# zjykzj/YOLOv4

Measured on AMD Instinct MI355X. Metric: images/sec fwd+bwd @608x608 bs=64 per GPU (YOLOv4 training step: forward + YOLOLoss + backward), higher is better.
Workload: dtype f32

## Files before the change

include/yolov4_amd.h:

```cpp
#ifndef YOLOV4_AMD_H
#define YOLOV4_AMD_H

#include <stddef.h>
#include <stdint.h>

#ifdef __cplusplus
extern "C" {
#endif

#define Y4_OK 0
#define Y4_ERR_SHAPE 1
#define Y4_ERR_NULL 2
#define Y4_ERR_LAUNCH 3
#define Y4_ERR_WORKSPACE 4
#define Y4_ERR_NODEVICE 5
#define Y4_ERR_FORMAT 6
#define Y4_ERR_UNSUPPORTED 7

#define Y4_ACT_LINEAR 0
#define Y4_ACT_LEAKY 1
#define Y4_ACT_MISH 2
#define Y4_ACT_RELU 3

const char* y4_strerror(int code);
int y4_version(void);
int y4_device_count(void);

int y4_set_conv_mode(int mode);
int y4_get_conv_mode(void);
int y4_set_planes_bf16(int on);
int y4_get_planes_bf16(void);
int y4_conv_planes_fit(int B, int H, int W, int Cin, int Cout, int k, int stride, int dgrad_planes);
size_t y4_conv2d_fwd_workspace(int Cin, int Cout, int k);
int y4_conv2d_fwd_f32(const float* x, int ldx, const float* w, float* y, int ldy,
                      int B, int H, int W, int Cin, int Cout, int k, int stride,
                      const float* scale, const float* shift, int act,
                      const float* residual, int ldr, const unsigned* x_amax ,
                      unsigned* y_amax ,
                      void* workspace, size_t workspace_bytes, void* stream);
size_t y4_conv2d_prepared_bytes(int Cout, int K);
int y4_conv2d_prepare_filter_f32(const float* w, int Cout, int K, void* prepared, size_t prepared_bytes, void* stream);
int y4_conv2d_fwd_prepared_f32(const float* x, int ldx, void* w_prepared, float* y, int ldy,
                               int B, int H, int W, int Cin, int Cout, int k, int stride,
                               const float* scale, const float* shift, int act,
                               const float* residual, int ldr, const unsigned* x_amax, unsigned* y_amax, void* stream);
int y4_amax_f32(const float* x, int ldx, long long M, int C, unsigned* amax_bits, void* stream);
int y4_amax_merge_u32(unsigned* dst, const unsigned* src, void* stream);

int y4_last_conv_kernel(char* buf, int cap);

size_t y4_conv2d_bnstats_workspace(int B, int H, int W, int Cin, int Cout, int k, int stride);
int y4_conv2d_fwd_bnstats_f32(const float* x, int ldx, const float* w, float* y, int ldy,
                              int B, int H, int W, int Cin, int Cout, int k, int stride,
                              float* partials, size_t partial_bytes, long long* nparts_host,
                              const unsigned* x_amax ,
                              void* workspace, size_t workspace_bytes ,
                              void* dgrad_filter ,
                              size_t dgrad_filter_bytes , void* stream);

int y4_planes_split_f32(const float* x, int ldx, long long M, int C, const unsigned* amax, void* planes, void* stream);
int y4_planes_split_into_f32(const float* x, int ldx, long long M, int C, const unsigned* amax, void* planes, int ld_planes, int c_valid,
                             void* stream);
int y4_conv2d_fwd_planes_f32(const void* x_planes, const float* w, float* y, int ldy,
                             int B, int H, int W, int Cin, int Cout, int k, int stride,
                             float* partials, size_t partial_bytes, long long* nparts_host, const unsigned* x_amax,
                             void* workspace, size_t workspace_bytes,
                             void* dgrad_filter ,
                             size_t dgrad_filter_bytes,
                             int y_bf16 ,
                             const float* bias ,
                             void* stream);

int y4_conv2d_dgrad_planes_f32(const void* dy_planes, const float* w , float* dx, int lddx,
                               int B, int H, int W, int Cin, int Cout, int k,
                               int stride ,
                               void* workspace, size_t workspace_bytes, const unsigned* dy_amax,
                               const float* residual, int ldr, void* stream);
size_t y4_conv2d_wgrad_planes_workspace(int B, int H, int W, int Cin, int Cout, int k, int stride);
int y4_conv2d_wgrad_planes_f32(const void* x_planes, const void* dy_planes, float* dw,
                               int B, int H, int W, int Cin, int Cout, int k, int stride,
                               void* workspace, size_t workspace_bytes, const unsigned* x_amax, const unsigned* dy_amax,
                               void* stream);

int y4_conv2d_generic_fwd_f32(const float* x, int ldx, const float* w, float* y, int ldy,
                              int B, int H, int W, int Cin, int Cout, int k, int stride,
                              const float* scale, const float* shift, int act, const float* residual, int ldr, void* stream);
int y4_conv2d_generic_dgrad_f32(const float* dy, int lddy, const float* w, float* dx, int lddx,
                                int B, int H, int W, int Cin, int Cout, int k, int stride,
                                const float* residual, int ldr, void* stream);
int y4_conv2d_generic_wgrad_f32(const float* x, int ldx, const float* dy, int lddy, float* dw,
                                int B, int H, int W, int Cin, int Cout, int k, int stride, void* stream);
int y4_conv2d_stem_dgrad_f32(const float* dy, int lddy, const float* w, float* dx, long long sxb, long long sxc, long long sxh,
                             long long sxw, int B, int H, int W, int Cout, void* stream);

int y4_conv2d_stem_fwd_f32(const float* x, long long sxb, long long sxc, long long sxh, long long sxw,
                           const float* w, float* y, int ldy, int B, int H, int W, int Cout,
                           const float* scale, const float* shift, int act,
                           float* bnstats_partials, void* stream);

size_t y4_conv2d_dgrad_workspace(int Cin, int Cout, int k);
int y4_conv2d_dgrad_f32(const float* dy, int lddy, const float* w , float* dx, int lddx,
                        int B, int H, int W, int Cin, int Cout, int k, int stride,
                        void* workspace, size_t workspace_bytes, const unsigned* dy_amax ,
                        const float* residual, int ldr, void* stream);

size_t y4_conv2d_wgrad_workspace(int B, int H, int W, int Cin, int Cout, int k, int stride);
int y4_conv2d_wgrad_f32(const float* x, int ldx, const float* dy, int lddy, float* dw,
                        int B, int H, int W, int Cin, int Cout, int k, int stride,
                        void* workspace, size_t workspace_bytes,
                        const unsigned* x_amax, const unsigned* dy_amax , void* stream);
size_t y4_conv2d_stem_wgrad_workspace(int B, int H, int W, int Cout);
int y4_conv2d_stem_wgrad_f32(const float* x, long long sxb, long long sxc, long long sxh, long long sxw,
                             const float* dy, int lddy, float* dw, int B, int H, int W, int Cout,
                             void* workspace, size_t workspace_bytes, void* stream);

int y4_stem_fused_ok(long long sxb, long long sxc, long long sxh, long long sxw, int B, int H, int W, int Cout);
size_t y4_stem_bn_act_fwd_workspace(int B, int H, int W, int Cout);
int y4_stem_bn_act_fwd_f32(const float* x, long long sxb, long long sxc, long long sxh, long long sxw, const float* w,
                           int B, int H, int W, int Cout, const float* gamma, const float* beta, int act,
                           float* mean, float* invstd, float* running_mean, float* running_var, long long* num_batches_tracked,
                           float momentum, float eps, float* z, int ldz, unsigned* out_amax,
                           void* workspace, size_t workspace_bytes, void* stream);
size_t y4_stem_bn_act_bwd_workspace(int B, int H, int W, int Cout);
int y4_stem_bn_act_bwd_f32(const float* x, long long sxb, long long sxc, long long sxh, long long sxw, const float* w,
                           const float* dz, int lddz, const float* mean, const float* invstd, const float* gamma,
                           const float* beta, int act, int B, int H, int W, int Cout,
                           float* dgamma, float* dbeta, float* dw, void* workspace, size_t workspace_bytes, void* stream);

size_t y4_bn_workspace(long long M, int C);
size_t y4_bn_finalize_workspace(int C);
int y4_bn_stats_f32(const float* y, int ldy, long long M, int C, float* mean, float* invstd,
                    float* running_mean, float* running_var, long long* num_batches_tracked,
                    float momentum, float eps, void* workspace, size_t workspace_bytes, void* stream);
int y4_bn_finalize_partials_f32(const float* partials, long long nparts, long long M, int C,
                                float* mean, float* invstd, float* running_mean, float* running_var,
                                long long* num_batches_tracked, float momentum, float eps,
                                void* workspace, size_t workspace_bytes, void* stream);
int y4_bn_planes_bound_f32(const float* gamma, const float* beta, int C, long long M, const unsigned* floor_word, unsigned* out,
                           void* stream);
int y4_bn_act_fwd_f32(const float* y, int ldy, const float* mean, const float* invstd,
                      const float* gamma, const float* beta, int act,
                      const float* residual, int ldr, float* z, int ldz,
                      long long M, int C, unsigned* out_amax, int z_planes, const unsigned* res_amax, float* planes_twin,
                      void* stream);
int y4_bn_act_bwd_f32(const float* dz, int lddz, const float* y, int ldy,
                      const float* mean, const float* invstd, const float* gamma, const float* beta,
                      int act, float* dy, int lddy, float* dgamma, float* dbeta,
                      long long M, int C, void* workspace, size_t workspace_bytes,
                      unsigned* out_amax ,
                      unsigned* f16_planes ,
                      float* planes_twin ,
                      int frozen_stats ,
                      void* stream);
size_t y4_bias_grad_workspace(long long M, int C);
int y4_bias_grad_f32(const float* dy, int lddy, long long M, int C, float* dbias,
                     void* workspace, size_t workspace_bytes, void* stream);
int y4_bn_fold_f32(const float* gamma, const float* beta, const float* running_mean,
                   const float* running_var, float eps, float* scale, float* shift, int C, void* stream);

int y4_copy_channels_f32(const float* src, int lds, float* dst, int ldd, long long M, int C, void* stream);
int y4_add_f32(const float* a, int lda, const float* b, int ldb, float* out, int ldo,
               long long M, int C, void* stream);
int y4_maxpool_s1_fwd_f32(const float* x, int ldx, float* y, int ldy, signed char* idx,
                          int B, int H, int W, int C, int ksize, void* stream);
int y4_maxpool_s1_bwd_f32(const float* dy, int lddy, const signed char* idx, float* dx, int lddx,
                          int accumulate, int B, int H, int W, int C, int ksize, void* stream);
int y4_upsample2x_fwd_f32(const float* x, int ldx, float* y, int ldy, int B, int H, int W, int C, void* stream);
int y4_upsample2x_bwd_f32(const float* dy, int lddy, float* dx, int lddx, int B, int H, int W, int C, void* stream);

int y4_yolo_decode_train_f32(const float* logits, int ldl, float* output, float* pred,
                             int B, int F, int A, int n_classes, const float* anchors_wh_host, void* stream);
int y4_yolo_decode_eval_f32(const float* logits, int ldl, float* out, long long n_total, long long box_off,
                            int B, int F, int A, int n_classes, const float* anchors_wh_host,
                            float stride, void* stream);
int y4_yolo_decode_bwd_f32(const float* logits, int ldl, const float* g_output, const float* g_pred,
                           float* g_logits, int B, int F, int A, int n_classes,
                           const float* anchors_wh_host, void* stream);

size_t y4_yolo_loss_workspace(int B, int F, int A, int K, int n_classes);
int y4_yolo_loss_fwd_f32(const float* output, const float* pred, const float* labels, int K,
                         int B, int F, int A, int n_classes, float stride, float ignore_thresh,
                         const float* all_anchors_host, int n_all_anchors, const int* anch_mask_host,
                         float* obj_mask, double* loss_parts,
                         void* workspace, size_t workspace_bytes, void* stream);
int y4_yolo_loss_bwd_f32(const float* output, int output_is_masked, const float* obj_mask,
                         const float* gscale, float* g_output,
                         int B, int F, int A, int K, int n_classes,
                         const void* workspace, size_t workspace_bytes, void* stream);
int y4_yolo_loss_mask_output_f32(float* output, const float* obj_mask, int B, int F, int A, int K,
                                 int n_classes, const void* workspace, size_t workspace_bytes, void* stream);
// ... 206 lines not shown
```

yolov4_amd/_lib.py:

```python
import ctypes
import os
from ctypes import c_char_p, c_double, c_float, c_int, c_longlong, c_size_t, c_void_p

_HERE = os.path.dirname(os.path.abspath(__file__))
LIB_PATH = os.environ.get('Y4_LIB_PATH') or os.path.join(_HERE, 'lib', 'libyolov4_amd.so')

ACT_IDS = {'linear': 0, 'leaky_relu': 1, 'mish': 2, 'relu': 3}


class Y4Error(RuntimeError):
    pass


P = c_void_p
I, L, F, Z = c_int, c_longlong, c_float, c_size_t

PROTOTYPES = {
    'y4_strerror': (c_char_p, [I]),
    'y4_version': (I, []),
    'y4_device_count': (I, []),
    'y4_set_conv_mode': (I, [I]),
    'y4_get_conv_mode': (I, []),
    'y4_set_planes_bf16': (I, [I]),
    'y4_get_planes_bf16': (I, []),
    'y4_conv_planes_fit': (I, [I, I, I, I, I, I, I, I]),
    'y4_conv2d_fwd_workspace': (Z, [I, I, I]),
    'y4_conv2d_fwd_f32': (I, [P, I, P, P, I, I, I, I, I, I, I, I, P, P, I, P, I, P, P, P, Z, P]),
    'y4_amax_f32': (I, [P, I, L, I, P, P]),
    'y4_conv2d_prepared_bytes': (Z, [I, I]),
    'y4_conv2d_prepare_filter_f32': (I, [P, I, I, P, Z, P]),
    'y4_conv2d_fwd_prepared_f32': (I, [P, I, P, P, I, I, I, I, I, I, I, I, P, P, I, P, I, P, P, P]),
    'y4_amax_merge_u32': (I, [P, P, P]),
    'y4_last_conv_kernel': (I, [ctypes.c_char_p, I]),
    'y4_conv2d_bnstats_workspace': (Z, [I, I, I, I, I, I, I]),
    'y4_conv2d_fwd_bnstats_f32': (I, [P, I, P, P, I, I, I, I, I, I, I, I, P, Z, P, P, P, Z, P, Z, P]),
    'y4_planes_split_f32': (I, [P, I, L, I, P, P, P]),
    'y4_planes_split_into_f32': (I, [P, I, L, I, P, P, I, I, P]),
    'y4_conv2d_fwd_planes_f32': (I, [P, P, P, I, I, I, I, I, I, I, I, P, Z, P, P, P, Z, P, Z, I, P, P]),
    'y4_conv2d_dgrad_planes_f32': (I, [P, P, P, I, I, I, I, I, I, I, I, P, Z, P, P, I, P]),
    'y4_conv2d_wgrad_planes_workspace': (Z, [I, I, I, I, I, I, I]),
    'y4_conv2d_wgrad_planes_f32': (I, [P, P, P, I, I, I, I, I, I, I, P, Z, P, P, P]),
    'y4_conv2d_generic_fwd_f32': (I, [P, I, P, P, I, I, I, I, I, I, I, I, P, P, I, P, I, P]),
    'y4_conv2d_generic_dgrad_f32': (I, [P, I, P, P, I, I, I, I, I, I, I, I, P, I, P]),
    'y4_conv2d_generic_wgrad_f32': (I, [P, I, P, I, P, I, I, I, I, I, I, I, P]),
    'y4_conv2d_stem_dgrad_f32': (I, [P, I, P, P, L, L, L, L, I, I, I, I, P]),
    'y4_conv2d_stem_fwd_f32': (I, [P, L, L, L, L, P, P, I, I, I, I, I, P, P, I, P, P]),
    'y4_conv2d_dgrad_workspace': (Z, [I, I, I]),
    'y4_conv2d_dgrad_f32': (I, [P, I, P, P, I, I, I, I, I, I, I, I, P, Z, P, P, I, P]),
    'y4_conv2d_wgrad_workspace': (Z, [I, I, I, I, I, I, I]),
    'y4_conv2d_wgrad_f32': (I, [P, I, P, I, P, I, I, I, I, I, I, I, P, Z, P, P, P]),
    'y4_conv2d_stem_wgrad_workspace': (Z, [I, I, I, I]),
    'y4_conv2d_stem_wgrad_f32': (I, [P, L, L, L, L, P, I, P, I, I, I, I, P, Z, P]),
    'y4_stem_fused_ok': (I, [L, L, L, L, I, I, I, I]),
    'y4_stem_bn_act_fwd_workspace': (Z, [I, I, I, I]),
    'y4_stem_bn_act_fwd_f32': (I, [P, L, L, L, L, P, I, I, I, I, P, P, I, P, P, P, P, P, F, F, P, I, P, P, Z, P]),
    'y4_stem_bn_act_bwd_workspace': (Z, [I, I, I, I]),
    'y4_stem_bn_act_bwd_f32': (I, [P, L, L, L, L, P, P, I, P, P, P, P, I, I, I, I, I, P, P, P, P, Z, P]),
    'y4_bn_workspace': (Z, [L, I]),
    'y4_bn_finalize_workspace': (Z, [I]),
    'y4_bn_finalize_partials_f32': (I, [P, L, L, I, P, P, P, P, P, F, F, P, Z, P]),
    'y4_bn_stats_f32': (I, [P, I, L, I, P, P, P, P, P, F, F, P, Z, P]),
    'y4_bn_act_fwd_f32': (I, [P, I, P, P, P, P, I, P, I, P, I, L, I, P, I, P, P, P]),
    'y4_bn_planes_bound_f32': (I, [P, P, I, L, P, P, P]),
    'y4_bn_act_bwd_f32': (I, [P, I, P, I, P, P, P, P, I, P, I, P, P, L, I, P, Z, P, P, P, I, P]),
    'y4_bias_grad_workspace': (Z, [L, I]),
    'y4_bias_grad_f32': (I, [P, I, L, I, P, P, Z, P]),
    'y4_bn_fold_f32': (I, [P, P, P, P, F, P, P, I, P]),
    'y4_copy_channels_f32': (I, [P, I, P, I, L, I, P]),
    'y4_add_f32': (I, [P, I, P, I, P, I, L, I, P]),
    'y4_maxpool_s1_fwd_f32': (I, [P, I, P, I, P, I, I, I, I, I, P]),
    'y4_maxpool_s1_bwd_f32': (I, [P, I, P, P, I, I, I, I, I, I, I, P]),
    'y4_upsample2x_fwd_f32': (I, [P, I, P, I, I, I, I, I, P]),
    'y4_upsample2x_bwd_f32': (I, [P, I, P, I, I, I, I, I, P]),
    'y4_yolo_decode_train_f32': (I, [P, I, P, P, I, I, I, I, P, P]),
    'y4_yolo_decode_eval_f32': (I, [P, I, P, L, L, I, I, I, I, P, F, P]),
    'y4_yolo_decode_bwd_f32': (I, [P, I, P, P, P, I, I, I, I, P, P]),
    'y4_yolo_loss_workspace': (Z, [I, I, I, I, I]),
    'y4_yolo_loss_fwd_f32': (I, [P, P, P, I, I, I, I, I, F, F, P, I, P, P, P, P, Z, P]),
    'y4_yolo_loss_bwd_f32': (I, [P, I, P, P, P, I, I, I, I, I, P, Z, P]),
    'y4_yolo_loss_mask_output_f32': (I, [P, P, I, I, I, I, I, P, Z, P]),
    'y4_yolo_loss_dense_targets_f32': (I, [P, P, P, I, I, I, I, I, P, Z, P]),
    'y4_yolo_box_loss_fwd_f32': (I, [P, I, F, I, I, I, I, I, P, P, Z, P]),
    'y4_yolo_box_loss_bwd_f32': (I, [P, I, F, P, P, I, I, I, I, I, P, Z, P]),
    'y4_post_count_f32': (I, [P, I, L, I, F, I, P, P]),
    'y4_post_scan_i32': (I, [P, I, L, P, P, P]),
    'y4_post_compact_f32': (I, [P, P, P, I, I, P, P, P, P]),
    'y4_post_nms_workspace': (Z, [L, I]),
    'y4_post_nms_f32': (I, [P, I, L, I, F, F, P, L, P, P, P, Z, P]),
    'y4_post_count_ex_f32': (I, [P, I, L, I, F, I, I, P, P]),
    'y4_post_nms_ex_workspace': (Z, [L, I, P]),
    'y4_post_nms_ex_f32': (I, [P, I, L, I, F, F, P, P, L, P, P, P, Z, P]),
    'y4_post_topk_workspace': (Z, [L, I]),
    'y4_post_topk_compact_f32': (I, [P, P, P, I, I, I, L, P, P, P, P, Z, P]),
    'y4_nms_workspace': (Z, [L]),
    'y4_nms_f32': (I, [P, P, L, F, I, P, P, P, Z, P]),
    'y4_bboxes_iou_f32': (I, [P, L, P, L, I, P, P]),
    'y4_act_fwd_f32': (I, [P, P, L, I, P]),
    'y4_act_bwd_f32': (I, [P, P, P, L, I, P]),
    'y4_upsample_nearest_fwd_f32': (I, [P, I, P, I, I, I, I, I, I, I, I, P]),
    'y4_upsample_nearest_bwd_f32': (I, [P, I, P, I, I, I, I, I, I, I, I, P]),
    'y4_adam_step_f32': (I, [P, P, P, P, L, F, F, F, F, F, I, F, P]),
    'y4_adam_hyper_f32': (I, [F, F, F, F, I, P]),
    'y4_adam_multi_step_f32': (I, [P, I, P, I, F, F, F, F, P]),
    'y4_sgd_multi_step_f32': (I, [P, I, P, I, F, P]),
    'y4_grad_sumsq_multi_f32': (I, [P, I, F, P, P]),
    'y4_grad_guard_f32': (I, [P, I, c_double, P, P]),
    'y4_adam_multi_step_guarded_f32': (I, [P, I, P, I, F, F, F, F, P, P]),
    'y4_sgd_multi_step_guarded_f32': (I, [P, I, P, I, F, P, P]),
    'y4_ema_multi_f32': (I, [P, I, F, P, P]),
    'y4_preprocess_u8_f32': (I, [P, I, I, L, I, P, L, L, L, I, P]),
    'y4_augment_means_u8': (I, [P, P, I, P, P]),
    'y4_augment_mosaic_u8_f32': (I, [P, P, I, P, P, I, P, P, L, L, L, L, I, P]),
    'y4_avgpool_global_fwd_f32': (I, [P, I, P, I, I, I, I, P]),
    'y4_avgpool_global_bwd_f32': (I, [P, I, P, I, I, I, I, P]),
    'y4_linear_fwd_f32': (I, [P, I, P, P, P, I, I, I, I, P]),
    'y4_linear_bwd_f32': (I, [P, I, P, P, I, P, I, P, P, I, I, I, P]),
    'y4_ce_smooth_fwd_f32': (I, [P, I, P, I, I, c_double, P, P, P]),
    'y4_ce_smooth_bwd_f32': (I, [P, I, P, P, P, P, I, I, I, c_double, P]),
    'y4_topk_correct_f32': (I, [P, I, P, I, I, P, I, P, P, P]),
    'y4_coco_workspace': (Z, [I, I]),
    'y4_coco_match_f64': (I, [P, P, P, I, P, P, P, P, P, I, I, P, P, P, P, P, Z, P]),
    'y4_coco_accumulate_f64': (I, [P, P, P, I, P, P, P, I, P, P, P, P, P]),
    'y4_jpeg_parse_host': (I, [P, Z, P]),
    'y4_jpeg_entropy_host': (I, [P, Z, P, P, L, P]),
    'y4_jpeg_workspace': (Z, [P, I]),
    'y4_jpeg_decode_u8': (I, [P, P, I, P, Z, P]),
    'y4_jpeg_encode_setup': (I, [I, I, I, I, I, I, P, P]),
    'y4_jpeg_encode_u8': (I, [P, P, I, P]),
    'y4_jpeg_encode_bound': (Z, [P]),
    'y4_jpeg_encode_host': (I, [P, P, P, P, Z, P]),
    'y4_draw_boxes_u8': (I, [P, P, I, P]),
}

ERR_FORMAT, ERR_UNSUPPORTED = 6, 7


NMS_METRICS = {'iou': 0, 'diou': 1}
NMS_SOFT = {None: 0, 'linear': 1, 'gaussian': 2}


class NmsOpts(ctypes.Structure):
    _fields_ = [('metric', c_int), ('soft', c_int), ('sigma', c_float), ('agnostic', c_int), ('max_det', c_int),
                ('reserved', c_int * 3)]


class AugSrc(ctypes.Structure):
    _fields_ = [('src', c_void_p), ('h', c_int), ('w', c_int), ('pitch', c_longlong), ('swap_rb', c_int),
                ('crop_left', c_int), ('crop_top', c_int), ('crop_w', c_int), ('crop_h', c_int), ('flip', c_int),
                ('color', c_int), ('dhue', c_float), ('dsat', c_float), ('dexp', c_float), ('win_x', c_int),
                ('win_y', c_int)]


class AugSample(ctypes.Structure):
    _fields_ = [('cut_x', c_int), ('cut_y', c_int), ('n_src', c_int), ('first', c_int)]


class JpegInfo(ctypes.Structure):
    _fields_ = [('width', c_int), ('height', c_int), ('ncomp', c_int), ('hs', c_int * 3), ('vs', c_int * 3),
                ('mcus_x', c_int), ('mcus_y', c_int), ('blocks_w', c_int * 3), ('blocks_h', c_int * 3),
                ('restart_interval', c_int), ('orientation', c_int), ('reserved', c_int), ('coef_count', c_longlong)]


class JpegJob(ctypes.Structure):
    _fields_ = [('coef', c_void_p), ('out', c_void_p), ('out_pitch', c_longlong), ('ws_offset', c_longlong),
                ('info', JpegInfo), ('apply_orientation', c_int), ('swap_rb', c_int), ('qt', (ctypes.c_uint16 * 64) * 3)]


class JpegEncJob(ctypes.Structure):
    _fields_ = [('pixels', c_void_p), ('coef', c_void_p), ('pitch', c_longlong), ('info', JpegInfo), ('swap_rb', c_int),
                ('reserved', c_int * 3), ('qt', (ctypes.c_uint16 * 64) * 3)]


class DrawBox(ctypes.Structure):
    _fields_ = [('x1', c_int), ('y1', c_int), ('x2', c_int), ('y2', c_int), ('half', c_int), ('px1', c_int), ('py1', c_int),
                ('px2', c_int), ('py2', c_int), ('tx', c_int), ('ty', c_int), ('scale', c_int), ('text_off', c_int),
                ('text_len', c_int), ('color', ctypes.c_uint8 * 4), ('reserved', c_int)]


class DrawJob(ctypes.Structure):
    _fields_ = [('image', c_void_p), ('pitch', c_longlong), ('width', c_int), ('height', c_int), ('boxes', c_void_p),
                ('boxes_host', c_void_p), ('text', c_void_p), ('glyphs', c_void_p), ('n_boxes', c_int), ('text_bytes', c_int),
                ('n_glyphs', c_int), ('reserved', c_int)]


_lib = None


def lib():
    global _lib
    if _lib is None:
        if not os.path.isfile(LIB_PATH):
            raise Y4Error(f'{LIB_PATH} is missing: build it with `make -C yolov4_amd/csrc` '
                          '(hipcc --offload-arch=gfx950); there is no fallback path')
        handle = ctypes.CDLL(LIB_PATH)
        for name, (res, args) in PROTOTYPES.items():
            fn = getattr(handle, name)
            fn.restype = res
            fn.argtypes = args
# ... 20 lines not shown
```

yolov4_amd/csrc/conv_f16x2.hip:

```cpp
#include <stdlib.h>
#include "common.h"
#include <cstdlib>
#include "conv_geom.h"

namespace {

using y4::ConvGeom;
using y4::WgradGeom;

typedef _Float16 f16x8 __attribute__((ext_vector_type(8)));
typedef _Float16 f16x2v __attribute__((ext_vector_type(2)));
typedef unsigned int u32x2 __attribute__((ext_vector_type(2)));

__device__ __host__ __forceinline__ unsigned f16x2_scale_exp(unsigned amax_bits) {
    const unsigned e = (amax_bits >> 23) & 0xffu;
    if (e == 0u || e == 255u) return 127u;
    int se = 268 - (int)e;
    if (se < 2) se = 2;
    if (se > 252) se = 252;
    return (unsigned)se;
}
__device__ __forceinline__ float f16x2_scale(const unsigned* amax) {
    return __uint_as_float(f16x2_scale_exp(amax ? *amax : 0u) << 23);
}
// ... 1292 lines not shown
        const f32x4 v = *reinterpret_cast<const f32x4*>(x + row * ld + c);
#pragma unroll
        for (int e = 0; e < 4; ++e) {
            const unsigned b = __float_as_uint(v[e]) & 0x7fffffffu;
            if (c + e < C && b < 0x7f800000u && b > m) m = b;
        }
    }
    amax_block_commit(m, out);
}
__global__ __launch_bounds__(256) void amax_strided_kernel(const float* __restrict__ x, long long ld, long long M, int C,
                                                           unsigned* __restrict__ out) {
    unsigned m = 0u;
    const long long total = M * C;
    for (long long i = blockIdx.x * (long long)blockDim.x + threadIdx.x; i < total; i += (long long)gridDim.x * blockDim.x) {
        const long long row = i / C;
        const unsigned b = __float_as_uint(x[row * ld + (i - row * C)]) & 0x7fffffffu;
        if (b < 0x7f800000u && b > m) m = b;
    }
    amax_block_commit(m, out);
}
__global__ void amax_merge_kernel(unsigned* __restrict__ dst, const unsigned* __restrict__ src) {
    if (threadIdx.x == 0 && blockIdx.x == 0) { const unsigned v = *src; if (v) atomicMax(dst, v); }
}

constexpr int AMAX_PART_MAX = 1024;
__global__ __launch_bounds__(256) void amax_partials_kernel(const float* __restrict__ x, long long n, unsigned* __restrict__ part) {
    __shared__ unsigned wmax[4];
    unsigned m = 0u;
    const long long n4 = n >> 2;
    for (long long i = blockIdx.x * (long long)blockDim.x + threadIdx.x; i < n4; i += (long long)gridDim.x * blockDim.x) {
        const f32x4 v = *reinterpret_cast<const f32x4*>(x + 4 * i);
#pragma unroll
        for (int e = 0; e < 4; ++e) {
            const unsigned b = __float_as_uint(v[e]) & 0x7fffffffu;
            if (b < 0x7f800000u && b > m) m = b;
        }
    }
    if (blockIdx.x == 0 && threadIdx.x < (int)(n & 3)) {
        const unsigned b = __float_as_uint(x[(n4 << 2) + threadIdx.x]) & 0x7fffffffu;
        if (b < 0x7f800000u && b > m) m = b;
    }
#pragma unroll
    for (int off = 32; off > 0; off >>= 1) {
        const unsigned o = (unsigned)__shfl_xor((int)m, off, 64);
        m = o > m ? o : m;
    }
    if ((threadIdx.x & 63) == 0) wmax[threadIdx.x >> 6] = m;
    __syncthreads();
    if (threadIdx.x == 0) {
        const unsigned a = wmax[0] > wmax[1] ? wmax[0] : wmax[1], b = wmax[2] > wmax[3] ? wmax[2] : wmax[3];
        part[blockIdx.x] = a > b ? a : b;
    }
}
__device__ __forceinline__ unsigned amax_fold_partials(const unsigned* __restrict__ part, int nparts, unsigned* __restrict__ out) {
    __shared__ unsigned wmax[4];
    unsigned m = 0u;
    for (int i = threadIdx.x; i < nparts; i += 256) { const unsigned v = part[i]; m = v > m ? v : m; }
#pragma unroll
    for (int off = 32; off > 0; off >>= 1) {
        const unsigned o = (unsigned)__shfl_xor((int)m, off, 64);
        m = o > m ? o : m;
    }
    if ((threadIdx.x & 63) == 0) wmax[threadIdx.x >> 6] = m;
    __syncthreads();
    const unsigned a = wmax[0] > wmax[1] ? wmax[0] : wmax[1], b = wmax[2] > wmax[3] ? wmax[2] : wmax[3];
    const unsigned v = a > b ? a : b;
    if (blockIdx.x == 0 && threadIdx.x == 0) *out = v;
    return v;
}
__global__ __launch_bounds__(256) void f16x2_split_filter_folded_kernel(const float* __restrict__ w, unsigned short* __restrict__ planes,
                                                                        long long n, const unsigned* __restrict__ part, int nparts,
                                                                        unsigned* __restrict__ amax_out) {
    const unsigned amax = amax_fold_partials(part, nparts, amax_out);
    const float s = __uint_as_float(f16x2_scale_exp(amax) << 23);
    for (long long i = blockIdx.x * (long long)blockDim.x + threadIdx.x; i < n; i += (long long)gridDim.x * blockDim.x) {
        unsigned short hi, lo;
        split2(w[i], s, hi, lo);
        const long long o = (i >> 5) * 64 + (i & 31);
        planes[o] = hi;
        planes[o + 32] = lo;
    }
}
__global__ __launch_bounds__(256) void f16x2_split_filter_dual_kernel(const float* __restrict__ w, unsigned short* __restrict__ planes,
                                                                      unsigned short* __restrict__ planes_t, int Cout, int Cin, int kk,
                                                                      int Cout_pad, const unsigned* __restrict__ part, int nparts,
                                                                      unsigned* __restrict__ amax_out, unsigned* __restrict__ amax_out_t,
                                                                      int mirror) {
    const unsigned amax = amax_fold_partials(part, nparts, amax_out);
    if (blockIdx.x == 0 && threadIdx.x == 0) *amax_out_t = amax;
    const float s = __uint_as_float(f16x2_scale_exp(amax) << 23);
    const long long n = (long long)Cout * kk * Cin;
    for (long long i = blockIdx.x * (long long)blockDim.x + threadIdx.x; i < n; i += (long long)gridDim.x * blockDim.x) {
        unsigned short hi, lo;
        split2(w[i], s, hi, lo);
        const long long o = (i >> 5) * 64 + (i & 31);
        planes[o] = hi;
        planes[o + 32] = lo;
    }
    const long long total = (long long)Cin * kk * Cout_pad;
    for (long long i = blockIdx.x * (long long)blockDim.x + threadIdx.x; i < total; i += (long long)gridDim.x * blockDim.x) {
        const int nn = (int)(i % Cout_pad);
        const long long t = i / Cout_pad;
        const int tp = (int)(t % kk);
        const int tap = mirror ? kk - 1 - tp : tp;
        const int c = (int)(t / kk);
        const float v = nn < Cout ? w[((long long)nn * kk + tap) * Cin + c] : 0.0f;
        unsigned short hi, lo;
        split2(v, s, hi, lo);
        const long long o = (i >> 5) * 64 + (i & 31);
        planes_t[o] = hi;
        planes_t[o + 32] = lo;
    }
}
__global__ __launch_bounds__(256) void f16x2_transpose_split_filter_folded_kernel(const float* __restrict__ w,
                                                                                  unsigned short* __restrict__ planes, int Cout, int Cin,
                                                                                  int kk, int Cout_pad, const unsigned* __restrict__ part,
                                                                                  int nparts, unsigned* __restrict__ amax_out, int mirror) {
    const unsigned amax = amax_fold_partials(part, nparts, amax_out);
    const float s = __uint_as_float(f16x2_scale_exp(amax) << 23);
    const long long total = (long long)Cin * kk * Cout_pad;
    for (long long i = blockIdx.x * (long long)blockDim.x + threadIdx.x; i < total;
         i += (long long)gridDim.x * blockDim.x) {
        const int n = (int)(i % Cout_pad);
        const long long t = i / Cout_pad;
        const int tp = (int)(t % kk);
        const int tap = mirror ? kk - 1 - tp : tp;
        const int c = (int)(t / kk);
        const float v = n < Cout ? w[((long long)n * kk + tap) * Cin + c] : 0.0f;
        unsigned short hi, lo;
        split2(v, s, hi, lo);
        const long long o = (i >> 5) * 64 + (i & 31);
        planes[o] = hi;
        planes[o + 32] = lo;
    }
}

constexpr int FP_PARTS = 256;
__global__ __launch_bounds__(256) void f16x2_refresh_filter_kernel(const float* __restrict__ w, unsigned short* __restrict__ planes,
                                                                   long long n, unsigned* part_max, unsigned long long* part_sum,
                                                                   unsigned* hdr) {
    __shared__ unsigned wmax[4];
    __shared__ unsigned long long wsum[4];
    __shared__ int is_last;
    unsigned m = 0u;
    unsigned long long cs = 0ull;
    auto take = [&](const float x, const unsigned long long i) {
        const unsigned bits = __float_as_uint(x);
        cs += (unsigned long long)bits * (2ull * i + 1ull) + 0x9e3779b97f4a7c15ull;
        const unsigned b = bits & 0x7fffffffu;
        if (b < 0x7f800000u && b > m) m = b;
    };
    {
        const long long n4 = n >> 2, stride = (long long)gridDim.x * blockDim.x;
        long long i = blockIdx.x * (long long)blockDim.x + threadIdx.x;
        for (; i + 3 * stride < n4; i += 4 * stride) {
            f32x4 v[4];
#pragma unroll
            for (int u = 0; u < 4; ++u) v[u] = *reinterpret_cast<const f32x4*>(w + 4 * (i + u * stride));
#pragma unroll
            for (int u = 0; u < 4; ++u)
#pragma unroll
                for (int e = 0; e < 4; ++e) take(v[u][e], (unsigned long long)(4 * (i + u * stride) + e));
        }
        for (; i < n4; i += stride) {
            const f32x4 v = *reinterpret_cast<const f32x4*>(w + 4 * i);
#pragma unroll
            for (int e = 0; e < 4; ++e) take(v[e], (unsigned long long)(4 * i + e));
        }
        if (blockIdx.x == 0 && threadIdx.x < (int)(n & 3)) take(w[(n4 << 2) + threadIdx.x], (unsigned long long)((n4 << 2) + threadIdx.x));
    }
#pragma unroll
    for (int off = 32; off > 0; off >>= 1) {
        const unsigned o = (unsigned)__shfl_xor((int)m, off, 64);
        m = o > m ? o : m;
        cs += __shfl_xor(cs, off, 64);
    }
    if ((threadIdx.x & 63) == 0) { wmax[threadIdx.x >> 6] = m; wsum[threadIdx.x >> 6] = cs; }
    __syncthreads();
    if (threadIdx.x == 0) {
        const unsigned a = wmax[0] > wmax[1] ? wmax[0] : wmax[1], b = wmax[2] > wmax[3] ? wmax[2] : wmax[3];
        __hip_atomic_store(part_max + blockIdx.x, a > b ? a : b, __ATOMIC_RELAXED, __HIP_MEMORY_SCOPE_AGENT);
        __hip_atomic_store(part_sum + blockIdx.x, wsum[0] + wsum[1] + wsum[2] + wsum[3], __ATOMIC_RELAXED, __HIP_MEMORY_SCOPE_AGENT);
        asm volatile("s_waitcnt vmcnt(0)" ::: "memory");
        const unsigned t = __hip_atomic_fetch_add(hdr + 5, 1u, __ATOMIC_RELAXED, __HIP_MEMORY_SCOPE_AGENT);
        is_last = t == gridDim.x - 1;
    }
    __syncthreads();
    if (!is_last) return;
    m = 0u; cs = 0ull;
// ... 107 lines not shown
    const size_t smem = 2ull * 2 * (TN_ + TJ_) * ROWB;
    auto kern = conv_wgrad_f16x2<TN_, TJ_, MS>;
    static Y4DynLds lds_attr;
    if (!lds_attr.ensure(reinterpret_cast<const void*>(kern), smem)) return Y4_ERR_LAUNCH;
    y4::note_kernel("conv_wgrad_f16x2<%d, %d, %d>", TN_, TJ_, MS);
    hipLaunchKernelGGL(kern, dim3(g.ntn * g.ntj * g.splits), dim3(256), smem, st, g);
    Y4_CHECK_LAUNCH();
    return Y4_OK;
}

int f16x2_shape() {
    static int s = -1;
    if (s < 0) {
        const char* e = getenv("Y4_F16X2_SHAPE");
        s = e ? atoi(e) : g_f16x2_shape;
        if (s != 16 && s != 32) s = g_f16x2_shape;
    }
    return s;
}

}

namespace y4 {

int f16x2_gather(const ConvGeom& g, bool transposed, hipStream_t st, int* nparts) {
    if (!transposed && !g.scale && !g.shift && !g.dst_amax && g.act == Y4_ACT_LINEAR && g.pad == 1 &&
        tile_conv_ok(g.Cs, g.Cs_valid, g.N, g.k, g.stride, g.Hs, g.Ws))
        return f16x2_tile(g, st, nparts);
    if (stream1x1_f16x2_ok(g)) return dispatch_stream1x1_f16x2(g, st, nparts);
    if (halo_ok(g)) {
        if (f16x2_shape() == 16) return transposed ? launch_halo_f16x2<true, 16>(g, st, nparts) : launch_halo_f16x2<false, 16>(g, st, nparts);
        return transposed ? launch_halo_f16x2<true, 32>(g, st, nparts) : launch_halo_f16x2<false, 32>(g, st, nparts);
    }
    if (f16x2_shape() == 16)
        return transposed ? dispatch_gather_f16x2<true, 16>(g, st, nparts) : dispatch_gather_f16x2<false, 16>(g, st, nparts);
    return transposed ? dispatch_gather_f16x2<true, 32>(g, st, nparts) : dispatch_gather_f16x2<false, 32>(g, st, nparts);
}

int f16x2_wgrad(const WgradGeom& g, hipStream_t st) {
    if (f16x2_shape() == 16) {
        if (g.tn == 128 && g.tj == 128) return launch_wgrad_f16x2<128, 128, 16>(g, st);
        if (g.tn == 128) return launch_wgrad_f16x2<128, 64, 16>(g, st);
        if (g.tj == 128) return launch_wgrad_f16x2<64, 128, 16>(g, st);
        return launch_wgrad_f16x2<64, 64, 16>(g, st);
    }
    if (g.tn == 128 && g.tj == 128) return launch_wgrad_f16x2<128, 128, 32>(g, st);
    if (g.tn == 128) return launch_wgrad_f16x2<128, 64, 32>(g, st);
    if (g.tj == 128) return launch_wgrad_f16x2<64, 128, 32>(g, st);
    return launch_wgrad_f16x2<64, 64, 32>(g, st);
}

static int filter_amax_partials(const float* w, long long n, unsigned* part, hipStream_t st) {
    if (reinterpret_cast<uintptr_t>(w) & 15) return -1;
    long long blocks = (n / 4 + 1023) / 1024;
    if (blocks < 1) blocks = 1;
    if (blocks > AMAX_PART_MAX) blocks = AMAX_PART_MAX;
    hipLaunchKernelGGL(amax_partials_kernel, dim3((unsigned)blocks), dim3(256), 0, st, w, n, part);
    return (int)blocks;
}

int f16x2_refresh_prepared(const float* w, void* prepared, int Cout, int K, hipStream_t st) {
    const long long n = (long long)Cout * K;
    unsigned* hdr = static_cast<unsigned*>(prepared);
    unsigned* part_max = hdr + 16;
    unsigned long long* part_sum = reinterpret_cast<unsigned long long*>(hdr + 16 + FP_PARTS);
    unsigned short* planes = reinterpret_cast<unsigned short*>(static_cast<char*>(prepared) + 64 + 4096);
    long long blocks = (n + 4095) / 4096;
    if (blocks < 1) blocks = 1;
    if (blocks > FP_PARTS) blocks = FP_PARTS;
    hipLaunchKernelGGL(f16x2_refresh_filter_kernel, dim3((unsigned)blocks), dim3(256), 0, st, w, planes, n, part_max, part_sum, hdr);
    Y4_CHECK_LAUNCH();
    return Y4_OK;
}

int f16x2_filter_planes(const float* w, unsigned short* planes, int Cout, int K, unsigned* amax_out, unsigned* part, hipStream_t st) {
    const long long n = (long long)Cout * K;
    const int np = filter_amax_partials(w, n, part, st);
    if (np < 0) return Y4_ERR_SHAPE;
    Y4_CHECK_LAUNCH();
    const int blocks = (int)((n + 255) / 256 > 4096 ? 4096 : (n + 255) / 256);
    hipLaunchKernelGGL(f16x2_split_filter_folded_kernel, dim3(blocks), dim3(256), 0, st, w, planes, n, part, np, amax_out);
    Y4_CHECK_LAUNCH();
    return Y4_OK;
}

int f16x2_filter_planes_dual(const float* w, unsigned short* planes, unsigned* amax_out, unsigned* part, unsigned short* planes_t,
                             unsigned* amax_out_t, int Cout, int Cin, int kk, int Cout_pad, bool mirror, hipStream_t st) {
    const long long n = (long long)Cout * kk * Cin;
    const int np = filter_amax_partials(w, n, part, st);
    if (np < 0) return Y4_ERR_SHAPE;
    Y4_CHECK_LAUNCH();
    const long long total = (long long)Cin * kk * Cout_pad;
    const long long most = n > total ? n : total;
    const int blocks = (int)((most + 255) / 256 > 4096 ? 4096 : (most + 255) / 256);
    hipLaunchKernelGGL(f16x2_split_filter_dual_kernel, dim3(blocks), dim3(256), 0, st, w, planes, planes_t, Cout, Cin, kk, Cout_pad,
                       part, np, amax_out, amax_out_t, mirror ? 1 : 0);
    Y4_CHECK_LAUNCH();
    return Y4_OK;
}

int f16x2_filter_planes_transposed(const float* w, unsigned short* planes, int Cout, int Cin, int kk, int Cout_pad,
                                   unsigned* amax_out, unsigned* part, hipStream_t st, bool mirror) {
    const int np = filter_amax_partials(w, (long long)Cout * kk * Cin, part, st);
    if (np < 0) return Y4_ERR_SHAPE;
    Y4_CHECK_LAUNCH();
    const long long total = (long long)Cin * kk * Cout_pad;
    const int blocks = (int)((total + 255) / 256 > 4096 ? 4096 : (total + 255) / 256);
    hipLaunchKernelGGL(f16x2_transpose_split_filter_folded_kernel, dim3(blocks), dim3(256), 0, st, w, planes, Cout, Cin, kk,
                       Cout_pad, part, np, amax_out, mirror ? 1 : 0);
    Y4_CHECK_LAUNCH();
    return Y4_OK;
// ... 26 lines not shown
```

yolov4_amd/csrc/conv_geom.h:

```cpp
#pragma once
#include "common.h"

namespace y4 {

struct ConvGeom {
    const float* src; const float* wt; float* dst;
    const float* scale; const float* shift; const float* res;
    float* stats;
    long long lds_, ldd, ldr;
    int B, Hs, Ws, Cs;
    int Cs_valid;
    int Hd, Wd, N;
    int k, stride, pad;
    int M;
    int K;
    int act;
    int mtiles, ntiles;
    int cls_tile0[5];
    int cls_h[2], cls_w[2];
    int cls_slot0[5];
    unsigned long long src_total_bytes;
    unsigned wt_bytes;
    const unsigned short* wt_planes;
    const unsigned* src_amax; const unsigned* wt_amax;
    unsigned* dst_amax;
};

struct WgradGeom {
    const float* x; const float* dy; float* out;
    long long ldx, lddy;
    int B, H, W, Cin, Ho, Wo, Cout;
    int k, stride, pad;
    int M;
    int J;
    int ntn, ntj, splits, chunks_per_split;
    int tn, tj;
    const unsigned* x_amax; const unsigned* dy_amax;
    unsigned long long x_total_bytes, dy_total_bytes;
};

int f16x2_gather(const ConvGeom& g, bool transposed, hipStream_t st, int* nparts);
int f16x2_wgrad(const WgradGeom& g, hipStream_t st);
int f16x2_refresh_prepared(const float* w, void* prepared, int Cout, int K, hipStream_t st);
int f16x2_filter_planes(const float* w, unsigned short* planes, int Cout, int K, unsigned* amax_out, unsigned* part, hipStream_t st);
int f16x2_filter_planes_dual(const float* w, unsigned short* planes, unsigned* amax_out, unsigned* part, unsigned short* planes_t,
                             unsigned* amax_out_t, int Cout, int Cin, int kk, int Cout_pad, bool mirror, hipStream_t st);
int f16x2_filter_planes_transposed(const float* w, unsigned short* planes, int Cout, int Cin, int kk, int Cout_pad,
                                   unsigned* amax_out, unsigned* part, hipStream_t st, bool mirror = false);
int slab_reduce(const float* slabs, float* dw, long long n, int splits, hipStream_t st);
int amax_launch(const float* x, long long ld, long long M, int C, unsigned* amax_bits, hipStream_t st,
                bool prezeroed = false);
int amax_merge(unsigned* dst, const unsigned* src, hipStream_t st);


bool tile_conv_ok(int Cs, int Cs_valid, int N, int k, int stride, int H, int W);
int f16x2_tile(const ConvGeom& g, hipStream_t st, int* nparts);
bool tile_dgrad_s2_ok(int Cs, int Cs_valid, int N, int k, int stride, int Hs, int Ws);
int f16x2_tile_dgrad_s2(const ConvGeom& g, hipStream_t st);

bool tile_wgrad_ok(int Cin, int Cout, int k, int stride, int H, int W, long long ldx, long long lddy);
int tile_wgrad_slabs(int Cin, int Cout);
int f16x2_wgrad_tile(const WgradGeom& g, hipStream_t st);

bool planes_conv_ok(int Cin, int Cout, int k, int stride);
int planes_conv(const void* src, const unsigned* src_amax, const void* wt_planes, const unsigned* wt_amax, float* dst, long long ldd,
                const float* res, long long ldr, float* stats, int* nparts, int B, int Hs, int Ws, int Cs, int N, int k, int stride,
                hipStream_t st, bool bf = false, bool dst_bf16 = false);
int planes_dgrad_s2(const void* dy, const unsigned* dy_amax, const void* wt_planes, const unsigned* wt_amax, float* dx, long long lddx,
                    int B, int H, int W, int Cin, int Cout, hipStream_t st, bool bf = false);
int planes_split(const float* x, long long ld, long long M, int C, const unsigned* amax, void* planes, hipStream_t st, bool bf = false,
                 long long pitch_ch = 0, int c_valid = 0);
void planes_wgrad_plan(int B, int H, int W, int Cin, int Cout, int k, int* ntn, int* ntj, int* splits, int* sps, int tn = 128, bool bf = false);
int planes_wgrad_tn(int Cout, bool bf);
int planes_wgrad(const void* x, const unsigned* x_amax, const void* dy, const unsigned* dy_amax, float* dw, void* workspace,
                 size_t workspace_bytes, int B, int H, int W, int Cin, int Cout, int k, hipStream_t st, bool bf = false,
                 int stride = 1);

void note_kernel(const char* fmt, ...);
}
```

yolov4_amd/csrc/conv_igemm.hip:

```cpp
#include <stdlib.h>
#include "common.h"
#include <cstdarg>
#include <cstdio>
#include "conv_geom.h"

namespace {

constexpr int BK = 32;


using y4::ConvGeom;
using y4::WgradGeom;

template <int BM, int BN, int WM, int WN, bool TRANSPOSED, int BKT = 32>
__global__ __launch_bounds__(256, (BKT == 16 ? 3 : 2)) void conv_gather_mfma_f32(const ConvGeom g) {
    constexpr int LPR = BKT / 4;
    constexpr int RPP = 256 / LPR;
    constexpr int PA = BM / RPP, PB = BN / RPP;
    constexpr int LDS_PITCH = BKT + 4;
    constexpr int BK = BKT;
    constexpr int WTM = BM / WM, WTN = BN / WN;
    constexpr int TM = WTM / 32, TN = WTN / 32;
    static_assert(WM * WN == 4, "4 waves");
    extern __shared__ __attribute__((aligned(16))) float smem[];
// ... 1551 lines not shown

constexpr int STEM_WAVES = 4096;

}

namespace y4 {
int stem_wgrad_fold(const float* slabs, int nslabs, double* part, float* dw, int Cout, hipStream_t st) {
    hipLaunchKernelGGL(stem_wgrad_reduce1_kernel, dim3(64), dim3(256), 0, st, slabs, part, nslabs);
    Y4_CHECK_LAUNCH();
    hipLaunchKernelGGL(stem_wgrad_reduce2_kernel, dim3(1), dim3(256), 0, st, part, dw, 64, Cout);
    Y4_CHECK_LAUNCH();
    return Y4_OK;
}
int slab_reduce(const float* slabs, float* dw, long long n, int splits, hipStream_t st) {
    if ((n & 3) == 0 && !(reinterpret_cast<uintptr_t>(dw) & 15) && !(reinterpret_cast<uintptr_t>(slabs) & 15)) {
        const long long nvec = n / 4;
        if (nvec >= 64 * 1024)
            hipLaunchKernelGGL(slab_reduce_vec_kernel<64>, dim3((unsigned)((nvec + 63) / 64)), dim3(256), 0, st,
                               reinterpret_cast<const f32x4*>(slabs), reinterpret_cast<f32x4*>(dw), nvec, splits);
        else
            hipLaunchKernelGGL(slab_reduce_vec_kernel<16>, dim3((unsigned)((nvec + 15) / 16)), dim3(256), 0, st,
                               reinterpret_cast<const f32x4*>(slabs), reinterpret_cast<f32x4*>(dw), nvec, splits);
    } else {
        const int blocks = (int)((n + 255) / 256 > 2048 ? 2048 : (n + 255) / 256);
        hipLaunchKernelGGL(slab_reduce_kernel, dim3(blocks), dim3(256), 0, st, slabs, dw, n, splits);
    }
    Y4_CHECK_LAUNCH();
    return Y4_OK;
}
}

extern "C" {

int y4_set_conv_mode(int mode) {
    if (mode < 0 || mode > 3) return Y4_ERR_SHAPE;
    g_conv_mode = mode;
    return Y4_OK;
}
int y4_get_conv_mode(void) { return g_conv_mode; }

constexpr size_t FWD_WS_HDR = 64 + 4096;

size_t y4_conv2d_fwd_workspace(int Cin, int Cout, int k) {
    if (Cin <= 0 || Cout <= 0 || k <= 0) return 0;
    return FWD_WS_HDR + (size_t)Cout * k * k * Cin * 6;
}

static int conv_fwd_impl(const float* x, int ldx, const float* w, float* y, int ldy,
                         int B, int H, int W, int Cin, int Cout, int k, int stride,
                         const float* scale, const float* shift, int act,
                         const float* residual, int ldr, float* stats, int* nparts, const unsigned* x_amax,
                         unsigned* y_amax, void* workspace, size_t workspace_bytes, void* stream,
                         void* w_prepared = nullptr, void* dgrad_filter = nullptr, size_t dgrad_filter_bytes = 0) {
    if (!x || (!w && !w_prepared) || !y) return Y4_ERR_NULL;
    if (B <= 0 || H <= 0 || W <= 0 || Cout <= 0 || (k != 1 && k != 3) || (stride != 1 && stride != 2))
        return Y4_ERR_SHAPE;
    if (Cin <= 0 || Cin % BK != 0 || ldx < Cin || ldy < Cout || (ldx & 3) || (residual && ldr < Cout))
        return Y4_ERR_SHAPE;
    if ((reinterpret_cast<uintptr_t>(x) & 15) || (reinterpret_cast<uintptr_t>(w) & 15)) return Y4_ERR_SHAPE;
    const int pad = (k - 1) / 2;
    ConvGeom g{};
    g.src = x; g.wt = w; g.dst = y; g.scale = scale; g.shift = shift; g.res = residual; g.stats = stats;
    g.lds_ = ldx; g.ldd = ldy; g.ldr = ldr;
    g.B = B; g.Hs = H; g.Ws = W; g.Cs = Cin; g.Cs_valid = Cin;
    g.Hd = (H + 2 * pad - k) / stride + 1;
    g.Wd = (W + 2 * pad - k) / stride + 1;
    g.N = Cout; g.k = k; g.stride = stride; g.pad = pad;
    const long long M = (long long)B * g.Hd * g.Wd;
    if (M >= (1ll << 31)) return Y4_ERR_SHAPE;
    g.M = (int)M; g.K = k * k * Cin; g.act = act;
    if (w_prepared) {
        if (g_conv_mode != 3) return Y4_ERR_SHAPE;
        if (reinterpret_cast<uintptr_t>(w_prepared) & 15) return Y4_ERR_SHAPE;
        unsigned* hdr = static_cast<unsigned*>(w_prepared);
        g.wt_planes = reinterpret_cast<unsigned short*>(static_cast<char*>(w_prepared) + 64 + 4096);
        if (!x_amax) {
            const int rc = y4::amax_launch(x, ldx, (long long)B * H * W, Cin, hdr + 1, y4_stream(stream));
            if (rc != Y4_OK) return rc;
            x_amax = hdr + 1;
        }
        g.src_amax = x_amax; g.wt_amax = hdr; g.dst_amax = y_amax;
        return y4::f16x2_gather(g, false, y4_stream(stream), nparts);
    }
    if (g_conv_mode != 0) {
        const long long nw = (long long)Cout * g.K;
        if (!workspace) return Y4_ERR_NULL;
        if (workspace_bytes < y4_conv2d_fwd_workspace(Cin, Cout, k)) return Y4_ERR_WORKSPACE;
        if (reinterpret_cast<uintptr_t>(workspace) & 15) return Y4_ERR_SHAPE;
        unsigned* hdr = static_cast<unsigned*>(workspace);
        unsigned short* planes = reinterpret_cast<unsigned short*>(static_cast<char*>(workspace) + FWD_WS_HDR);
        g.wt_planes = planes;
        if (g_conv_mode == 3) {
            int rc;
            if (dgrad_filter) {
                if (dgrad_filter_bytes < y4_conv2d_dgrad_workspace(Cin, Cout, k)) return Y4_ERR_WORKSPACE;
                if (reinterpret_cast<uintptr_t>(dgrad_filter) & 15) return Y4_ERR_SHAPE;
                const int cp = (Cout + 31) / 32 * 32;
                unsigned* hdr_t = reinterpret_cast<unsigned*>(static_cast<char*>(dgrad_filter) + (size_t)Cin * k * k * cp * 6);
                rc = y4::f16x2_filter_planes_dual(w, planes, hdr, hdr + 16, static_cast<unsigned short*>(dgrad_filter), hdr_t, Cout, Cin,
                                                  k * k, cp, y4::tile_conv_ok(cp, Cout, Cin, k, stride, H, W), y4_stream(stream));
            } else {
                rc = y4::f16x2_filter_planes(w, planes, Cout, g.K, hdr, hdr + 16, y4_stream(stream));
            }
            if (rc != Y4_OK) return rc;
            if (!x_amax) {
                rc = y4::amax_launch(x, ldx, (long long)B * H * W, Cin, hdr + 1, y4_stream(stream));
                if (rc != Y4_OK) return rc;
                x_amax = hdr + 1;
            }
            g.src_amax = x_amax; g.wt_amax = hdr; g.dst_amax = y_amax;
            return y4::f16x2_gather(g, false, y4_stream(stream), nparts);
        }
        const int blocks = (int)((nw + 255) / 256 > 4096 ? 4096 : (nw + 255) / 256);
        hipLaunchKernelGGL(split_filter_kernel, dim3(blocks), dim3(256), 0, y4_stream(stream), w, planes, nw,
                           g_conv_mode == 2 ? 1 : 3);
        Y4_CHECK_LAUNCH();
    }
    return dispatch_gather<false>(g, y4_stream(stream), nparts);
}

int y4_conv2d_fwd_f32(const float* x, int ldx, const float* w, float* y, int ldy,
                      int B, int H, int W, int Cin, int Cout, int k, int stride,
                      const float* scale, const float* shift, int act,
                      const float* residual, int ldr, const unsigned* x_amax, unsigned* y_amax,
                      void* workspace, size_t workspace_bytes, void* stream) {
    return conv_fwd_impl(x, ldx, w, y, ldy, B, H, W, Cin, Cout, k, stride, scale, shift, act, residual, ldr, nullptr,
                         nullptr, x_amax, y_amax, workspace, workspace_bytes, stream);
}

int y4_amax_f32(const float* x, int ldx, long long M, int C, unsigned* amax_bits, void* stream) {
    if (!x || !amax_bits) return Y4_ERR_NULL;
    if (M < 0 || C <= 0 || ldx < C) return Y4_ERR_SHAPE;
    return y4::amax_launch(x, ldx, M, C, amax_bits, y4_stream(stream));
}

int y4_amax_merge_u32(unsigned* dst, const unsigned* src, void* stream) {
    if (!dst || !src) return Y4_ERR_NULL;
    return y4::amax_merge(dst, src, y4_stream(stream));
}

size_t y4_conv2d_bnstats_workspace(int B, int H, int W, int Cin, int Cout, int k, int stride) {
    if (B <= 0 || H <= 0 || W <= 0 || Cout <= 0 || (k != 1 && k != 3) || (stride != 1 && stride != 2)) return 0;
    const int pad = (k - 1) / 2;
    const long long M = (long long)B * ((H + 2 * pad - k) / stride + 1) * ((W + 2 * pad - k) / stride + 1);
    long long rows = Cin == 3 ? (M + 255) / 256 : (M + 63) / 64;
    const long long per_img = (long long)B * ((M / B + 127) / 128);
    if (per_img > rows) rows = per_img;
    return (size_t)rows * 2 * Cout * sizeof(float);
}

int y4_conv2d_fwd_bnstats_f32(const float* x, int ldx, const float* w, float* y, int ldy,
                              int B, int H, int W, int Cin, int Cout, int k, int stride,
                              float* partials, size_t partial_bytes, long long* nparts_host, const unsigned* x_amax,
                              void* workspace, size_t workspace_bytes, void* dgrad_filter, size_t dgrad_filter_bytes,
                              void* stream) {
// ... 48 lines not shown
    ConvGeom g{};
    if (residual && ldr < Cin) return Y4_ERR_SHAPE;
    g.src = dy; g.wt = wt; g.dst = dx; g.scale = nullptr; g.shift = nullptr; g.res = residual;
    g.wt_planes = static_cast<const unsigned short*>(workspace);
    g.lds_ = lddy; g.ldd = lddx; g.ldr = ldr;
    g.B = B;
    g.Hs = (H + 2 * pad - k) / stride + 1;
    g.Ws = (W + 2 * pad - k) / stride + 1;
    g.Cs = Cout_pad; g.Cs_valid = Cout;
    g.Hd = H; g.Wd = W; g.N = Cin; g.k = k; g.stride = stride; g.pad = pad;
    const long long M = (long long)B * H * W;
    if (M >= (1ll << 31)) return Y4_ERR_SHAPE;
    g.M = (int)M; g.K = k * k * Cout_pad; g.act = Y4_ACT_LINEAR;
    if (g_conv_mode == 3) {
        if (!dy_amax) {
            const int rc = y4::amax_launch(dy, lddy, (long long)B * g.Hs * g.Ws, Cout, hdr + 1, st);
            if (rc != Y4_OK) return rc;
            dy_amax = hdr + 1;
        }
        g.src_amax = dy_amax; g.wt_amax = wamax;
        if (y4::tile_conv_ok(Cout_pad, Cout, Cin, k, stride, H, W)) return y4::f16x2_tile(g, st, nullptr);
        if (y4::tile_dgrad_s2_ok(Cout_pad, Cout, Cin, k, stride, g.Hs, g.Ws)) return y4::f16x2_tile_dgrad_s2(g, st);
        return y4::f16x2_gather(g, true, st, nullptr);
    }
    return dispatch_gather<true>(g, st);
}

int y4_conv2d_dgrad_f32(const float* dy, int lddy, const float* w, float* dx, int lddx,
                        int B, int H, int W, int Cin, int Cout, int k, int stride,
                        void* workspace, size_t workspace_bytes, const unsigned* dy_amax,
                        const float* residual, int ldr, void* stream) {
    return conv_dgrad_impl(dy, lddy, w, dx, lddx, B, H, W, Cin, Cout, k, stride, workspace, workspace_bytes, dy_amax,
                           residual, ldr, stream);
}

int y4_last_conv_kernel(char* buf, int cap) {
    if (!buf || cap <= 0) return Y4_ERR_NULL;
    snprintf(buf, (size_t)cap, "%s", g_last_kernel);
    g_last_kernel[0] = 0;
    return Y4_OK;
}

size_t y4_conv2d_prepared_bytes(int Cout, int K) {
    if (Cout <= 0 || K <= 0) return 0;
    return 64 + 4096 + (size_t)Cout * (size_t)K * 4;
}

int y4_conv2d_prepare_filter_f32(const float* w, int Cout, int K, void* prepared, size_t prepared_bytes, void* stream) {
    if (!w || !prepared) return Y4_ERR_NULL;
    if (Cout <= 0 || K <= 0 || (K & 31)) return Y4_ERR_SHAPE;
    if (prepared_bytes < y4_conv2d_prepared_bytes(Cout, K)) return Y4_ERR_WORKSPACE;
    if ((reinterpret_cast<uintptr_t>(prepared) & 15) || (reinterpret_cast<uintptr_t>(w) & 15)) return Y4_ERR_SHAPE;
    return y4::f16x2_refresh_prepared(w, prepared, Cout, K, y4_stream(stream));
}

int y4_conv2d_fwd_prepared_f32(const float* x, int ldx, void* w_prepared, float* y, int ldy,
                               int B, int H, int W, int Cin, int Cout, int k, int stride,
                               const float* scale, const float* shift, int act,
                               const float* residual, int ldr, const unsigned* x_amax, unsigned* y_amax, void* stream) {
    if (!w_prepared) return Y4_ERR_NULL;
    return conv_fwd_impl(x, ldx, nullptr, y, ldy, B, H, W, Cin, Cout, k, stride, scale, shift, act, residual, ldr, nullptr,
                         nullptr, x_amax, y_amax, nullptr, 0, stream, w_prepared);
}

size_t y4_conv2d_wgrad_workspace(int B, int H, int W, int Cin, int Cout, int k, int stride) {
    WgradGeom g{};
    wgrad_plan(B, H, W, Cin, Cout, k, stride, g);
    int splits = g.splits;
    if (y4::tile_wgrad_ok(Cin, Cout, k, stride, H, W, 0, 0) && y4::tile_wgrad_slabs(Cin, Cout) > splits) splits = y4::tile_wgrad_slabs(Cin, Cout);
    return (splits > 1 ? (size_t)splits * Cout * g.J * sizeof(float) : 0) + 64;
}

int y4_conv2d_wgrad_f32(const float* x, int ldx, const float* dy, int lddy, float* dw,
                        int B, int H, int W, int Cin, int Cout, int k, int stride,
                        void* workspace, size_t workspace_bytes, const unsigned* x_amax, const unsigned* dy_amax,
                        void* stream) {
    if (!x || !dy || !dw) return Y4_ERR_NULL;
    if (B <= 0 || H <= 0 || W <= 0 || Cout <= 0 || (k != 1 && k != 3) || (stride != 1 && stride != 2))
        return Y4_ERR_SHAPE;
    if (Cin <= 0 || (Cin & 3) || ldx < Cin || (ldx & 3) || (lddy & 3) || lddy < ((Cout + 3) & ~3)) return Y4_ERR_SHAPE;
    if ((reinterpret_cast<uintptr_t>(x) & 15) || (reinterpret_cast<uintptr_t>(dy) & 15)) return Y4_ERR_SHAPE;
    WgradGeom g{};
    wgrad_plan(B, H, W, Cin, Cout, k, stride, g);
    if ((long long)B * g.Ho * g.Wo >= (1ll << 31)) return Y4_ERR_SHAPE;
    g.x = x; g.dy = dy; g.ldx = ldx; g.lddy = lddy;
    {
        g.x_total_bytes = (unsigned long long)B * H * W * (unsigned long long)ldx * 4ull;
        g.dy_total_bytes = (unsigned long long)B * g.Ho * g.Wo * (unsigned long long)lddy * 4ull;
        const unsigned long long range_px = (unsigned long long)g.chunks_per_split * 32ull + 2ull * g.Ho * g.Wo;
        const unsigned long long per_px = 4ull * (unsigned long long)(lddy > ldx * stride * stride ? lddy : ldx * stride * stride);
        if (range_px * per_px >= 0xfffffff0ull) return Y4_ERR_SHAPE;
    }
    hipStream_t st = y4_stream(stream);
    const bool tile = g_conv_mode == 3 && y4::tile_wgrad_ok(Cin, Cout, k, stride, H, W, ldx, lddy);
    if (tile) g.splits = y4::tile_wgrad_slabs(Cin, Cout);
    const size_t slab_bytes = g.splits > 1 ? (size_t)g.splits * Cout * g.J * sizeof(float) : 0;
    if (g.splits > 1) {
        if (!workspace) return Y4_ERR_NULL;
        if (workspace_bytes < slab_bytes) return Y4_ERR_WORKSPACE;
        g.out = static_cast<float*>(workspace);
    } else {
        g.out = dw;
    }
    int rc;
    if (g_conv_mode == 3) {
        if (!x_amax || !dy_amax) {
// ... 100 lines not shown
```

yolov4_amd/csrc/conv_planes.hip:

```cpp
#include <stdlib.h>
#include <type_traits>
#include "common.h"
#include "conv_geom.h"

namespace {

typedef _Float16 f16x8 __attribute__((ext_vector_type(8)));
typedef float f32x4v __attribute__((ext_vector_type(4)));

__device__ __host__ __forceinline__ unsigned pl_scale_exp(unsigned amax_bits) {
    const unsigned e = (amax_bits >> 23) & 0xffu;
    if (e == 0u || e == 255u) return 127u;
    int se = 268 - (int)e;
    if (se < 2) se = 2;
    if (se > 252) se = 252;
    return (unsigned)se;
}
__device__ __forceinline__ float pl_scale(const unsigned* amax) { return __uint_as_float(pl_scale_exp(amax ? *amax : 0u) << 23); }
__device__ __forceinline__ float pl_unscale(const unsigned* amax) { return __uint_as_float((254u - pl_scale_exp(amax ? *amax : 0u)) << 23); }

struct PlaneConvGeom {
    const unsigned char* src;
    const unsigned char* wt;
    float* dst; long long ldd;
// ... 1128 lines not shown
    const long long total = M * (C / 4);
    const int blocks = (int)((total + 255) / 256 > 4096 ? 4096 : (total + 255) / 256);
    if (bf) {
        hipLaunchKernelGGL(planes_split_bf16_kernel, dim3(blocks > 0 ? blocks : 1), dim3(256), 0, st, x, ld, M, C,
                           static_cast<unsigned char*>(planes), pitch, c_valid > 0 ? c_valid : C);
        Y4_CHECK_LAUNCH();
        return Y4_OK;
    }
    hipLaunchKernelGGL(planes_split_kernel, dim3(blocks > 0 ? blocks : 1), dim3(256), 0, st, x, ld, M, C, amax,
                       static_cast<unsigned char*>(planes), pitch, c_valid > 0 ? c_valid : C);
    Y4_CHECK_LAUNCH();
    return Y4_OK;
}

}

static int g_planes_bf16 = 0;
static inline bool pl_mode_ok() { const int m = y4_get_conv_mode(); return m == 3 || m == 2; }
static inline bool pl_bf() { const int m = y4_get_conv_mode(); return m == 2 || (m == 3 && g_planes_bf16); }

extern "C" {

int y4_set_planes_bf16(int on) { g_planes_bf16 = on ? 1 : 0; return Y4_OK; }
int y4_conv_planes_fit(int B, int H, int W, int Cin, int Cout, int k, int stride, int dgrad_planes) {
    if (!pl_mode_ok()) return 0;
    const bool bf = pl_bf();
    if (bf && ((Cin & 63) || (Cout & 63))) return 0;
    return y4::planes_fit(B, H, W, Cin, Cout, k, stride, bf, dgrad_planes != 0) ? 1 : 0;
}
int y4_get_planes_bf16(void) { return g_planes_bf16; }

int y4_planes_split_f32(const float* x, int ldx, long long M, int C, const unsigned* amax, void* planes, void* stream) {
    if (!x || !planes || (!amax && !pl_bf())) return Y4_ERR_NULL;
    if (M <= 0 || C <= 0 || (C & 31) || ldx < C || (ldx & 3)) return Y4_ERR_SHAPE;
    if (pl_bf() && (C & 63)) return Y4_ERR_SHAPE;
    if ((reinterpret_cast<uintptr_t>(x) & 15) || (reinterpret_cast<uintptr_t>(planes) & 15)) return Y4_ERR_SHAPE;
    return y4::planes_split(x, ldx, M, C, amax, planes, y4_stream(stream), pl_bf());
}

int y4_planes_split_into_f32(const float* x, int ldx, long long M, int C, const unsigned* amax, void* planes, int ld_planes, int c_valid,
                             void* stream) {
    if (!x || !planes || (!amax && !pl_bf())) return Y4_ERR_NULL;
    if (M <= 0 || C <= 0 || (C & 31) || ldx < C || (ldx & 3) || ld_planes < C || (ld_planes & 31) || c_valid < 0 || c_valid > C) return Y4_ERR_SHAPE;
    if (pl_bf() && (C & 63)) return Y4_ERR_SHAPE;
    if ((reinterpret_cast<uintptr_t>(x) & 15) || (reinterpret_cast<uintptr_t>(planes) & 127)) return Y4_ERR_SHAPE;
    return y4::planes_split(x, ldx, M, C, amax, planes, y4_stream(stream), pl_bf(), ld_planes, c_valid);
}

int y4_conv2d_fwd_planes_f32(const void* x_planes, const float* w, float* y, int ldy,
                             int B, int H, int W, int Cin, int Cout, int k, int stride,
                             float* partials, size_t partial_bytes, long long* nparts_host, const unsigned* x_amax,
                             void* workspace, size_t workspace_bytes, void* dgrad_filter, size_t dgrad_filter_bytes,
                             int y_bf16, const float* bias, void* stream) {
    if (!x_planes || !w || !y || !workspace) return Y4_ERR_NULL;
    if (bias && (y_bf16 || partials || (reinterpret_cast<uintptr_t>(bias) & 3))) return Y4_ERR_SHAPE;
    if (!pl_mode_ok()) return Y4_ERR_SHAPE;
    const bool bf = pl_bf();
    if (!bf && !x_amax) return Y4_ERR_NULL;
    if (B <= 0 || H <= 0 || W <= 0 || !y4::planes_conv_ok(Cin, Cout, k, stride) || ldy < Cout || (ldy & 3)) return Y4_ERR_SHAPE;
    if (bf && (Cin & 63)) return Y4_ERR_SHAPE;
    if (workspace_bytes < y4_conv2d_fwd_workspace(Cin, Cout, k)) return Y4_ERR_WORKSPACE;
    if ((reinterpret_cast<uintptr_t>(x_planes) & 15) || (reinterpret_cast<uintptr_t>(w) & 15) ||
        (reinterpret_cast<uintptr_t>(workspace) & 15) || (reinterpret_cast<uintptr_t>(y) & 15)) return Y4_ERR_SHAPE;
    const int pad = (k - 1) / 2;
    const long long M = (long long)B * ((H + 2 * pad - k) / stride + 1) * ((W + 2 * pad - k) / stride + 1);
    if (partials && partial_bytes < (size_t)((M + 127) / 128) * 2 * Cout * sizeof(float)) return Y4_ERR_WORKSPACE;
    hipStream_t st = y4_stream(stream);
    unsigned* hdr = static_cast<unsigned*>(workspace);
    unsigned short* planes = reinterpret_cast<unsigned short*>(static_cast<char*>(workspace) + 64 + 4096);
    int rc;
    if (dgrad_filter) {
        if ((Cout & 31) || (bf && (Cout & 63))) return Y4_ERR_SHAPE;
        if (dgrad_filter_bytes < y4_conv2d_dgrad_workspace(Cin, Cout, k)) return Y4_ERR_WORKSPACE;
        if (reinterpret_cast<uintptr_t>(dgrad_filter) & 15) return Y4_ERR_SHAPE;
        unsigned* hdr_t = reinterpret_cast<unsigned*>(static_cast<char*>(dgrad_filter) + (size_t)Cin * k * k * Cout * 6);
        if (bf) rc = bf16_filter(w, planes, static_cast<unsigned short*>(dgrad_filter), Cout, Cin, k * k, stride == 1, st);
        else rc = y4::f16x2_filter_planes_dual(w, planes, hdr, hdr + 16, static_cast<unsigned short*>(dgrad_filter), hdr_t, Cout, Cin, k * k,
                                               Cout, stride == 1, st);
    } else {
        if (bf) rc = bf16_filter(w, planes, nullptr, Cout, Cin, k * k, false, st);
        else rc = y4::f16x2_filter_planes(w, planes, Cout, k * k * Cin, hdr, hdr + 16, st);
    }
    if (rc != Y4_OK) return rc;
    int np = 0;
    rc = y4::planes_conv(x_planes, x_amax, planes, hdr, y, ldy, bias, 0, partials, &np, B, H, W, Cin, Cout, k, stride, st, bf, y_bf16 != 0);
    if (nparts_host) *nparts_host = np;
    return rc;
}


int y4_conv2d_dgrad_planes_f32(const void* dy_planes, const float* w, float* dx, int lddx,
                               int B, int H, int W, int Cin, int Cout, int k, int stride,
                               void* workspace, size_t workspace_bytes, const unsigned* dy_amax,
                               const float* residual, int ldr, void* stream) {
    if (!dy_planes || !dx || !workspace) return Y4_ERR_NULL;
    if (!pl_mode_ok()) return Y4_ERR_SHAPE;
    const bool bf = pl_bf();
    if (!bf && !dy_amax) return Y4_ERR_NULL;
    if (stride == 2) {
        if ((bf && (Cout & 63)) || k != 3 || residual || B <= 0 || H <= 0 || W <= 0 || (H & 1) || (W & 1) || !y4::planes_conv_ok(Cout, Cin, k, 1) ||
            lddx < Cin || (lddx & 3)) return Y4_ERR_SHAPE;
        if (workspace_bytes < y4_conv2d_dgrad_workspace(Cin, Cout, k)) return Y4_ERR_WORKSPACE;
        if ((reinterpret_cast<uintptr_t>(dy_planes) & 15) || (reinterpret_cast<uintptr_t>(w) & 15) ||
            (reinterpret_cast<uintptr_t>(workspace) & 15) || (reinterpret_cast<uintptr_t>(dx) & 15)) return Y4_ERR_SHAPE;
        hipStream_t st2 = y4_stream(stream);
        unsigned* hdr2 = reinterpret_cast<unsigned*>(static_cast<char*>(workspace) + (size_t)Cin * 9 * Cout * 6);
        if (w) {
            const int rc = bf ? bf16_filter(w, nullptr, static_cast<unsigned short*>(workspace), Cout, Cin, 9, false, st2)
                              : y4::f16x2_filter_planes_transposed(w, static_cast<unsigned short*>(workspace), Cout, Cin, 9, Cout, hdr2, hdr2 + 16, st2, false);
            if (rc != Y4_OK) return rc;
        }
        return y4::planes_dgrad_s2(dy_planes, dy_amax, workspace, hdr2, dx, lddx, B, H, W, Cin, Cout, st2, bf);
    }
    if (stride != 1) return Y4_ERR_SHAPE;
    if (B <= 0 || H <= 0 || W <= 0 || !y4::planes_conv_ok(Cout, Cin, k, 1) || lddx < Cin || (lddx & 3)) return Y4_ERR_SHAPE;
    if (bf && (Cout & 63)) return Y4_ERR_SHAPE;
    if (residual && (ldr < Cin || (ldr & 3) || (reinterpret_cast<uintptr_t>(residual) & 15))) return Y4_ERR_SHAPE;
    if (workspace_bytes < y4_conv2d_dgrad_workspace(Cin, Cout, k)) return Y4_ERR_WORKSPACE;
    if ((reinterpret_cast<uintptr_t>(dy_planes) & 15) || (reinterpret_cast<uintptr_t>(w) & 15) ||
        (reinterpret_cast<uintptr_t>(workspace) & 15) || (reinterpret_cast<uintptr_t>(dx) & 15)) return Y4_ERR_SHAPE;
    hipStream_t st = y4_stream(stream);
    const long long total = (long long)Cin * k * k * Cout;
    unsigned* hdr = reinterpret_cast<unsigned*>(static_cast<char*>(workspace) + (size_t)total * 6);
    if (w) {
        const int rc = bf ? bf16_filter(w, nullptr, static_cast<unsigned short*>(workspace), Cout, Cin, k * k, true, st)
                          : y4::f16x2_filter_planes_transposed(w, static_cast<unsigned short*>(workspace), Cout, Cin, k * k, Cout, hdr, hdr + 16, st, true);
        if (rc != Y4_OK) return rc;
    }
    return y4::planes_conv(dy_planes, dy_amax, workspace, hdr, dx, lddx, residual, ldr, nullptr, nullptr, B, H, W, Cout, Cin, k, 1, st, bf);
}

size_t y4_conv2d_wgrad_planes_workspace(int B, int H, int W, int Cin, int Cout, int k, int stride) {
    if (B <= 0 || H <= 0 || W <= 0 || Cin <= 0 || Cout <= 0 || k <= 0 || (stride != 1 && stride != 2)) return 0;
// ... 28 lines not shown
```

yolov4_amd/csrc/pointwise.hip:

```cpp
#include "common.h"

namespace {

constexpr int PW_THREADS = 256;
constexpr int PW_UNROLL = 4;
#define Y4_ACT_SWITCH(ACTV, CALL)                                              \
    switch (ACTV) {                                                            \
        case Y4_ACT_MISH: { constexpr int A_ = Y4_ACT_MISH; CALL; } break;     \
        case Y4_ACT_LEAKY: { constexpr int A_ = Y4_ACT_LEAKY; CALL; } break;   \
        case Y4_ACT_RELU: { constexpr int A_ = Y4_ACT_RELU; CALL; } break;     \
        default: { constexpr int A_ = Y4_ACT_LINEAR; CALL; } break;            \
    }

struct RowMap {
    int tpr;
    int rpb;
};
static inline RowMap row_map(int C) {
    RowMap r;
    int c4 = C / 4;
    r.tpr = c4 < PW_THREADS ? c4 : PW_THREADS;
    int p = 1;
    while (p * 2 <= r.tpr) p *= 2;
    r.tpr = p;
// ... 73 lines not shown
    for (int c0 = 0; c0 < C2; c0 += cw) {
        const int c = c0 + col;
        double s[8] = {0, 0, 0, 0, 0, 0, 0, 0};
        if (c < C2) {
            long long p = p0 + rg;
            for (; p + 7ll * rg_n < p1; p += 8ll * rg_n) {
                float v[8];
#pragma unroll
                for (int u = 0; u < 8; ++u) v[u] = part[(p + (long long)u * rg_n) * C2 + c];
#pragma unroll
                for (int u = 0; u < 8; ++u) s[u] += (double)v[u];
            }
            for (; p < p1; p += rg_n) s[0] += (double)part[p * C2 + c];
        }
        red[threadIdx.x] = ((s[0] + s[1]) + (s[2] + s[3])) + ((s[4] + s[5]) + (s[6] + s[7]));
        __syncthreads();
        if (rg == 0 && c < C2) {
            double t = red[col];
            for (int g = 1; g < rg_n; ++g) t += red[g * cw + col];
            bacc[(long long)blockIdx.x * C2 + c] = t;
        }
        __syncthreads();
    }
}

__device__ __forceinline__ void fold_rows32(const double* __restrict__ bacc, int nb, int C, int c0, double (&red)[2][8][32],
                                            double& s, double& ss) {
    const int cl = threadIdx.x & 31, g = threadIdx.x >> 5;
    const int c = c0 + cl;
    double a = 0, b2 = 0;
    if (c < C) {
        int r = g;
        for (; r + 56 < nb; r += 64) {
            double va[8], vb[8];
#pragma unroll
            for (int u = 0; u < 8; ++u) {
                va[u] = bacc[(long long)(r + 8 * u) * 2 * C + c];
                vb[u] = bacc[(long long)(r + 8 * u) * 2 * C + C + c];
            }
#pragma unroll
            for (int u = 0; u < 8; ++u) { a += va[u]; b2 += vb[u]; }
        }
        for (; r < nb; r += 8) { a += bacc[(long long)r * 2 * C + c]; b2 += bacc[(long long)r * 2 * C + C + c]; }
    }
    red[0][g][cl] = a; red[1][g][cl] = b2;
    __syncthreads();
    s = 0; ss = 0;
    if (g == 0) {
#pragma unroll
        for (int k = 0; k < 8; ++k) { s += red[0][k][cl]; ss += red[1][k][cl]; }
    }
}

__global__ __launch_bounds__(256) void bn_finalize_kernel(const double* __restrict__ bacc, int nb, long long M, int C, float eps,
                                                          float momentum, float* __restrict__ mean, float* __restrict__ invstd,
                                                          float* __restrict__ rmean, float* __restrict__ rvar, long long* nbt) {
    __shared__ double red[2][8][32];
    double s, ss;
    fold_rows32(bacc, nb, C, blockIdx.x * 32, red, s, ss);
    if (blockIdx.x == 0 && threadIdx.x == 0 && nbt) *nbt += 1;
    const int c = blockIdx.x * 32 + (threadIdx.x & 31);
    if ((threadIdx.x >> 5) != 0 || c >= C) return;
    const double mu = s / (double)M;
    double var = ss / (double)M - mu * mu;
    if (var < 0) var = 0;
    mean[c] = (float)mu;
    invstd[c] = (float)(1.0 / sqrt(var + (double)eps));
    if (rmean) rmean[c] = (1.0f - momentum) * rmean[c] + momentum * (float)mu;
    if (rvar) {
        const double unb = M > 1 ? var * (double)M / (double)(M - 1) : var;
        rvar[c] = (1.0f - momentum) * rvar[c] + momentum * (float)unb;
    }
}


__global__ __launch_bounds__(256) void bn_planes_bound_kernel(const float* __restrict__ gamma, const float* __restrict__ beta, int C,
                                                              float sqrt_m1, const unsigned* __restrict__ res_amax,
                                                              unsigned* __restrict__ out, const unsigned* __restrict__ floor_word = nullptr) {
    __shared__ float red[256];
    float m = 0.f;
    for (int c = threadIdx.x; c < C; c += 256) m = fmaxf(m, fabsf(gamma[c]) * sqrt_m1 + fabsf(beta[c]));
    red[threadIdx.x] = m;
    __syncthreads();
    for (int s = 128; s > 0; s >>= 1) {
        if (threadIdx.x < s) red[threadIdx.x] = fmaxf(red[threadIdx.x], red[threadIdx.x + s]);
        __syncthreads();
    }
    if (threadIdx.x == 0) {
        float b = red[0] * 1.0001f;
        if (res_amax) b += __uint_as_float(*res_amax) * 1.0001f;
        unsigned w = __float_as_uint(b);
        if (floor_word && *floor_word > w) w = *floor_word;
        *out = w;
    }
}


__device__ __forceinline__ unsigned st_off(unsigned voff, unsigned soff) { return voff + soff; }
constexpr int POL_NT = 2;
typedef unsigned u2v __attribute__((ext_vector_type(2)));
__device__ __forceinline__ unsigned pair_swap(unsigned v) {
    return (unsigned)__builtin_amdgcn_update_dpp(0, (int)v, 0xB1, 0xf, 0xf, true);
}
__device__ __forceinline__ unsigned planes_col_off(int c0, bool paired) {
    const unsigned tile = (unsigned)(c0 >> 5) * 128u;
    return paired ? tile + ((c0 & 4) ? 64u : 0u) + (unsigned)((c0 & 24) >> 3) * 16u : tile + (unsigned)(c0 & 31) * 2u;
}
__device__ __forceinline__ void store_planes4(__amdgpu_buffer_rsrc_t rs, unsigned voff, unsigned soff, int c0, const f32x4 o, float ps,
                                              bool paired) {
    typedef _Float16 h2 __attribute__((ext_vector_type(2)));
    h2 h01, h23, l01, l23;
    const float t0 = o[0] * ps, t1 = o[1] * ps, t2 = o[2] * ps, t3 = o[3] * ps;
    h01[0] = (_Float16)t0; h01[1] = (_Float16)t1; h23[0] = (_Float16)t2; h23[1] = (_Float16)t3;
    l01[0] = (_Float16)((t0 - (float)h01[0]) * 2048.f); l01[1] = (_Float16)((t1 - (float)h01[1]) * 2048.f);
    l23[0] = (_Float16)((t2 - (float)h23[0]) * 2048.f); l23[1] = (_Float16)((t3 - (float)h23[1]) * 2048.f);
    const unsigned hv0 = __builtin_bit_cast(unsigned, h01), hv1 = __builtin_bit_cast(unsigned, h23);
    const unsigned lv0 = __builtin_bit_cast(unsigned, l01), lv1 = __builtin_bit_cast(unsigned, l23);
    if (paired) {
        const bool odd = (c0 & 4) != 0;
        const unsigned r0 = pair_swap(odd ? hv0 : lv0), r1 = pair_swap(odd ? hv1 : lv1);
        u32x4 v;
        if (odd) { v[0] = r0; v[1] = r1; v[2] = lv0; v[3] = lv1; }
        else { v[0] = hv0; v[1] = hv1; v[2] = r0; v[3] = r1; }
        __builtin_amdgcn_raw_buffer_store_b128(v, rs, (int)st_off(voff, soff), 0, 0);
    } else {
        u2v hv, lv;
        hv[0] = hv0; hv[1] = hv1; lv[0] = lv0; lv[1] = lv1;
        __builtin_amdgcn_raw_buffer_store_b64(hv, rs, (int)st_off(voff, soff), 0, 0);
        __builtin_amdgcn_raw_buffer_store_b64(lv, rs, (int)(st_off(voff, soff) + 64u), 0, 0);
    }
}

__device__ __forceinline__ void store_bf16x4(__amdgpu_buffer_rsrc_t rs, unsigned voff, unsigned soff, const f32x4 o) {
    u2v v;
    v[0] = (unsigned)__builtin_bit_cast(unsigned short, (__bf16)o[0]) | ((unsigned)__builtin_bit_cast(unsigned short, (__bf16)o[1]) << 16);
    v[1] = (unsigned)__builtin_bit_cast(unsigned short, (__bf16)o[2]) | ((unsigned)__builtin_bit_cast(unsigned short, (__bf16)o[3]) << 16);
    __builtin_amdgcn_raw_buffer_store_b64(v, rs, (int)st_off(voff, soff), 0, 0);
}

template <bool YBF> struct YRaw { u32x4 r; };
template <> struct YRaw<true> { u2v r; };
template <bool YBF, int POL>
__device__ __forceinline__ void y_load(YRaw<YBF>& d, __amdgpu_buffer_rsrc_t rs, unsigned voff, unsigned soff) {
    if constexpr (YBF) d.r = __builtin_amdgcn_raw_buffer_load_b64(rs, (int)voff, (int)soff, POL);
    else d.r = __builtin_amdgcn_raw_buffer_load_b128(rs, (int)voff, (int)soff, POL);
}
template <bool YBF> __device__ __forceinline__ f32x4 y_get(const YRaw<YBF>& d) {
// ... 584 lines not shown
}
static int fold_partials(const float* part, long long nparts, int C, double* bacc, int* nb, hipStream_t st) {
    long long want = (nparts + 15) / 16;
    int blocks = (int)(want < FOLD_BLOCKS ? want : FOLD_BLOCKS);
    if (blocks < 1) blocks = 1;
    const long long per = (nparts + blocks - 1) / blocks;
    blocks = (int)((nparts + per - 1) / per);
    if (blocks < 1) blocks = 1;
    *nb = blocks;
    int cw = 32;
    while (cw < 2 * C && cw < PW_THREADS) cw *= 2;
    hipLaunchKernelGGL(fold_partials_kernel, dim3(blocks), dim3(PW_THREADS), 0, st, part, nparts, 2 * C, cw, bacc);
    Y4_CHECK_LAUNCH();
    return Y4_OK;
}

int y4_bn_stats_f32(const float* y, int ldy, long long M, int C, float* mean, float* invstd,
                    float* running_mean, float* running_var, long long* num_batches_tracked,
                    float momentum, float eps, void* workspace, size_t workspace_bytes, void* stream) {
    if (!y || !mean || !invstd || !workspace) return Y4_ERR_NULL;
    if (!vec_ok(y, ldy, C) || M <= 0) return Y4_ERR_SHAPE;
    if (workspace_bytes < y4_bn_workspace(M, C)) return Y4_ERR_WORKSPACE;
    hipStream_t st = y4_stream(stream);
    double* acc = static_cast<double*>(workspace);
    double* bacc = acc + 2 * C;
    float* part = reinterpret_cast<float*>(acc + (size_t)(1 + FOLD_BLOCKS) * 2 * C);
    const RowMap rm = row_map(C);
    const int nrows = stat_rows(M, rm.rpb);
    const long long blocks = bn_blocks(M, C);
    hipLaunchKernelGGL(bn_stats_kernel, dim3((unsigned)blocks), dim3(PW_THREADS), 0, st, y, (long long)ldy, M, C,
                       rm.tpr, rm.rpb, nrows, part);
    Y4_CHECK_LAUNCH();
    int nb = 0;
    { const int rc = fold_partials(part, blocks, C, bacc, &nb, st); if (rc != Y4_OK) return rc; }
    hipLaunchKernelGGL(bn_finalize_kernel, dim3((C + 31) / 32), dim3(256), 0, st, bacc, nb, M, C, eps, momentum, mean,
                       invstd, running_mean, running_var, num_batches_tracked);
    Y4_CHECK_LAUNCH();
    return Y4_OK;
}

int y4_bn_finalize_partials_f32(const float* partials, long long nparts, long long M, int C,
                                float* mean, float* invstd, float* running_mean, float* running_var,
                                long long* num_batches_tracked, float momentum, float eps,
                                void* workspace, size_t workspace_bytes, void* stream) {
    if (!partials || !mean || !invstd || !workspace) return Y4_ERR_NULL;
    if (nparts <= 0 || M <= 0 || C <= 0) return Y4_ERR_SHAPE;
    if (workspace_bytes < y4_bn_finalize_workspace(C)) return Y4_ERR_WORKSPACE;
    hipStream_t st = y4_stream(stream);
    double* bacc = static_cast<double*>(workspace) + 2 * C;
    int nb = 0;
    { const int rc = fold_partials(partials, nparts, C, bacc, &nb, st); if (rc != Y4_OK) return rc; }
    hipLaunchKernelGGL(bn_finalize_kernel, dim3((C + 31) / 32), dim3(256), 0, st, bacc, nb, M, C, eps, momentum, mean,
                       invstd, running_mean, running_var, num_batches_tracked);
    Y4_CHECK_LAUNCH();
    return Y4_OK;
}

int y4_bn_planes_bound_f32(const float* gamma, const float* beta, int C, long long M, const unsigned* floor_word, unsigned* out,
                           void* stream) {
    if (!gamma || !beta || !out) return Y4_ERR_NULL;
    if (C <= 0 || M <= 0) return Y4_ERR_SHAPE;
    hipLaunchKernelGGL(bn_planes_bound_kernel, dim3(1), dim3(256), 0, y4_stream(stream), gamma, beta, C,
                       sqrtf((float)(M > 1 ? M - 1 : 1)), nullptr, out, floor_word);
    Y4_CHECK_LAUNCH();
    return Y4_OK;
}

int y4_bn_act_fwd_f32(const float* y, int ldy, const float* mean, const float* invstd,
                      const float* gamma, const float* beta, int act,
                      const float* residual, int ldr, float* z, int ldz,
                      long long M, int C, unsigned* out_amax, int z_planes, const unsigned* res_amax, float* planes_twin,
                      void* stream) {
    if (!y || !mean || !invstd || !gamma || !beta) return Y4_ERR_NULL;
    const int ybf = (z_planes >> 4) & 1;
    z_planes &= 15;
    if (!z && (!out_amax || z_planes)) return Y4_ERR_NULL;
    if (z_planes < 0 || z_planes > 3) return Y4_ERR_SHAPE;
    if (planes_twin && (!z_planes || (reinterpret_cast<uintptr_t>(planes_twin) & 15))) return Y4_ERR_SHAPE;
    if (z_planes && ((!out_amax && z_planes != 3) || (C & 31))) return Y4_ERR_SHAPE;
    if (z_planes && !planes_twin && ldz != C && (ldz < C || (ldz & 31) || (reinterpret_cast<uintptr_t>(z) & 127))) return Y4_ERR_SHAPE;
    if (z_planes == 2 && residual && !res_amax) return Y4_ERR_NULL;
    if (!vec_ok(y, ldy, C) || (z && !vec_ok(z, ldz, C)) || (residual && !vec_ok(residual, ldr, C)) || M <= 0)
        return Y4_ERR_SHAPE;
    if (z_planes == 2) {
        hipLaunchKernelGGL(bn_planes_bound_kernel, dim3(1), dim3(256), 0, y4_stream(stream), gamma, beta, C,
                           sqrtf((float)(M > 1 ? M - 1 : 1)), residual ? res_amax : nullptr, out_amax);
        Y4_CHECK_LAUNCH();
    }
    const RowMap rm = row_map(C);
    long long blocks = (M + rm.rpb * PW_UNROLL - 1) / (rm.rpb * PW_UNROLL);
    if (blocks > 256 * 16) blocks = 256 * 16;
    const bool nt = bn_loads_nt(M, C);
#define Y4_BN_FWD(RES_, YBF_)                                                                                                    \
    if (nt) Y4_BN_FWD_(RES_, YBF_, true); else Y4_BN_FWD_(RES_, YBF_, false)
#define Y4_BN_FWD_(RES_, YBF_, NT_)                                                                                              \
    hipLaunchKernelGGL((bn_act_fwd_kernel<A_, RES_, YBF_, NT_>), dim3((unsigned)blocks), dim3(PW_THREADS), 0, y4_stream(stream), y, \
                       (long long)ldy, mean, invstd, gamma, beta, residual, (long long)ldr, z, (long long)ldz, M, C, rm.tpr,      \
                       rm.rpb, z_planes == 3 ? nullptr : out_amax, z_planes == 3 ? 2 : (z_planes ? 1 : 0), planes_twin)
    if (residual) {
        if (ybf) { Y4_ACT_SWITCH(act, Y4_BN_FWD(true, true)); }
        else { Y4_ACT_SWITCH(act, Y4_BN_FWD(true, false)); }
    } else {
        if (ybf) { Y4_ACT_SWITCH(act, Y4_BN_FWD(false, true)); }
        else { Y4_ACT_SWITCH(act, Y4_BN_FWD(false, false)); }
    }
#undef Y4_BN_FWD
// ... 227 lines not shown
```

yolov4_amd/darknet/darknet.py:

```python
import os

import torch
from torch import nn

from .. import ops


class Mish(nn.Module):

    def forward(self, x):
        return ops.ActFn.apply(x, 'mish')


_ACT_MODULES = {
    'relu': lambda: nn.ReLU(inplace=True),
    'leaky_relu': lambda: nn.LeakyReLU(negative_slope=0.1, inplace=True),
    'mish': Mish,
    'linear': nn.Identity,
}


class ConvBNAct(nn.Module):

    def __init__(self, in_ch: int, out_ch: int, kernel_size: int, stride: int, bias=False, bn=True, act='leaky_relu'):
        super().__init__()
        if act not in _ACT_MODULES:
            raise ValueError(f"{act} does not support.")
        pad = (kernel_size - 1) // 2
        self.conv = nn.Conv2d(in_ch, out_ch, (kernel_size, kernel_size), (stride, stride), padding=pad, bias=bias)
        self.conv.weight.data = self.conv.weight.data.contiguous(memory_format=torch.channels_last)
        self.norm = nn.BatchNorm2d(out_ch) if bn else nn.Identity()
        self.act = _ACT_MODULES[act]()
        self.act_name = act
        self.kernel_size = kernel_size
        self.stride = stride
        self.has_bn = bool(bn)

    def forward(self, x, residual=None, out=None, dres_put=None, dres_take=None, out_planes=False, dx_put=None, scale_from=None):
        n = self.norm
        io = {}
        out_planes = soft(out_planes, self)
        cfg = {'out': out, 'k': self.kernel_size, 's': self.stride, 'act': self.act_name, 'bn': self.has_bn,
               'training': self.training, 'io': io, 'x_amax': ops.amax_of(x), 'out_amax': ops.amax_of(out),
               'dres_put': dres_put, 'dres_take': dres_take, 'out_planes': out_planes, 'dx_put': dx_put,
               'out_cat': getattr(out, 'y4_cat', None), 'scale_from': scale_from,
               'x_twin': getattr(x, 'y4_twin', None) if takes_planes(self, x.shape[2:], geo_of(x)) else None,
               'grad': torch.is_grad_enabled()}
        if self.has_bn:
            use_batch_stats = self.training or n.running_mean is None
            cfg['training'] = use_batch_stats
            cfg['eps'] = n.eps
            cfg['momentum'] = n.momentum if n.momentum is not None else 1.0 / float(int(n.num_batches_tracked) + 1)
            track = self.training and n.track_running_stats
            cfg['running_mean'] = n.running_mean if (track or not use_batch_stats) else None
            cfg['running_var'] = n.running_var if (track or not use_batch_stats) else None
            cfg['nbt'] = n.num_batches_tracked if track else None
            gamma, beta = n.weight, n.bias
            cfg['gamma_param'], cfg['beta_param'] = n.weight, n.bias
        else:
            gamma = beta = None
        w = self.conv.weight
        if w.dim() == 4 and not w.is_contiguous(memory_format=torch.channels_last):
            self.conv.weight.data = w.data.contiguous(memory_format=torch.channels_last)
            w = self.conv.weight
        cfg['weight_param'] = self.conv.weight
        z = ops.ConvBNActFn.apply(x, w, self.conv.bias, gamma, beta, residual, cfg)
        if io.get('z_planes'):
            z = ops.as_planes(z)
        if io.get('z_twin') is not None:
            z.y4_twin = io['z_twin']
        return ops.tag_amax(z, io.get('z_amax'))


def observed(*mods):
    g = torch.nn.modules.module
    if (g._global_forward_hooks or g._global_forward_pre_hooks or g._global_backward_hooks or g._global_backward_pre_hooks
            or getattr(g, '_global_forward_hooks_always_called', None)):
        return True
    for m in mods:
        if m is not None and (m._forward_hooks or m._forward_pre_hooks or m._backward_hooks or m._backward_pre_hooks):
            return True
    return False


def soft(want, *mods):
    return 'both' if (want is True and observed(*mods)) else want


def takes_planes(m, hw=None, geo=None):
    if isinstance(m, ConvBNAct) and not m.has_bn:
        return _nobn_takes_planes(m, geo)
    if not isinstance(m, ConvBNAct) or not m.has_bn or not m.training:
        return False
    if geo is not None and hw is None and m.stride == 1:
        hw = geo[1:]
    if m.stride != 1 and not (hw is not None and ops.planes_stride2_ok(m.kernel_size, m.stride, int(hw[0]), int(hw[1]))):
        return False
    ci, co = m.conv.in_channels, m.conv.out_channels
    pm = ops.planes_mode()
    co_min = 64 if (pm == 'bf16' and _BF16_N64 and m.kernel_size == 1 and m.stride == 1) else 128
    if ci % 32 or co % 32 or co < co_min or ci < 64 or m.kernel_size not in (1, 3):
        return False
    if not (ops.PLANES['on'] and m.conv.weight.is_cuda):
        return False
    if not (pm == 'f16x2' or (pm == 'bf16' and ci % 64 == 0 and co % 64 == 0)):
        return False
    return geo is None or ops.planes_fit(geo[0], geo[1], geo[2], ci, co, m.kernel_size, m.stride, dgrad=m.stride == 1)


_HEAD_PLANES = os.environ.get('Y4_HEAD_PLANES', '1') != '0'
_BF16_N64 = os.environ.get('Y4_BF16_N64', '1') != '0'


def _nobn_takes_planes(m, geo):
    if not (_HEAD_PLANES and m.training and torch.is_grad_enabled() and m.act_name == 'linear' and m.stride == 1
            and m.kernel_size in (1, 3) and ops.PLANES['on'] and m.conv.weight.is_cuda):
        return False
    pm = ops.planes_mode()
    if pm is None:
# ... 152 lines not shown
```

yolov4_amd/ops.py:

```python
import ctypes
import functools
import os

import torch

from ._lib import ACT_IDS, Y4Error, check, float_array, int_array, lib

CL = torch.channels_last


def _stream():
    return ctypes.c_void_p(torch.cuda.current_stream().cuda_stream)


def _ptr(t):
    return ctypes.c_void_p(t.data_ptr()) if t is not None else None


def _require_gpu(t, what):
    if not t.is_cuda:
        raise Y4Error(f'{what}: tensor is on {t.device}; the yolov4_amd hot path runs on an MI355X only '
                      '(no CPU fallback)')
    if t.dtype != torch.float32:
        raise Y4Error(f'{what}: expected float32, got {t.dtype}')


def nhwc_pitch(t):
    if t.dim() != 4:
        return None
    B, C, H, W = t.shape
    sb, sc, sh, sw = t.stride()
    if C > 1 and sc != 1:
        return None
    ld = sw if W > 1 else (sh if H > 1 else (sb if B > 1 else C))
    if ld < C:
        return None
    if W > 1 and sw != ld:
        return None
    if H > 1 and sh != W * ld:
        return None
    if B > 1 and sb != H * W * ld:
        return None
    return ld


def empty_nhwc(B, C, H, W, device, pad_to=1):
    Cp = (C + pad_to - 1) // pad_to * pad_to
    buf = torch.empty((B, Cp, H, W), device=device, dtype=torch.float32, memory_format=CL)
    return buf if Cp == C else buf[:, :C]


def as_nhwc(t, need_vec4=True, min_pitch=0):
    ld = nhwc_pitch(t)
    ok = ld is not None and (not need_vec4 or (ld % 4 == 0 and t.data_ptr() % 16 == 0)) and ld >= min_pitch
    if ok:
        return t, ld
    B, C, H, W = t.shape
    pad = 1
    if need_vec4:
# ... 149 lines not shown
_S2_PLANES = os.environ.get('Y4_PLANES_S2', '1') != '0'
_S2_DGRAD_PLANES = os.environ.get('Y4_PLANES_S2_DGRAD', '1') != '0'
_BF16_Y = os.environ.get('Y4_BF16_Y', '1') != '0'


def conv_fwd_raw(x, w, k, s, scale=None, shift=None, act='linear', residual=None, out=None, out_pad=1, x_amax=None,
                 out_amax=None, w_prepared=None):
    L = lib()
    B, Cin, H, W = x.shape
    Cout = w.shape[0]
    Ho, Wo = conv_out_hw(H, W, k, s)
    if out is None:
        out = empty_nhwc(B, Cout, Ho, Wo, x.device, pad_to=out_pad)
    ldy = nhwc_pitch(out)
    w = krsc(w)
    if not fast_conv_shape(Cin, k, s) or (Cin == 3 and (Cout > 32 or residual is not None)):
        if k % 2 == 0:
            raise Y4Error('even kernel sizes are not supported (pad = (k - 1) // 2 would not keep the map size)')
        x, ldx = as_nhwc(x, need_vec4=False)
        ldr = 0
        if residual is not None:
            residual, ldr = as_nhwc(residual, need_vec4=False)
        check(L.y4_conv2d_generic_fwd_f32(_ptr(x), ldx, _ptr(w), _ptr(out), ldy, B, H, W, Cin, Cout, k, s, _ptr(scale), _ptr(shift),
                                          ACT_IDS[act], _ptr(residual), ldr, _stream()), 'conv2d_generic_fwd')
        return out
    if Cin == 3:
        if k != 3 or s != 1 or residual is not None:
            raise Y4Error('Cin=3 is supported for the 3x3/s1 stem only')
        sb, sc, sh, sw = x.stride()
        check(L.y4_conv2d_stem_fwd_f32(_ptr(x), sb, sc, sh, sw, _ptr(w), _ptr(out), ldy, B, H, W, Cout,
                                       _ptr(scale), _ptr(shift), ACT_IDS[act], None, _stream()), 'conv2d_stem_fwd')
        return out
    x, ldx = as_nhwc(x)
    ldr = 0
    if residual is not None:
        residual, ldr = as_nhwc(residual, need_vec4=False)
    if w_prepared is not None:
        check(L.y4_conv2d_fwd_prepared_f32(_ptr(x), ldx, _ptr(w_prepared), _ptr(out), ldy, B, H, W, Cin, Cout, k, s,
                                           _ptr(scale), _ptr(shift), ACT_IDS[act], _ptr(residual), ldr, _ptr(x_amax),
                                           _ptr(out_amax), _stream()), 'conv2d_fwd_prepared')
        return out
    nbytes = L.y4_conv2d_fwd_workspace(Cin, Cout, k)
    ws = _ws(nbytes, x.device)
    check(L.y4_conv2d_fwd_f32(_ptr(x), ldx, _ptr(w), _ptr(out), ldy, B, H, W, Cin, Cout, k, s,
                              _ptr(scale), _ptr(shift), ACT_IDS[act], _ptr(residual), ldr, _ptr(x_amax), _ptr(out_amax),
                              _ptr(ws), nbytes, _stream()), 'conv2d_fwd')
    return out


def dgrad_filter_buffer(Cin, Cout, k, device):
    return _ws(lib().y4_conv2d_dgrad_workspace(Cin, Cout, k), device)


def conv_fwd_bnstats_raw(x, w, k, s, running_mean, running_var, nbt, momentum, eps, x_amax=None, dgrad_filter=None):
    L = lib()
    B, Cin, H, W = x.shape
    Cout = w.shape[0]
    Ho, Wo = conv_out_hw(H, W, k, s)
    if not fast_conv_shape(Cin, k, s) or (Cin == 3 and Cout > 32) or Cout % 4:
        if Cout % 4:
            raise Y4Error('BatchNorm over a channel count that is not a multiple of 4 is not supported')
        y = conv_fwd_raw(x, w, k, s, out=empty_nhwc(B, Cout, Ho, Wo, x.device, pad_to=4), x_amax=x_amax)
        mean, invstd = bn_stats_raw(y, running_mean, running_var, nbt, momentum, eps)
        return y, mean, invstd
    y = empty_nhwc(B, Cout, Ho, Wo, x.device)
    ldy = nhwc_pitch(y)
    w = krsc(w)
    pbytes = L.y4_conv2d_bnstats_workspace(B, H, W, Cin, Cout, k, s)
    part = _ws(pbytes, x.device)
    if Cin == 3:
        if k != 3 or s != 1:
            raise Y4Error('Cin=3 is supported for the 3x3/s1 stem only')
        sb, sc, sh, sw = x.stride()
        check(L.y4_conv2d_stem_fwd_f32(_ptr(x), sb, sc, sh, sw, _ptr(w), _ptr(y), ldy, B, H, W, Cout,
                                       None, None, ACT_IDS['linear'], _ptr(part), _stream()), 'conv2d_stem_fwd')
        nparts = (B * H * W + 255) // 256
    else:
        x, ldx = as_nhwc(x)
        n = ctypes.c_longlong(0)
        nbytes = L.y4_conv2d_fwd_workspace(Cin, Cout, k)
        cws = _ws(nbytes, x.device)
        check(L.y4_conv2d_fwd_bnstats_f32(_ptr(x), ldx, _ptr(w), _ptr(y), ldy, B, H, W, Cin, Cout, k, s,
                                          _ptr(part), pbytes, ctypes.byref(n), _ptr(x_amax), _ptr(cws), nbytes,
                                          _ptr(dgrad_filter), dgrad_filter.numel() if dgrad_filter is not None else 0, _stream()),
              'conv2d_fwd_bnstats')
        nparts = n.value
    mean = torch.empty(Cout, device=x.device, dtype=torch.float32)
    invstd = torch.empty(Cout, device=x.device, dtype=torch.float32)
    wsb = L.y4_bn_finalize_workspace(Cout)
    ws = _ws(wsb, x.device)
    check(L.y4_bn_finalize_partials_f32(_ptr(part), nparts, B * Ho * Wo, Cout, _ptr(mean), _ptr(invstd),
                                        _ptr(running_mean), _ptr(running_var), _ptr(nbt), float(momentum), float(eps),
                                        _ptr(ws), wsb, _stream()), 'bn_finalize_partials')
    return y, mean, invstd


def stem_fused_ok(x, Cout, k, s):
    if x.dim() != 4 or x.shape[1] != 3 or k != 3 or s != 1 or x.dtype != torch.float32:
        return False
    B, _, H, W = x.shape
    return bool(lib().y4_stem_fused_ok(*x.stride(), B, H, W, Cout))


def stem_bn_act_fwd_raw(x, w, gamma, beta, act, running_mean, running_var, nbt, momentum, eps, out=None, out_amax=None):
    L = lib()
    B, _, H, W = x.shape
    Cout = w.shape[0]
    z = out if _slot_ok(out, (B, Cout, H, W)) else empty_nhwc(B, Cout, H, W, x.device)
    mean = torch.empty(Cout, device=x.device, dtype=torch.float32)
    invstd = torch.empty(Cout, device=x.device, dtype=torch.float32)
    nbytes = L.y4_stem_bn_act_fwd_workspace(B, H, W, Cout)
    ws = _ws(nbytes, x.device)
    check(L.y4_stem_bn_act_fwd_f32(_ptr(x), *x.stride(), _ptr(krsc(w)), B, H, W, Cout, _ptr(gamma), _ptr(beta), ACT_IDS[act],
                                   _ptr(mean), _ptr(invstd), _ptr(running_mean), _ptr(running_var), _ptr(nbt), float(momentum),
                                   float(eps), _ptr(z), nhwc_pitch(z), _ptr(out_amax), _ptr(ws), nbytes, _stream()),
          'stem_bn_act_fwd')
    return z, mean, invstd


def stem_bn_act_bwd_raw(x, w, dz, mean, invstd, gamma, beta, act, dgamma_out=None, dbeta_out=None, dw_out=None):
    L = lib()
    B, _, H, W = x.shape
    Cout = w.shape[0]
    dz, lddz = as_nhwc(dz, need_vec4=False)

    def slot(t):
        ok = t is not None and t.dtype == torch.float32 and tuple(t.shape) == (Cout,) and t.is_contiguous() and t.is_cuda
        return t if ok else torch.empty(Cout, device=x.device, dtype=torch.float32)
    dgamma, dbeta = slot(dgamma_out), slot(dbeta_out)
    if dw_out is not None and tuple(dw_out.shape) == tuple(w.shape) and _is_krsc_dense(dw_out):
        dw = dw_out
        WGRAD_STATS['in_place'] += 1
    else:
        WGRAD_STATS['temporary'] += 1
        dw = krsc(torch.empty(tuple(w.shape), device=x.device, dtype=torch.float32).contiguous(memory_format=CL))
    nbytes = L.y4_stem_bn_act_bwd_workspace(B, H, W, Cout)
    ws = _ws(nbytes, x.device)
    check(L.y4_stem_bn_act_bwd_f32(_ptr(x), *x.stride(), _ptr(krsc(w)), _ptr(dz), lddz, _ptr(mean), _ptr(invstd), _ptr(gamma),
                                   _ptr(beta), ACT_IDS[act], B, H, W, Cout, _ptr(dgamma), _ptr(dbeta), _ptr(dw),
                                   _ptr(ws), nbytes, _stream()), 'stem_bn_act_bwd')
    return dw, dgamma, dbeta


class Planes:
    __slots__ = ('buf', 'shape', 'amax')

# ... 4 lines not shown
class PlanesTensor(torch.Tensor):
    __torch_function__ = torch._C._disabled_torch_function_impl

    def _refuse(self, *a, **kw):
        raise Y4Error('this tensor holds a PRE-SPLIT activation (two fp16 pieces per element, csrc/conv_planes.hip), not '
                      'float32 values: only ConvBNAct can consume it.  Register the forward hook before the forward pass '
                      '(hooked modules return fp32), or run with Y4_PLANES=0 to keep every intermediate tensor fp32.')

    cpu = to = numpy = tolist = item = float = double = half = bfloat16 = int = long = clone = _refuse
    sum = mean = abs = max = min = amax = amin = norm = std = var = exp = log = sigmoid = tanh = relu = _refuse
    __add__ = __radd__ = __sub__ = __rsub__ = __mul__ = __rmul__ = __truediv__ = __rtruediv__ = __neg__ = __pow__ = _refuse
    __iadd__ = __isub__ = __imul__ = __itruediv__ = __matmul__ = __getitem__ = __setitem__ = _refuse
    __lt__ = __le__ = __gt__ = __ge__ = __float__ = __int__ = __bool__ = __array__ = __dlpack__ = _refuse
    __reduce_ex__ = __reduce__ = __deepcopy__ = _refuse

    def __repr__(self, *a, **kw):
        return (f'PlanesTensor(shape={tuple(self.shape)}, device={self.device}: pre-split fp16 pairs, NOT float32 values; '
                'see yolov4_amd.ops.PlanesTensor)')

    __str__ = __repr__

    def __format__(self, spec):
        return self.__repr__()

    def detach(self):
        return as_planes(torch.Tensor.detach(self), getattr(self, 'y4_amax', None))


def as_planes(t, cell=None):
    if type(t) is not PlanesTensor:
        t = t.as_subclass(PlanesTensor)
    t.y4_planes = True
    if cell is not None:
        t.y4_amax = cell
    return t


def planes_split_raw(x, amax=None):
    L = lib()
    B, C, H, W = x.shape
    x, ldx = as_nhwc(x)
    if planes_mode() == 'bf16':
        amax = None
    else:
        if amax is None:
            amax = amax_of(x)
        if amax is None:
            amax = amax_raw(x)
    buf = torch.empty((B, H, W, C * 4), dtype=torch.uint8, device=x.device)
    check(L.y4_planes_split_f32(_ptr(x), ldx, B * H * W, C, _ptr(amax), _ptr(buf), _stream()), 'planes_split')
    return Planes(buf, (B, C, H, W), amax)


def conv_fwd_planes_raw(xp, w, k, s, stats=True, dgrad_filter=None, y_bf16=False, bias=None, out=None):
    L = lib()
    B, Cin, H, W = xp.shape
    Cout = w.shape[0]
    Ho, Wo = conv_out_hw(H, W, k, s)
    y = out if _slot_ok(out, (B, Cout, Ho, Wo)) else empty_nhwc(B, Cout, Ho, Wo, xp.buf.device)
    w = krsc(w)
    nbytes = L.y4_conv2d_fwd_workspace(Cin, Cout, k)
    ws = _ws(nbytes, xp.buf.device)
    pbytes = ((B * Ho * Wo + 127) // 128) * 2 * Cout * 4 if stats else 0
    part = _ws(pbytes, xp.buf.device) if stats else None
    n = ctypes.c_longlong(0)
    check(L.y4_conv2d_fwd_planes_f32(_ptr(xp.buf), _ptr(w), _ptr(y), nhwc_pitch(y), B, H, W, Cin, Cout, k, s,
                                     _ptr(part), pbytes, ctypes.byref(n), _ptr(xp.amax), _ptr(ws), nbytes,
                                     _ptr(dgrad_filter), dgrad_filter.numel() if dgrad_filter is not None else 0,
                                     1 if y_bf16 else 0, _ptr(bias), _stream()),
          'conv2d_fwd_planes')
    return (y, part, n.value) if stats else y


def conv_fwd_planes_bnstats_raw(xp, w, k, s, running_mean, running_var, nbt, momentum, eps, dgrad_filter=None, y_bf16=False):
    L = lib()
    y, part, nparts = conv_fwd_planes_raw(xp, w, k, s, dgrad_filter=dgrad_filter, y_bf16=y_bf16)
    Cout = w.shape[0]
    M = y.shape[0] * y.shape[2] * y.shape[3]
    mean = torch.empty(Cout, device=y.device, dtype=torch.float32)
    invstd = torch.empty(Cout, device=y.device, dtype=torch.float32)
    wsb = L.y4_bn_finalize_workspace(Cout)
    ws = _ws(wsb, y.device)
    check(L.y4_bn_finalize_partials_f32(_ptr(part), nparts, M, Cout, _ptr(mean), _ptr(invstd),
                                        _ptr(running_mean), _ptr(running_var), _ptr(nbt), float(momentum), float(eps),
                                        _ptr(ws), wsb, _stream()), 'bn_finalize_partials')
    return y, mean, invstd


def planes_of(t):
    if t is None or not getattr(t, 'y4_planes', False):
        return None
    return Planes(t, t.shape, getattr(t, 'y4_amax', None))


def conv_dgrad_planes_raw(dyp, w, x_shape, k, residual=None, prepared=None, s=1):
    L = lib()
    B, Cin, H, W = x_shape
    Cout = w.shape[0]
    dx = empty_nhwc(B, Cin, H, W, dyp.buf.device)
    nbytes = L.y4_conv2d_dgrad_workspace(Cin, Cout, k)
    ws = prepared if prepared is not None else _ws(nbytes, dyp.buf.device)
    ldr = 0
    if residual is not None:
        residual, ldr = as_nhwc(residual)
    check(L.y4_conv2d_dgrad_planes_f32(_ptr(dyp.buf), None if prepared is not None else _ptr(krsc(w)), _ptr(dx), nhwc_pitch(dx), B, H, W, Cin, Cout, k,
                                       s, _ptr(ws), nbytes, _ptr(dyp.amax), _ptr(residual), ldr, _stream()), 'conv2d_dgrad_planes')
    return dx


def conv_wgrad_planes_raw(xp, dyp, w_shape, k, out=None, s=1):
    L = lib()
    B, Cin, H, W = xp.shape
    Cout = w_shape[0]
    if out is not None and tuple(out.shape) == tuple(w_shape) and _is_krsc_dense(out) and out.data_ptr() % 16 == 0:
        dw = out
        WGRAD_STATS['in_place'] += 1
    else:
        WGRAD_STATS['temporary'] += 1
        dw = krsc(torch.empty(w_shape, device=xp.buf.device, dtype=torch.float32).contiguous(memory_format=CL))
    nbytes = L.y4_conv2d_wgrad_planes_workspace(B, H, W, Cin, Cout, k, s)
    ws = _ws(nbytes, xp.buf.device)
    check(L.y4_conv2d_wgrad_planes_f32(_ptr(xp.buf), _ptr(dyp.buf), _ptr(dw), B, H, W, Cin, Cout, k, s, _ptr(ws), nbytes,
                                       _ptr(xp.amax), _ptr(dyp.amax), _stream()), 'conv2d_wgrad_planes')
    return dw


def conv_stem_dgrad_raw(dy, w, x):
    L = lib()
    B, _, H, W = x.shape
    dy, lddy = as_nhwc(dy, need_vec4=False)
    dx = torch.empty_like(x, memory_format=torch.preserve_format)
    sb, sc, sh, sw = dx.stride()
    check(L.y4_conv2d_stem_dgrad_f32(_ptr(dy), lddy, _ptr(krsc(w)), _ptr(dx), sb, sc, sh, sw, B, H, W, w.shape[0], _stream()),
          'conv2d_stem_dgrad')
    return dx


def last_conv_kernel():
# ... 47 lines not shown
    Cout = w_shape[0]
    if out is not None and tuple(out.shape) == tuple(w_shape) and _is_krsc_dense(out) and out.data_ptr() % 16 == 0:
        dw = out
        WGRAD_STATS['in_place'] += 1
    else:
        WGRAD_STATS['temporary'] += 1
        dw = torch.empty(w_shape, device=dy.device, dtype=torch.float32).contiguous(memory_format=CL)
        dw = krsc(dw)
    if k not in (1, 3) or s not in (1, 2) or (Cin % 4 and Cin != 3) or (Cin == 3 and (k != 3 or s != 1 or Cout > 32)):
        xs, ldx = as_nhwc(x, need_vec4=False)
        dys, lddy = as_nhwc(dy, need_vec4=False)
        check(L.y4_conv2d_generic_wgrad_f32(_ptr(xs), ldx, _ptr(dys), lddy, _ptr(dw), B, H, W, Cin, Cout, k, s, _stream()),
              'conv2d_generic_wgrad')
        return dw
    if Cin == 3:
        dy, lddy = as_nhwc(dy, need_vec4=False)
        nbytes = L.y4_conv2d_stem_wgrad_workspace(B, H, W, Cout)
        ws = _ws(nbytes, dy.device)
        sb, sc, sh, sw = x.stride()
        check(L.y4_conv2d_stem_wgrad_f32(_ptr(x), sb, sc, sh, sw, _ptr(dy), lddy, _ptr(dw), B, H, W, Cout,
                                         _ptr(ws), nbytes, _stream()), 'conv2d_stem_wgrad')
        return dw
    x, ldx = as_nhwc(x)
    dy, lddy = as_nhwc(dy, min_pitch=(Cout + 3) // 4 * 4)
    nbytes = L.y4_conv2d_wgrad_workspace(B, H, W, Cin, Cout, k, s)
    ws = _ws(nbytes, dy.device)
    check(L.y4_conv2d_wgrad_f32(_ptr(x), ldx, _ptr(dy), lddy, _ptr(dw), B, H, W, Cin, Cout, k, s,
                                _ptr(ws), nbytes, _ptr(x_amax), _ptr(dy_amax), _stream()), 'conv2d_wgrad')
    return dw


def bn_stats_raw(y, running_mean, running_var, nbt, momentum, eps):
    L = lib()
    B, C, H, W = y.shape
    y, ld = as_nhwc(y)
    mean = torch.empty(C, device=y.device, dtype=torch.float32)
    invstd = torch.empty(C, device=y.device, dtype=torch.float32)
    nbytes = L.y4_bn_workspace(B * H * W, C)
    ws = _ws(nbytes, y.device)
    check(L.y4_bn_stats_f32(_ptr(y), ld, B * H * W, C, _ptr(mean), _ptr(invstd), _ptr(running_mean),
                            _ptr(running_var), _ptr(nbt), float(momentum), float(eps), _ptr(ws), nbytes, _stream()),
          'bn_stats')
    return mean, invstd


def _slot_ok(out, shape):
    if out is None:
        return False
    ld = nhwc_pitch(out)
    return (tuple(out.shape) == tuple(shape) and out.dtype == torch.float32 and ld is not None and ld % 4 == 0
            and out.data_ptr() % 16 == 0)


def bn_act_fwd_raw(y, mean, invstd, gamma, beta, act, residual=None, out=None, out_amax=None, planes=False, y_bf16=False, cell=None):
    L = lib()
    B, C, H, W = y.shape
    y, ldy = as_nhwc(y)
    ldr = 0
    if residual is not None:
        residual, ldr = as_nhwc(residual)
    yb = 16 if y_bf16 else 0
    if planes == 'slot':
        cb = out.y4_cat
        if residual is not None or not _slot_ok(out, (B, C, H, W)):
            raise Y4Error('a pre-split concat slot takes a BatchNorm result of its own shape, without a skip operand')
        bf = planes_mode() == 'bf16'
        zp = out.data_ptr()
        if bf:
            zp = cb.buf.data_ptr() + (zp - cb.buf.data_ptr()) // 2
        check(L.y4_bn_act_fwd_f32(_ptr(y), ldy, _ptr(mean), _ptr(invstd), _ptr(gamma), _ptr(beta), ACT_IDS[act], None, 0,
                                  ctypes.c_void_p(zp), nhwc_pitch(out), B * H * W, C, None if bf else _ptr(cb.cell[0:1]),
                                  (3 if bf else 1) + yb, None, None, _stream()), 'bn_act_fwd(planes slot)')
        return out
    if planes:
        both = planes == 'both'
        zp = empty_nhwc(B, C, H, W, y.device)
        z = (out if _slot_ok(out, (B, C, H, W)) else empty_nhwc(B, C, H, W, y.device)) if both else zp
        args = (_ptr(y), ldy, _ptr(mean), _ptr(invstd), _ptr(gamma), _ptr(beta), ACT_IDS[act], _ptr(residual), ldr)
        if planes_mode() == 'bf16':
            check(L.y4_bn_act_fwd_f32(*args, _ptr(z), nhwc_pitch(z), B * H * W, C, None, 3 + yb, None,
                                      _ptr(zp) if both else None, _stream()), 'bn_act_fwd(bf16)')
            zp = as_planes(zp)
            if both:
                z.y4_twin = zp
                return z
            return zp
        given = cell is not None
        if given and (residual is not None or both):
            raise Y4Error('a given plane scale goes with a plain planes-only result')
        cell = cell if given else planes_cell(y.device)
        res_cell = amax_of(residual) if residual is not None else None
        if given:
            mode = 1
        elif residual is not None and res_cell is None:
            check(L.y4_bn_act_fwd_f32(*args, None, C, B * H * W, C, _ptr(cell), yb, None, None, _stream()), 'bn_act_fwd(measure)')
            mode = 1
        else:
            mode = 2
        check(L.y4_bn_act_fwd_f32(*args, _ptr(z), nhwc_pitch(z), B * H * W, C, _ptr(cell), mode + yb, _ptr(res_cell),
                                  _ptr(zp) if both else None, _stream()), 'bn_act_fwd(planes)')
        zp = as_planes(zp, cell)
        if both:
            z.y4_twin = zp
            return tag_amax(z, cell[0:1])
        return as_planes(zp, cell[0:1])
    z = out if _slot_ok(out, (B, C, H, W)) else empty_nhwc(B, C, H, W, y.device)
    check(L.y4_bn_act_fwd_f32(_ptr(y), ldy, _ptr(mean), _ptr(invstd), _ptr(gamma), _ptr(beta), ACT_IDS[act],
                              _ptr(residual), ldr, _ptr(z), nhwc_pitch(z), B * H * W, C, _ptr(out_amax), yb, None, None, _stream()),
          'bn_act_fwd')
    return z


def bn_act_bwd_raw(dz, y, mean, invstd, gamma, beta, act, dgamma_out=None, dbeta_out=None, out_amax=None, planes=None,
                   frozen=False, bf16=False, twin=False, y_bf16=False):
    L = lib()
    B, C, H, W = y.shape
    dz, lddz = as_nhwc(dz)
    y, ldy = as_nhwc(y)
    dy = empty_nhwc(B, C, H, W, y.device)

    def slot(t):
        ok = t is not None and t.dtype == torch.float32 and tuple(t.shape) == (C,) and t.is_contiguous() and t.is_cuda
        return t if ok else torch.empty(C, device=y.device, dtype=torch.float32)
    dgamma, dbeta = slot(dgamma_out), slot(dbeta_out)
    dyp = empty_nhwc(B, C, H, W, y.device) if twin else None
    nbytes = L.y4_bn_workspace(B * H * W, C)
    ws = _ws(nbytes, y.device)
    check(L.y4_bn_act_bwd_f32(_ptr(dz), lddz, _ptr(y), ldy, _ptr(mean), _ptr(invstd), _ptr(gamma), _ptr(beta),
                              ACT_IDS[act], _ptr(dy), nhwc_pitch(dy), _ptr(dgamma), _ptr(dbeta), B * H * W, C,
                              _ptr(ws), nbytes, _ptr(out_amax), _ptr(planes), _ptr(dyp) if twin else None,
                              (1 if frozen else 0) | (2 if bf16 else 0) | (4 if y_bf16 else 0), _stream()),
          'bn_act_bwd')
    if twin:
        return dy, dgamma, dbeta, dyp
    return dy, dgamma, dbeta


def bias_grad_raw(dy):
    L = lib()
    B, C, H, W = dy.shape
    dy, ld = as_nhwc(dy, need_vec4=False)
    db = torch.empty(C, device=dy.device, dtype=torch.float32)
    nbytes = L.y4_bias_grad_workspace(B * H * W, C)
    ws = _ws(nbytes, dy.device)
    check(L.y4_bias_grad_f32(_ptr(dy), ld, B * H * W, C, _ptr(db), _ptr(ws), nbytes, _stream()), 'bias_grad')
# ... 28 lines not shown
    if ldd is None:
        raise Y4Error('copy_into: destination is not NHWC')
    check(L.y4_copy_channels_f32(_ptr(src), lds, _ptr(dst), ldd, B * H * W, C, _stream()), 'copy_channels')


_ASYNC = {'on': os.environ.get('Y4_ASYNC_WGRAD', '0') == '1', 'streams': {}, 'join_queued': False}


def set_async_wgrad(on):
    _ASYNC['on'] = bool(on)


def side_stream(device):
    key = device.index if device.index is not None else torch.cuda.current_device()
    st = _ASYNC['streams'].get(key)
    if st is None:
        st = torch.cuda.Stream(device=device)
        _ASYNC['streams'][key] = st
    return st


def join_side_stream(device=None):
    for st in _ASYNC['streams'].values():
        torch.cuda.current_stream(st.device).wait_stream(st)
    _ASYNC['join_queued'] = False


def _wgrad_to_param(x, dy, param, k, s, x_amax=None, dy_amax=None, fn=None):
    main = torch.cuda.current_stream(x.device)
    side = side_stream(x.device)
    ev = main.record_event()
    with torch.cuda.stream(side):
        side.wait_event(ev)
        dw = fn() if fn is not None else conv_wgrad_raw(x, dy, tuple(param.shape), k, s, x_amax=x_amax, dy_amax=dy_amax)
        if param.grad is None:
            dw.record_stream(main)
            param.grad = dw
        else:
            param.grad.record_stream(side)
            param.grad.add_(dw)
        ready = getattr(param, '_y4_grad_ready', None)
        if ready is not None:
            ready()
    x.record_stream(side)
    dy.record_stream(side)
    for cell in (x_amax, dy_amax):
        if cell is not None:
            cell.record_stream(side)
    if not _ASYNC['join_queued']:
        _ASYNC['join_queued'] = True
        torch.autograd.Variable._execution_engine.queue_callback(join_side_stream)


def _pad_out_channels(weight, bias, cop):
    co = weight.shape[0]
    if cop == co:
        return weight, bias
    wp = torch.zeros((cop,) + tuple(weight.shape[1:]), dtype=weight.dtype, device=weight.device).contiguous(memory_format=torch.channels_last)
    wp[:co].copy_(weight)
    bp = None
    if bias is not None:
        bp = torch.zeros(cop, dtype=bias.dtype, device=bias.device)
        bp[:co].copy_(bias)
    return wp, bp


def _split_padded(t, cop, amax=None):
    B, C, H, W = t.shape
    t, ld = as_nhwc(t)
    if ld < cop:
        v = empty_nhwc(B, cop, H, W, t.device)
        v[:, :C].copy_(t)
        t, ld = v, nhwc_pitch(v)
    buf = torch.empty((B, H, W, cop * 4), dtype=torch.uint8, device=t.device)
    check(lib().y4_planes_split_into_f32(_ptr(t), ld, B * H * W, cop, _ptr(amax), _ptr(buf), cop, C, _stream()), 'planes_split(padded)')
    return Planes(buf, (B, cop, H, W), amax)


class ConvBNActFn(torch.autograd.Function):

    @staticmethod
    def forward(ctx, x, weight, bias, gamma, beta, residual, cfg):
        k, s, act, training, bn = cfg['k'], cfg['s'], cfg['act'], cfg['training'], cfg['bn']
        _require_gpu(x, 'ConvBNAct input')
        _require_gpu(weight, 'ConvBNAct weight')
        dest = cfg.pop('out', None)
        ctx.cfg = {key: cfg.get(key) for key in ('k', 's', 'act', 'gamma_param', 'beta_param', 'weight_param',
                                                 'dres_put', 'dres_take', 'dx_put')}
        ctx.x_shape = tuple(x.shape)
        ctx.has_res = residual is not None
        f16 = f16x2_mode() and x.shape[1] != 3
        bfm = planes_mode() == 'bf16'
        xp = planes_of(x)
        if xp is None and cfg.get('x_twin') is not None:
            xp = planes_of(cfg['x_twin'])
        ctx.x_planes = xp is not None
        nobn_planes = xp is not None and not bn and act == 'linear' and residual is None and s == 1 and cfg.get('grad', True)
        if xp is not None and not ((f16 or bfm) and x.shape[1] % 32 == 0 and (nobn_planes or (
                bn and training and weight.shape[0] % 32 == 0 and (s == 1 or planes_stride2_ok(k, s, x.shape[2], x.shape[3]))))):
            raise Y4Error('a pre-split (planes) tensor reached a conv that cannot consume it')
        x_amax = live(cfg.get('x_amax')) if f16 else None
        z_amax = None
        io = cfg.get('io')
        if xp is not None:
            x_amax = xp.amax
        elif f16 and x_amax is None and (ctx.needs_input_grad[0] or ctx.needs_input_grad[1]):
            x_amax = amax_raw(x)
        ctx.x_amax = x_amax
        if bn and training:
            if x.shape[0] * conv_out_hw(x.shape[2], x.shape[3], k, s)[0] * conv_out_hw(x.shape[2], x.shape[3], k, s)[1] <= 1:
                raise ValueError('Expected more than 1 value per channel when training')
            ctx.dgrad_filter = None
            if ((f16 or (bfm and xp is not None)) and ctx.needs_input_grad[0] and x.shape[1] % 32 == 0 and fast_conv_shape(x.shape[1], k, s)
                    and weight.shape[0] % 4 == 0 and (xp is None or weight.shape[0] % 32 == 0)
                    and not (bfm and xp is not None and s == 2
                             and not s2_plane_dgrad(x.shape[0], x.shape[2], x.shape[3], x.shape[1], weight.shape[0]))):
                ctx.dgrad_filter = dgrad_filter_buffer(x.shape[1], weight.shape[0], k, x.device)
            ybf = ctx.y_bf16 = bool(bfm and xp is not None and weight.shape[0] % 32 == 0 and _BF16_Y)
            cb = cfg.get('out_cat')
            if (xp is None and residual is None and not cfg.get('out_planes') and not (cb is not None and cb.planes)
                    and not ctx.needs_input_grad[0] and stem_fused_ok(x, weight.shape[0], k, s)):
                if f16x2_mode():
                    z_amax = live(cfg.get('out_amax')) if (dest is not None and _slot_ok(dest, (x.shape[0], weight.shape[0]) + tuple(x.shape[2:]))) else None
                    if z_amax is None:
                        z_amax = new_amax(x.device)
                z, mean, invstd = stem_bn_act_fwd_raw(x, weight, gamma, beta, act, cfg['running_mean'], cfg['running_var'],
                                                      cfg['nbt'], cfg['momentum'], cfg['eps'], out=dest, out_amax=z_amax)
                ctx.save_for_backward(x, weight, mean, invstd, gamma, beta)
                ctx.mode = 'stem_fused'
                if io is not None:
                    io['z_amax'] = z_amax
                return z
            if xp is not None:
                y, mean, invstd = conv_fwd_planes_bnstats_raw(xp, weight, k, s, cfg['running_mean'], cfg['running_var'],
                                                              cfg['nbt'], cfg['momentum'], cfg['eps'], dgrad_filter=ctx.dgrad_filter,
                                                              y_bf16=ybf)
            else:
                y, mean, invstd = conv_fwd_bnstats_raw(x, weight, k, s, cfg['running_mean'], cfg['running_var'],
                                                       cfg['nbt'], cfg['momentum'], cfg['eps'], x_amax=x_amax,
                                                       dgrad_filter=ctx.dgrad_filter)
            want = cfg.get('out_planes')
            cb = cfg.get('out_cat')
            if cb is not None and cb.planes:
                z = bn_act_fwd_raw(y, mean, invstd, gamma, beta, act, residual, out=dest, planes='slot', y_bf16=ybf)
                if io is not None:
                    io['z_planes'] = True
                z_amax = cb.cell[0:1] if cb.cell is not None else None
            elif want and (f16 or bfm) and y.shape[1] % 32 == 0 and (want == 'both' or dest is None):
                sf = cfg.get('scale_from')
                z = bn_act_fwd_raw(y, mean, invstd, gamma, beta, act, residual, out=dest if want == 'both' else None,
                                   planes='both' if want == 'both' else True, y_bf16=ybf,
                                   cell=sf.cell if (sf is not None and sf.planes and sf.cell is not None and want is True) else None)
                z_amax = getattr(z, 'y4_amax', None)
                if io is not None:
                    io['z_planes'] = want != 'both'
                    io['z_twin'] = getattr(z, 'y4_twin', None)
            else:
                if f16x2_mode():
                    z_amax = live(cfg.get('out_amax')) if (dest is not None and _slot_ok(dest, tuple(y.shape))) else None
                    if z_amax is None:
                        z_amax = new_amax(x.device)
                z = bn_act_fwd_raw(y, mean, invstd, gamma, beta, act, residual, out=dest, out_amax=z_amax, y_bf16=ybf)
            ctx.save_for_backward(xp.buf if xp is not None else x, weight, y, mean, invstd, gamma, beta)
            ctx.mode = 'bn_train'
        elif bn and cfg.get('grad', True) and any(ctx.needs_input_grad[i] for i in (0, 1, 3, 4)):
            y = conv_fwd_raw(x, weight, k, s, x_amax=x_amax, out=empty_nhwc(x.shape[0], weight.shape[0],
                                                                              *conv_out_hw(x.shape[2], x.shape[3], k, s), x.device, pad_to=4))
            invstd, _ = bn_fold_raw(torch.ones_like(gamma), beta, cfg['running_mean'], cfg['running_var'], cfg['eps'])
            mean = cfg['running_mean']
            if f16x2_mode():
                z_amax = live(cfg.get('out_amax')) if (dest is not None and _slot_ok(dest, tuple(y.shape))) else None
                if z_amax is None:
                    z_amax = new_amax(x.device)
            z = bn_act_fwd_raw(y, mean, invstd, gamma, beta, act, residual, out=dest, out_amax=z_amax)
            ctx.save_for_backward(x, weight, y, mean.detach().clone(), invstd, gamma, beta)
            ctx.mode = 'bn_eval_grad'
        elif bn:
            frozen = not cfg.get('grad', True) and os.environ.get('Y4_NO_INFER_CACHE') != '1'
            fast = f16 and fast_conv_shape(x.shape[1], k, s)
            wprep = prepared_filter(cfg['weight_param']) if (frozen and fast and cfg.get('weight_param') is not None) else None
            scale, shift = bn_fold_raw(gamma, beta, cfg['running_mean'], cfg['running_var'], cfg['eps'])
            o = dest
            Ho, Wo = conv_out_hw(x.shape[2], x.shape[3], k, s)
            o = o if _slot_ok(o, (x.shape[0], weight.shape[0], Ho, Wo)) else None
            if fast:
                z_amax = live(cfg.get('out_amax')) if o is not None else None
                if z_amax is None:
                    z_amax = new_amax(x.device)
            z = conv_fwd_raw(x, weight, k, s, scale, shift, act, residual, out=o, x_amax=x_amax, out_amax=z_amax,
                             w_prepared=wprep)
            ctx.mode = 'bn_eval'
        elif nobn_planes:
            co = weight.shape[0]
            q = 64 if bfm else 32
            cop = (co + q - 1) // q * q
            wpad, bpad = _pad_out_channels(weight, bias, cop)
            Ho, Wo = conv_out_hw(x.shape[2], x.shape[3], k, s)
            zf = empty_nhwc(x.shape[0], cop, Ho, Wo, x.device)
            ctx.dgrad_filter = dgrad_filter_buffer(x.shape[1], cop, k, x.device) if ctx.needs_input_grad[0] else None
            conv_fwd_planes_raw(xp, wpad, k, s, stats=False, dgrad_filter=ctx.dgrad_filter, bias=bpad, out=zf)
            z = zf[:, :co]
            ctx.save_for_backward(xp.buf, weight)
            ctx.mode = 'nobn_linear'
        else:
            wprep = prepared_filter(cfg['weight_param']) if (not cfg.get('grad', True) and f16 and fast_conv_shape(x.shape[1], k, s)
                                                              and os.environ.get('Y4_NO_INFER_CACHE') != '1'
                                                              and cfg.get('weight_param') is not None) else None
            z = conv_fwd_raw(x, weight, k, s, None, bias, act, residual, out_pad=32, x_amax=x_amax, w_prepared=wprep)
            if act != 'linear':
                ctx.mode = 'nobn_act'
            else:
                ctx.save_for_backward(x, weight)
                ctx.mode = 'nobn_linear'
        if io is not None:
            io['z_amax'] = z_amax
        return z

    @staticmethod
    def backward(ctx, dz):
        cfg = ctx.cfg
        k, s, act = cfg['k'], cfg['s'], cfg['act']
        f16 = f16x2_mode() and ctx.x_shape[1] != 3
        dy_amax = dy_pl = dyP = wq = None
        x_amax = live(ctx.x_amax)
        x_planes = getattr(ctx, 'x_planes', False)
        if ctx.mode == 'stem_fused':
            x, weight, mean, invstd, gamma, beta = ctx.saved_tensors
            gp, bp, wp = cfg.get('gamma_param'), cfg.get('beta_param'), cfg.get('weight_param')

            def fresh(p):
                return p is not None and getattr(p, '_y4_grad_fresh', False) and p.grad is not None
            sink = fresh(gp) and fresh(bp) and ctx.needs_input_grad[3] and ctx.needs_input_grad[4]
            wsink = fresh(wp) and ctx.needs_input_grad[1]
            dw, dgamma, dbeta = stem_bn_act_bwd_raw(x, weight, dz, mean, invstd, gamma, beta, act,
                                                    gp.grad if sink else None, bp.grad if sink else None,
                                                    wp.grad if wsink else None)
            if sink and dgamma is gp.grad and dbeta is bp.grad:
                gp._y4_grad_fresh = bp._y4_grad_fresh = False
                gp._y4_grad_ready()
                bp._y4_grad_ready()
                dgamma = dbeta = None
            if wsink:
                wp._y4_grad_fresh = False
                if dw is not wp.grad:
                    wp.grad.add_(dw)
                wp._y4_grad_ready()
                dw = None
            return None, dw if ctx.needs_input_grad[1] else None, None, dgamma, dbeta, None, None
        if ctx.mode in ('bn_train', 'bn_eval_grad'):
            x, weight, y, mean, invstd, gamma, beta = ctx.saved_tensors
            gp, bp = cfg.get('gamma_param'), cfg.get('beta_param')
            sink = (gp is not None and bp is not None and getattr(gp, '_y4_grad_fresh', False)
                    and getattr(bp, '_y4_grad_fresh', False) and gp.grad is not None and bp.grad is not None
# ... 741 lines not shown
```

yolov4_amd/yolo/model/yolov4.py:

```python
import os
from collections import OrderedDict
from typing import Dict

import torch
from torch import nn

from ... import ops
from ...darknet.darknet import ConvBNAct, CSPDownSample0, CSPDownSample, chain, geo_of, observed, plan_for, soft, takes_planes
from .yololayer import YOLOLayer

L = 'leaky_relu'


def _five(big, small):
    return nn.Sequential(ConvBNAct(big, small, 1, 1, act=L), ConvBNAct(small, big, 3, 1, act=L),
                         ConvBNAct(big, small, 1, 1, act=L), ConvBNAct(small, big, 3, 1, act=L),
                         ConvBNAct(big, small, 1, 1, act=L))


class Backbone(nn.Module):

    def __init__(self):
        super().__init__()
        self.stem = ConvBNAct(3, 32, 3, 1, act='mish')
# ... 159 lines not shown
        self.yolo2 = nn.Sequential(ConvBNAct(256, 512, 3, 1, act=L),
                                   ConvBNAct(512, oc, 1, 1, bias=True, bn=False, act='linear'),
                                   YOLOLayer(cfg, layer_no=1, device=device))
        self.yolo3 = nn.Sequential(ConvBNAct(512, 1024, 3, 1, act=L),
                                   ConvBNAct(1024, oc, 1, 1, bias=True, bn=False, act='linear'),
                                   YOLOLayer(cfg, layer_no=2, device=device))

    def logits(self, p1, p2, p3):
        assert p1.shape[1] == 128 and p2.shape[1] == 256 and p3.shape[1] == 512
        out = []
        for h, p in ((self.yolo1, p1), (self.yolo2, p2), (self.yolo3, p3)):
            want = takes_planes(h[1], geo=geo_of(p)) and not observed(self, h, h[0], h[1])
            out.append(h[1](h[0](p, out_planes=bool(want))))
        return out

    def forward(self, p1, p2, p3):
        if observed(self.yolo1, self.yolo2, self.yolo3):
            return tuple(h(p) for h, p in ((self.yolo1, p1), (self.yolo2, p2), (self.yolo3, p3)))
        return tuple(h[2](lg) for h, lg in zip((self.yolo1, self.yolo2, self.yolo3), self.logits(p1, p2, p3)))


class YOLOv4(nn.Module):

    def __init__(self, cfg: Dict, device=None):
        super().__init__()
        assert cfg['TYPE'] == 'YOLOv4'
        self.backbone = Backbone()
        self.neck = Neck()
        self.head = Head(cfg, device=device)
        self._init(ckpt_path=cfg['BACKBONE_PRETRAINED'])

    def _init(self, ckpt_path=None):
        for m in self.modules():
            if isinstance(m, nn.Conv2d):
                nn.init.kaiming_normal_(m.weight, mode="fan_out", nonlinearity="relu")
                if m.bias is not None:
                    nn.init.constant_(m.bias, 0)
            elif isinstance(m, nn.BatchNorm2d):
                nn.init.normal_(m.weight, 0, 0.01)
                nn.init.constant_(m.bias, 0)
        if ckpt_path is not None and os.path.isfile(ckpt_path):
            ckpt = torch.load(ckpt_path, map_location='cpu', weights_only=True)['state_dict']
            ckpt = OrderedDict((k.replace("module.backbone.", ""), v) for k, v in ckpt.items() if 'backbone' in k)
            self.backbone.load_state_dict(ckpt, strict=True)

    def forward(self, x):
        if x.dtype != torch.float32:
            x = x.float()
        B, H, W = geo_of(x)
        hp = tuple(soft(takes_planes(h[0], geo=(B, -(-H // st), -(-W // st))), self.neck, self.neck.pan, self.head, h, h[0])
                   for h, st in ((self.head.yolo1, 8), (self.head.yolo2, 16), (self.head.yolo3, 32)))
        seen = observed(self.backbone, self.neck, self.neck.spp, self.neck.spp.conv1, self.neck.fpn)
        readers = ((self.neck.fpn.conv11,), (self.neck.fpn.conv4,), () if seen else (self.neck.spp.conv1[0],))
        p1, p2, p3 = self.neck(*self.backbone(x, readers=readers), head_planes=hp)
        if self.training:
            return list(self.head(p1, p2, p3))
        if observed(self.head, self.head.yolo1, self.head.yolo2, self.head.yolo3):
            return torch.cat(list(self.head(p1, p2, p3)), dim=1)
        logits = self.head.logits(p1, p2, p3)
        layers = (self.head.yolo1[2], self.head.yolo2[2], self.head.yolo3[2])
        counts = [ly.n_anchors * lg.shape[2] * lg.shape[3] for ly, lg in zip(layers, logits)]
        n_total = sum(counts)
        out = torch.empty((x.shape[0], n_total, 5 + layers[0].n_classes), device=x.device, dtype=torch.float32)
        off = 0
        for ly, lg, n in zip(layers, logits, counts):
            ly.decode_into(lg, out, n_total, off)
            off += n
        return out
```

Before: 452.2.

## Batch all conv filter plane preparation into two grouped kernel launches per step

After: 454.3 (median of 6 runs). Within noise of the previous version (+0.5%).

```diff
diff --git a/include/yolov4_amd.h b/include/yolov4_amd.h
--- a/include/yolov4_amd.h
+++ b/include/yolov4_amd.h
@@ -32,7 +32,7 @@
 int y4_get_planes_bf16(void);
 int y4_conv_planes_fit(int B, int H, int W, int Cin, int Cout, int k, int stride, int dgrad_planes);
 size_t y4_conv2d_fwd_workspace(int Cin, int Cout, int k);
-int y4_conv2d_fwd_f32(const float* x, int ldx, const float* w, float* y, int ldy,
+int y4_conv2d_fwd_f32(const float* x, int ldx, const float* w , float* y, int ldy,
                       int B, int H, int W, int Cin, int Cout, int k, int stride,
                       const float* scale, const float* shift, int act,
                       const float* residual, int ldr, const unsigned* x_amax ,
@@ -50,7 +50,7 @@
 int y4_last_conv_kernel(char* buf, int cap);
 
 size_t y4_conv2d_bnstats_workspace(int B, int H, int W, int Cin, int Cout, int k, int stride);
-int y4_conv2d_fwd_bnstats_f32(const float* x, int ldx, const float* w, float* y, int ldy,
+int y4_conv2d_fwd_bnstats_f32(const float* x, int ldx, const float* w , float* y, int ldy,
                               int B, int H, int W, int Cin, int Cout, int k, int stride,
                               float* partials, size_t partial_bytes, long long* nparts_host,
                               const unsigned* x_amax ,
@@ -58,10 +58,31 @@
                               void* dgrad_filter ,
                               size_t dgrad_filter_bytes , void* stream);
 
+#define Y4_FILTER_F16X2 0
+#define Y4_FILTER_BF16  1
+typedef struct y4_filter_desc {
+    const float* w;
+    long long fwd_off;
+    long long tr_off;
+    int Cout, Cin, kk;
+    int Cout_fwd;
+    int Cout_pad;
+    int mirror;
+    int format;
+    int blocks_max, first_max;
+    int blocks_split, first_split;
+    int reserved;
+} y4_filter_desc;
+int y4_conv2d_filter_table_layout(y4_filter_desc* table_host, int n_filters, size_t* arena_bytes, int* total_blocks_max,
+                                  int* total_blocks_split);
+int y4_conv2d_prepare_filters_f32(const y4_filter_desc* table_dev, const y4_filter_desc* table_host, int n_filters,
+                                  int total_blocks_max, int total_blocks_split, void* arena, size_t arena_bytes, void* stream);
+int y4_conv2d_dgrad_filter_mirror(int x_planes, int H, int W, int Cin, int Cout, int k, int stride);
+
 int y4_planes_split_f32(const float* x, int ldx, long long M, int C, const unsigned* amax, void* planes, void* stream);
 int y4_planes_split_into_f32(const float* x, int ldx, long long M, int C, const unsigned* amax, void* planes, int ld_planes, int c_valid,
                              void* stream);
-int y4_conv2d_fwd_planes_f32(const void* x_planes, const float* w, float* y, int ldy,
+int y4_conv2d_fwd_planes_f32(const void* x_planes, const float* w , float* y, int ldy,
                              int B, int H, int W, int Cin, int Cout, int k, int stride,
                              float* partials, size_t partial_bytes, long long* nparts_host, const unsigned* x_amax,
                              void* workspace, size_t workspace_bytes,
@@ -136,6 +157,11 @@
                                 float* mean, float* invstd, float* running_mean, float* running_var,
                                 long long* num_batches_tracked, float momentum, float eps,
                                 void* workspace, size_t workspace_bytes, void* stream);
+int y4_bn_finalize_partials_bound_f32(const float* partials, long long nparts, long long M, int C,
+                                      float* mean, float* invstd, float* running_mean, float* running_var,
+                                      long long* num_batches_tracked, float momentum, float eps,
+                                      const float* gamma, const float* beta, const unsigned* res_amax, const unsigned* floor_word,
+                                      unsigned* bound_out, void* workspace, size_t workspace_bytes, void* stream);
 int y4_bn_planes_bound_f32(const float* gamma, const float* beta, int C, long long M, const unsigned* floor_word, unsigned* out,
                            void* stream);
 int y4_bn_act_fwd_f32(const float* y, int ldy, const float* mean, const float* invstd,
diff --git a/yolov4_amd/_lib.py b/yolov4_amd/_lib.py
--- a/yolov4_amd/_lib.py
+++ b/yolov4_amd/_lib.py
@@ -29,6 +29,9 @@
     'y4_amax_f32': (I, [P, I, L, I, P, P]),
     'y4_conv2d_prepared_bytes': (Z, [I, I]),
     'y4_conv2d_prepare_filter_f32': (I, [P, I, I, P, Z, P]),
+    'y4_conv2d_filter_table_layout': (I, [P, I, P, P, P]),
+    'y4_conv2d_prepare_filters_f32': (I, [P, P, I, I, I, P, Z, P]),
+    'y4_conv2d_dgrad_filter_mirror': (I, [I, I, I, I, I, I, I]),
     'y4_conv2d_fwd_prepared_f32': (I, [P, I, P, P, I, I, I, I, I, I, I, I, P, P, I, P, I, P, P, P]),
     'y4_amax_merge_u32': (I, [P, P, P]),
     'y4_last_conv_kernel': (I, [ctypes.c_char_p, I]),
@@ -59,6 +62,7 @@
     'y4_bn_workspace': (Z, [L, I]),
     'y4_bn_finalize_workspace': (Z, [I]),
     'y4_bn_finalize_partials_f32': (I, [P, L, L, I, P, P, P, P, P, F, F, P, Z, P]),
+    'y4_bn_finalize_partials_bound_f32': (I, [P, L, L, I, P, P, P, P, P, F, F, P, P, P, P, P, P, Z, P]),
     'y4_bn_stats_f32': (I, [P, I, L, I, P, P, P, P, P, F, F, P, Z, P]),
     'y4_bn_act_fwd_f32': (I, [P, I, P, P, P, P, I, P, I, P, I, L, I, P, I, P, P, P]),
     'y4_bn_planes_bound_f32': (I, [P, P, I, L, P, P, P]),
@@ -144,6 +148,15 @@
                 ('reserved', c_int * 3)]
 
 
+FILTER_F16X2, FILTER_BF16 = 0, 1
+
+
+class FilterDesc(ctypes.Structure):
+    _fields_ = [('w', c_void_p), ('fwd_off', c_longlong), ('tr_off', c_longlong), ('Cout', c_int), ('Cin', c_int), ('kk', c_int),
+                ('Cout_fwd', c_int), ('Cout_pad', c_int), ('mirror', c_int), ('format', c_int), ('blocks_max', c_int),
+                ('first_max', c_int), ('blocks_split', c_int), ('first_split', c_int), ('reserved', c_int)]
+
+
 class AugSrc(ctypes.Structure):
     _fields_ = [('src', c_void_p), ('h', c_int), ('w', c_int), ('pitch', c_longlong), ('swap_rb', c_int),
                 ('crop_left', c_int), ('crop_top', c_int), ('crop_w', c_int), ('crop_h', c_int), ('flip', c_int),
diff --git a/yolov4_amd/csrc/conv_f16x2.hip b/yolov4_amd/csrc/conv_f16x2.hip
--- a/yolov4_amd/csrc/conv_f16x2.hip
+++ b/yolov4_amd/csrc/conv_f16x2.hip
@@ -1368,7 +1368,8 @@
         part[blockIdx.x] = a > b ? a : b;
     }
 }
-__device__ __forceinline__ unsigned amax_fold_partials(const unsigned* __restrict__ part, int nparts, unsigned* __restrict__ out) {
+__device__ __forceinline__ unsigned amax_fold_partials(const unsigned* __restrict__ part, int nparts, unsigned* __restrict__ out,
+                                                       bool first) {
     __shared__ unsigned wmax[4];
     unsigned m = 0u;
     for (int i = threadIdx.x; i < nparts; i += 256) { const unsigned v = part[i]; m = v > m ? v : m; }
@@ -1381,8 +1382,11 @@
     __syncthreads();
     const unsigned a = wmax[0] > wmax[1] ? wmax[0] : wmax[1], b = wmax[2] > wmax[3] ? wmax[2] : wmax[3];
     const unsigned v = a > b ? a : b;
-    if (blockIdx.x == 0 && threadIdx.x == 0) *out = v;
+    if (first && threadIdx.x == 0) *out = v;
     return v;
+}
+__device__ __forceinline__ unsigned amax_fold_partials(const unsigned* __restrict__ part, int nparts, unsigned* __restrict__ out) {
+    return amax_fold_partials(part, nparts, out, blockIdx.x == 0);
 }
 __global__ __launch_bounds__(256) void f16x2_split_filter_folded_kernel(const float* __restrict__ w, unsigned short* __restrict__ planes,
                                                                         long long n, const unsigned* __restrict__ part, int nparts,
@@ -1451,6 +1455,104 @@
     }
 }
 
+using y4_desc = y4_filter_desc;
+__device__ __forceinline__ int filter_of_block(const y4_desc* __restrict__ tab, int n, int b, bool split) {
+    int lo = 0, hi = n - 1;
+    while (lo < hi) {
+        const int mid = (lo + hi + 1) >> 1;
+        const int f = split ? tab[mid].first_split : tab[mid].first_max;
+        if (f <= b) lo = mid; else hi = mid - 1;
+    }
+    return lo;
+}
+__device__ __forceinline__ unsigned short bf16_bits_rn(float v) { return __builtin_bit_cast(unsigned short, (__bf16)v); }
+
+__global__ __launch_bounds__(256) void filters_amax_partials_kernel(const y4_desc* __restrict__ tab, int n_filters,
+                                                                    unsigned char* __restrict__ arena) {
+    __shared__ unsigned wmax[4];
+    const int f = filter_of_block(tab, n_filters, (int)blockIdx.x, false);
+    const y4_desc d = tab[f];
+    const int lb = (int)blockIdx.x - d.first_max;
+    if (lb >= d.blocks_max) return;
+    const float* __restrict__ x = d.w;
+    const long long n = (long long)d.Cout_fwd * d.kk * d.Cin, nv = (long long)d.Cout * d.kk * d.Cin;
+    unsigned m = 0u;
+    const long long n4 = n >> 2;
+    for (long long i = lb * 256ll + threadIdx.x; i < n4; i += (long long)d.blocks_max * 256) {
+        if (4 * i >= nv) break;
+        const f32x4 v = *reinterpret_cast<const f32x4*>(x + 4 * i);
+#pragma unroll
+        for (int e = 0; e < 4; ++e) {
+            const unsigned b = __float_as_uint(v[e]) & 0x7fffffffu;
+            if (b < 0x7f800000u && b > m) m = b;
+        }
+    }
+#pragma unroll
+    for (int off = 32; off > 0; off >>= 1) {
+        const unsigned o = (unsigned)__shfl_xor((int)m, off, 64);
+        m = o > m ? o : m;
+    }
+    if ((threadIdx.x & 63) == 0) wmax[threadIdx.x >> 6] = m;
+    __syncthreads();
+    if (threadIdx.x == 0) {
+        const unsigned a = wmax[0] > wmax[1] ? wmax[0] : wmax[1], b = wmax[2] > wmax[3] ? wmax[2] : wmax[3];
+        reinterpret_cast<unsigned*>(arena + d.fwd_off)[16 + lb] = a > b ? a : b;
+    }
+}
+
+__global__ __launch_bounds__(256) void filters_split_kernel(const y4_desc* __restrict__ tab, int n_filters,
+                                                            unsigned char* __restrict__ arena) {
+    const int f = filter_of_block(tab, n_filters, (int)blockIdx.x, true);
+    const y4_desc d = tab[f];
+    const int lb = (int)blockIdx.x - d.first_split;
+    if (lb >= d.blocks_split) return;
+    const float* __restrict__ w = d.w;
+    const int Cout = d.Cout, Cin = d.Cin, kk = d.kk, Cout_pad = d.Cout_pad;
+    const long long nv = (long long)Cout * kk * Cin, n = (long long)d.Cout_fwd * kk * Cin;
+    const long long total = (long long)Cin * kk * Cout_pad;
+    const long long i0 = lb * 256ll + threadIdx.x, step = (long long)d.blocks_split * 256;
+    unsigned* hdr = reinterpret_cast<unsigned*>(arena + d.fwd_off);
+    unsigned short* planes = reinterpret_cast<unsigned short*>(arena + d.fwd_off + 64 + 4096);
+    unsigned short* planes_t = d.tr_off >= 0 ? reinterpret_cast<unsigned short*>(arena + d.tr_off) : nullptr;
+    if (d.format == Y4_FILTER_BF16) {
+        for (long long i = i0; i < n; i += step) planes[i] = bf16_bits_rn(i < nv ? w[i] : 0.0f);
+        if (planes_t)
+            for (long long i = i0; i < total; i += step) {
+                const int nn = (int)(i % Cout_pad);
+                const long long t = i / Cout_pad;
+                const int tp = (int)(t % kk);
+                const int tap = d.mirror ? kk - 1 - tp : tp;
+                const int c = (int)(t / kk);
+                planes_t[i] = bf16_bits_rn(nn < Cout ? w[((long long)nn * kk + tap) * Cin + c] : 0.0f);
+            }
+        return;
+    }
+    const unsigned amax = amax_fold_partials(hdr + 16, d.blocks_max, hdr, lb == 0);
+    const float s = __uint_as_float(f16x2_scale_exp(amax) << 23);
+    for (long long i = i0; i < n; i += step) {
+        unsigned short hi, lo;
+        split2(i < nv ? w[i] : 0.0f, s, hi, lo);
+        const long long o = (i >> 5) * 64 + (i & 31);
+        planes[o] = hi;
+        planes[o + 32] = lo;
+    }
+    if (!planes_t) return;
+    if (lb == 0 && threadIdx.x == 0) *reinterpret_cast<unsigned*>(arena + d.tr_off + total * 6) = amax;
+    for (long long i = i0; i < total; i += step) {
+        const int nn = (int)(i % Cout_pad);
+        const long long t = i / Cout_pad;
+        const int tp = (int)(t % kk);
+        const int tap = d.mirror ? kk - 1 - tp : tp;
+        const int c = (int)(t / kk);
+        const float v = nn < Cout ? w[((long long)nn * kk + tap) * Cin + c] : 0.0f;
+        unsigned short hi, lo;
+        split2(v, s, hi, lo);
+        const long long o = (i >> 5) * 64 + (i & 31);
+        planes_t[o] = hi;
+        planes_t[o + 32] = lo;
+    }
+}
+
 constexpr int FP_PARTS = 256;
 __global__ __launch_bounds__(256) void f16x2_refresh_filter_kernel(const float* __restrict__ w, unsigned short* __restrict__ planes,
                                                                    long long n, unsigned* part_max, unsigned long long* part_sum,
@@ -1664,11 +1766,28 @@
 
 static int filter_amax_partials(const float* w, long long n, unsigned* part, hipStream_t st) {
     if (reinterpret_cast<uintptr_t>(w) & 15) return -1;
+    const int blocks = filter_amax_blocks(n);
+    hipLaunchKernelGGL(amax_partials_kernel, dim3((unsigned)blocks), dim3(256), 0, st, w, n, part);
+    return (int)blocks;
+}
+
+int filter_amax_blocks(long long n) {
     long long blocks = (n / 4 + 1023) / 1024;
     if (blocks < 1) blocks = 1;
-    if (blocks > AMAX_PART_MAX) blocks = AMAX_PART_MAX;
-    hipLaunchKernelGGL(amax_partials_kernel, dim3((unsigned)blocks), dim3(256), 0, st, w, n, part);
-    return (int)blocks;
+    return (int)(blocks > AMAX_PART_MAX ? AMAX_PART_MAX : blocks);
+}
+
+int f16x2_prepare_filters(const y4_filter_desc* table_dev, int n_filters, int total_blocks_max, int total_blocks_split, void* arena,
+                          hipStream_t st) {
+    if (total_blocks_max > 0) {
+        hipLaunchKernelGGL(filters_amax_partials_kernel, dim3((unsigned)total_blocks_max), dim3(256), 0, st, table_dev, n_filters,
+                           static_cast<unsigned char*>(arena));
+        Y4_CHECK_LAUNCH();
+    }
+    hipLaunchKernelGGL(filters_split_kernel, dim3((unsigned)total_blocks_split), dim3(256), 0, st, table_dev, n_filters,
+                       static_cast<unsigned char*>(arena));
+    Y4_CHECK_LAUNCH();
+    return Y4_OK;
 }
 
 int f16x2_refresh_prepared(const float* w, void* prepared, int Cout, int K, hipStream_t st) {
diff --git a/yolov4_amd/csrc/conv_geom.h b/yolov4_amd/csrc/conv_geom.h
--- a/yolov4_amd/csrc/conv_geom.h
+++ b/yolov4_amd/csrc/conv_geom.h
@@ -47,6 +47,9 @@
                              unsigned* amax_out_t, int Cout, int Cin, int kk, int Cout_pad, bool mirror, hipStream_t st);
 int f16x2_filter_planes_transposed(const float* w, unsigned short* planes, int Cout, int Cin, int kk, int Cout_pad,
                                    unsigned* amax_out, unsigned* part, hipStream_t st, bool mirror = false);
+int filter_amax_blocks(long long n);
+int f16x2_prepare_filters(const y4_filter_desc* table_dev, int n_filters, int total_blocks_max, int total_blocks_split, void* arena,
+                          hipStream_t st);
 int slab_reduce(const float* slabs, float* dw, long long n, int splits, hipStream_t st);
 int amax_launch(const float* x, long long ld, long long M, int C, unsigned* amax_bits, hipStream_t st,
                 bool prezeroed = false);
diff --git a/yolov4_amd/csrc/conv_igemm.hip b/yolov4_amd/csrc/conv_igemm.hip
--- a/yolov4_amd/csrc/conv_igemm.hip
+++ b/yolov4_amd/csrc/conv_igemm.hip
@@ -1627,7 +1627,7 @@
                          const float* residual, int ldr, float* stats, int* nparts, const unsigned* x_amax,
                          unsigned* y_amax, void* workspace, size_t workspace_bytes, void* stream,
                          void* w_prepared = nullptr, void* dgrad_filter = nullptr, size_t dgrad_filter_bytes = 0) {
-    if (!x || (!w && !w_prepared) || !y) return Y4_ERR_NULL;
+    if (!x || !y || (!w && !w_prepared && !(g_conv_mode == 3 && workspace))) return Y4_ERR_NULL;
     if (B <= 0 || H <= 0 || W <= 0 || Cout <= 0 || (k != 1 && k != 3) || (stride != 1 && stride != 2))
         return Y4_ERR_SHAPE;
     if (Cin <= 0 || Cin % BK != 0 || ldx < Cin || ldy < Cout || (ldx & 3) || (residual && ldr < Cout))
@@ -1672,10 +1672,10 @@
                 if (reinterpret_cast<uintptr_t>(dgrad_filter) & 15) return Y4_ERR_SHAPE;
                 const int cp = (Cout + 31) / 32 * 32;
                 unsigned* hdr_t = reinterpret_cast<unsigned*>(static_cast<char*>(dgrad_filter) + (size_t)Cin * k * k * cp * 6);
-                rc = y4::f16x2_filter_planes_dual(w, planes, hdr, hdr + 16, static_cast<unsigned short*>(dgrad_filter), hdr_t, Cout, Cin,
-                                                  k * k, cp, y4::tile_conv_ok(cp, Cout, Cin, k, stride, H, W), y4_stream(stream));
+                rc = !w ? Y4_OK : y4::f16x2_filter_planes_dual(w, planes, hdr, hdr + 16, static_cast<unsigned short*>(dgrad_filter), hdr_t, Cout, Cin,
+                                                               k * k, cp, y4::tile_conv_ok(cp, Cout, Cin, k, stride, H, W), y4_stream(stream));
             } else {
-                rc = y4::f16x2_filter_planes(w, planes, Cout, g.K, hdr, hdr + 16, y4_stream(stream));
+                rc = !w ? Y4_OK : y4::f16x2_filter_planes(w, planes, Cout, g.K, hdr, hdr + 16, y4_stream(stream));
             }
             if (rc != Y4_OK) return rc;
             if (!x_amax) {
@@ -1830,6 +1830,76 @@
     if (prepared_bytes < y4_conv2d_prepared_bytes(Cout, K)) return Y4_ERR_WORKSPACE;
     if ((reinterpret_cast<uintptr_t>(prepared) & 15) || (reinterpret_cast<uintptr_t>(w) & 15)) return Y4_ERR_SHAPE;
     return y4::f16x2_refresh_prepared(w, prepared, Cout, K, y4_stream(stream));
+}
+
+static bool filter_desc_ok(const y4_filter_desc& d) {
+    if (d.Cout <= 0 || d.Cin <= 0 || (d.Cin & 31) || (d.kk != 1 && d.kk != 9)) return false;
+    if (d.Cout_fwd < d.Cout || d.Cout_pad < d.Cout) return false;
+    if (d.format != Y4_FILTER_F16X2 && d.format != Y4_FILTER_BF16) return false;
+    const long long most = (long long)(d.Cout_fwd > d.Cout_pad ? d.Cout_fwd : d.Cout_pad) * d.kk * d.Cin;
+    return most < (1ll << 31);
+}
+static void filter_desc_blocks(const y4_filter_desc& d, int* bmax, int* bsplit) {
+    const long long n = (long long)d.Cout_fwd * d.kk * d.Cin, total = (long long)d.Cin * d.kk * d.Cout_pad;
+    *bmax = d.format == Y4_FILTER_BF16 ? 0 : y4::filter_amax_blocks(n);
+    const long long most = (d.tr_off >= 0 && total > n) ? total : n;
+    long long b = (most + 2047) / 2048;
+    *bsplit = (int)(b < 1 ? 1 : (b > 4096 ? 4096 : b));
+}
+static size_t filter_fwd_bytes(const y4_filter_desc& d) { return FWD_WS_HDR + (size_t)d.Cout_fwd * d.kk * d.Cin * 6; }
+static size_t filter_tr_bytes(const y4_filter_desc& d) { return (size_t)d.Cin * d.kk * d.Cout_pad * 6 + 64 + 4096; }
+
+int y4_conv2d_filter_table_layout(y4_filter_desc* t, int n_filters, size_t* arena_bytes, int* total_blocks_max,
+                                  int* total_blocks_split) {
+    if (!t || !arena_bytes || !total_blocks_max || !total_blocks_split) return Y4_ERR_NULL;
+    if (n_filters < 1) return Y4_ERR_SHAPE;
+    for (int i = 0; i < n_filters; ++i)
+        if (!filter_desc_ok(t[i])) return Y4_ERR_SHAPE;
+    size_t off = 0;
+    long long fm = 0, fs = 0;
+    for (int i = 0; i < n_filters; ++i) {
+        y4_filter_desc& d = t[i];
+        filter_desc_blocks(d, &d.blocks_max, &d.blocks_split);
+        d.first_max = (int)fm; d.first_split = (int)fs;
+        fm += d.blocks_max; fs += d.blocks_split;
+        d.fwd_off = (long long)off;
+        off = (off + filter_fwd_bytes(d) + 255) & ~(size_t)255;
+        if (d.tr_off >= 0) {
+            d.tr_off = (long long)off;
+            off = (off + filter_tr_bytes(d) + 255) & ~(size_t)255;
+        } else d.tr_off = -1;
+        d.reserved = 0;
+        if (fm >= (1ll << 31) || fs >= (1ll << 31)) return Y4_ERR_SHAPE;
+    }
+    *arena_bytes = off; *total_blocks_max = (int)fm; *total_blocks_split = (int)fs;
+    return Y4_OK;
+}
+
+int y4_conv2d_prepare_filters_f32(const y4_filter_desc* table_dev, const y4_filter_desc* t, int n_filters,
+                                  int total_blocks_max, int total_blocks_split, void* arena, size_t arena_bytes, void* stream) {
+    if (!table_dev || !t || !arena) return Y4_ERR_NULL;
+    if (n_filters < 1 || (reinterpret_cast<uintptr_t>(arena) & 255) || (reinterpret_cast<uintptr_t>(table_dev) & 7)) return Y4_ERR_SHAPE;
+    long long fm = 0, fs = 0;
+    for (int i = 0; i < n_filters; ++i) {
+        const y4_filter_desc& d = t[i];
+        if (!d.w) return Y4_ERR_NULL;
+        if (!filter_desc_ok(d) || (reinterpret_cast<uintptr_t>(d.w) & 15)) return Y4_ERR_SHAPE;
+        int bm, bs;
+        filter_desc_blocks(d, &bm, &bs);
+        if (d.blocks_max != bm || d.blocks_split < 1 || d.blocks_split > 65536 || d.first_max != fm || d.first_split != fs) return Y4_ERR_SHAPE;
+        fm += d.blocks_max; fs += d.blocks_split;
+        if (d.fwd_off < 0 || (d.fwd_off & 15) || (d.tr_off >= 0 && (d.tr_off & 15))) return Y4_ERR_SHAPE;
+        if ((size_t)d.fwd_off + filter_fwd_bytes(d) > arena_bytes) return Y4_ERR_WORKSPACE;
+        if (d.tr_off >= 0 && (size_t)d.tr_off + filter_tr_bytes(d) > arena_bytes) return Y4_ERR_WORKSPACE;
+    }
+    if (fm != total_blocks_max || fs != total_blocks_split || fs < 1) return Y4_ERR_SHAPE;
+    return y4::f16x2_prepare_filters(table_dev, n_filters, total_blocks_max, total_blocks_split, arena, y4_stream(stream));
+}
+
+int y4_conv2d_dgrad_filter_mirror(int x_planes, int H, int W, int Cin, int Cout, int k, int stride) {
+    if (x_planes) return stride == 1 ? 1 : 0;
+    const int cp = (Cout + 31) / 32 * 32;
+    return y4::tile_conv_ok(cp, Cout, Cin, k, stride, H, W) ? 1 : 0;
 }
 
 int y4_conv2d_fwd_prepared_f32(const float* x, int ldx, void* w_prepared, float* y, int ldy,
diff --git a/yolov4_amd/csrc/conv_planes.hip b/yolov4_amd/csrc/conv_planes.hip
--- a/yolov4_amd/csrc/conv_planes.hip
+++ b/yolov4_amd/csrc/conv_planes.hip
@@ -1204,7 +1204,7 @@
                              float* partials, size_t partial_bytes, long long* nparts_host, const unsigned* x_amax,
                              void* workspace, size_t workspace_bytes, void* dgrad_filter, size_t dgrad_filter_bytes,
                              int y_bf16, const float* bias, void* stream) {
-    if (!x_planes || !w || !y || !workspace) return Y4_ERR_NULL;
+    if (!x_planes || !y || !workspace) return Y4_ERR_NULL;
     if (bias && (y_bf16 || partials || (reinterpret_cast<uintptr_t>(bias) & 3))) return Y4_ERR_SHAPE;
     if (!pl_mode_ok()) return Y4_ERR_SHAPE;
     const bool bf = pl_bf();
@@ -1226,11 +1226,13 @@
         if (dgrad_filter_bytes < y4_conv2d_dgrad_workspace(Cin, Cout, k)) return Y4_ERR_WORKSPACE;
         if (reinterpret_cast<uintptr_t>(dgrad_filter) & 15) return Y4_ERR_SHAPE;
         unsigned* hdr_t = reinterpret_cast<unsigned*>(static_cast<char*>(dgrad_filter) + (size_t)Cin * k * k * Cout * 6);
-        if (bf) rc = bf16_filter(w, planes, static_cast<unsigned short*>(dgrad_filter), Cout, Cin, k * k, stride == 1, st);
+        if (!w) rc = Y4_OK;
+        else if (bf) rc = bf16_filter(w, planes, static_cast<unsigned short*>(dgrad_filter), Cout, Cin, k * k, stride == 1, st);
         else rc = y4::f16x2_filter_planes_dual(w, planes, hdr, hdr + 16, static_cast<unsigned short*>(dgrad_filter), hdr_t, Cout, Cin, k * k,
                                                Cout, stride == 1, st);
     } else {
-        if (bf) rc = bf16_filter(w, planes, nullptr, Cout, Cin, k * k, false, st);
+        if (!w) rc = Y4_OK;
+        else if (bf) rc = bf16_filter(w, planes, nullptr, Cout, Cin, k * k, false, st);
         else rc = y4::f16x2_filter_planes(w, planes, Cout, k * k * Cin, hdr, hdr + 16, st);
     }
     if (rc != Y4_OK) return rc;
diff --git a/yolov4_amd/csrc/pointwise.hip b/yolov4_amd/csrc/pointwise.hip
--- a/yolov4_amd/csrc/pointwise.hip
+++ b/yolov4_amd/csrc/pointwise.hip
@@ -149,32 +149,9 @@
     }
 }
 
-__global__ __launch_bounds__(256) void bn_finalize_kernel(const double* __restrict__ bacc, int nb, long long M, int C, float eps,
-                                                          float momentum, float* __restrict__ mean, float* __restrict__ invstd,
-                                                          float* __restrict__ rmean, float* __restrict__ rvar, long long* nbt) {
-    __shared__ double red[2][8][32];
-    double s, ss;
-    fold_rows32(bacc, nb, C, blockIdx.x * 32, red, s, ss);
-    if (blockIdx.x == 0 && threadIdx.x == 0 && nbt) *nbt += 1;
-    const int c = blockIdx.x * 32 + (threadIdx.x & 31);
-    if ((threadIdx.x >> 5) != 0 || c >= C) return;
-    const double mu = s / (double)M;
-    double var = ss / (double)M - mu * mu;
-    if (var < 0) var = 0;
-    mean[c] = (float)mu;
-    invstd[c] = (float)(1.0 / sqrt(var + (double)eps));
-    if (rmean) rmean[c] = (1.0f - momentum) * rmean[c] + momentum * (float)mu;
-    if (rvar) {
-        const double unb = M > 1 ? var * (double)M / (double)(M - 1) : var;
-        rvar[c] = (1.0f - momentum) * rvar[c] + momentum * (float)unb;
-    }
-}
-
-
-__global__ __launch_bounds__(256) void bn_planes_bound_kernel(const float* __restrict__ gamma, const float* __restrict__ beta, int C,
-                                                              float sqrt_m1, const unsigned* __restrict__ res_amax,
-                                                              unsigned* __restrict__ out, const unsigned* __restrict__ floor_word = nullptr) {
-    __shared__ float red[256];
+__device__ __forceinline__ void bn_planes_bound_block(const float* __restrict__ gamma, const float* __restrict__ beta, int C,
+                                                      float sqrt_m1, const unsigned* __restrict__ res_amax,
+                                                      unsigned* __restrict__ out, const unsigned* __restrict__ floor_word, float* red) {
     float m = 0.f;
     for (int c = threadIdx.x; c < C; c += 256) m = fmaxf(m, fabsf(gamma[c]) * sqrt_m1 + fabsf(beta[c]));
     red[threadIdx.x] = m;
@@ -190,6 +167,43 @@
         if (floor_word && *floor_word > w) w = *floor_word;
         *out = w;
     }
+}
+
+__global__ __launch_bounds__(256) void bn_finalize_kernel(const double* __restrict__ bacc, int nb, long long M, int C, float eps,
+                                                          float momentum, float* __restrict__ mean, float* __restrict__ invstd,
+                                                          float* __restrict__ rmean, float* __restrict__ rvar, long long* nbt,
+                                                          const float* __restrict__ gamma = nullptr, const float* __restrict__ beta = nullptr,
+                                                          float sqrt_m1 = 0.f, const unsigned* __restrict__ res_amax = nullptr,
+                                                          const unsigned* __restrict__ floor_word = nullptr,
+                                                          unsigned* __restrict__ bound_out = nullptr) {
+    __shared__ double red[2][8][32];
+    double s, ss;
+    fold_rows32(bacc, nb, C, blockIdx.x * 32, red, s, ss);
+    if (blockIdx.x == 0 && threadIdx.x == 0 && nbt) *nbt += 1;
+    const int c = blockIdx.x * 32 + (threadIdx.x & 31);
+    if ((threadIdx.x >> 5) == 0 && c < C) {
+        const double mu = s / (double)M;
+        double var = ss / (double)M - mu * mu;
+        if (var < 0) var = 0;
+        mean[c] = (float)mu;
+        invstd[c] = (float)(1.0 / sqrt(var + (double)eps));
+        if (rmean) rmean[c] = (1.0f - momentum) * rmean[c] + momentum * (float)mu;
+        if (rvar) {
+            const double unb = M > 1 ? var * (double)M / (double)(M - 1) : var;
+            rvar[c] = (1.0f - momentum) * rvar[c] + momentum * (float)unb;
+        }
+    }
+    if (blockIdx.x != 0 || !bound_out) return;
+    __syncthreads();
+    bn_planes_bound_block(gamma, beta, C, sqrt_m1, res_amax, bound_out, floor_word, reinterpret_cast<float*>(&red[0][0][0]));
+}
+
+
+__global__ __launch_bounds__(256) void bn_planes_bound_kernel(const float* __restrict__ gamma, const float* __restrict__ beta, int C,
+                                                              float sqrt_m1, const unsigned* __restrict__ res_amax,
+                                                              unsigned* __restrict__ out, const unsigned* __restrict__ floor_word = nullptr) {
+    __shared__ float red[256];
+    bn_planes_bound_block(gamma, beta, C, sqrt_m1, res_amax, out, floor_word, red);
 }
 
 
@@ -880,6 +894,25 @@
     { const int rc = fold_partials(partials, nparts, C, bacc, &nb, st); if (rc != Y4_OK) return rc; }
     hipLaunchKernelGGL(bn_finalize_kernel, dim3((C + 31) / 32), dim3(256), 0, st, bacc, nb, M, C, eps, momentum, mean,
                        invstd, running_mean, running_var, num_batches_tracked);
+    Y4_CHECK_LAUNCH();
+    return Y4_OK;
+}
+
+int y4_bn_finalize_partials_bound_f32(const float* partials, long long nparts, long long M, int C,
+                                      float* mean, float* invstd, float* running_mean, float* running_var,
+                                      long long* num_batches_tracked, float momentum, float eps,
+                                      const float* gamma, const float* beta, const unsigned* res_amax, const unsigned* floor_word,
+                                      unsigned* bound_out, void* workspace, size_t workspace_bytes, void* stream) {
+    if (!partials || !mean || !invstd || !workspace || !gamma || !beta || !bound_out) return Y4_ERR_NULL;
+    if (nparts <= 0 || M <= 0 || C <= 0) return Y4_ERR_SHAPE;
+    if (workspace_bytes < y4_bn_finalize_workspace(C)) return Y4_ERR_WORKSPACE;
+    hipStream_t st = y4_stream(stream);
+    double* bacc = static_cast<double*>(workspace) + 2 * C;
+    int nb = 0;
+    { const int rc = fold_partials(partials, nparts, C, bacc, &nb, st); if (rc != Y4_OK) return rc; }
+    hipLaunchKernelGGL(bn_finalize_kernel, dim3((C + 31) / 32), dim3(256), 0, st, bacc, nb, M, C, eps, momentum, mean,
+                       invstd, running_mean, running_var, num_batches_tracked, gamma, beta,
+                       sqrtf((float)(M > 1 ? M - 1 : 1)), res_amax, floor_word, bound_out);
     Y4_CHECK_LAUNCH();
     return Y4_OK;
 }
diff --git a/yolov4_amd/darknet/darknet.py b/yolov4_amd/darknet/darknet.py
--- a/yolov4_amd/darknet/darknet.py
+++ b/yolov4_amd/darknet/darknet.py
@@ -45,7 +45,8 @@
                'dres_put': dres_put, 'dres_take': dres_take, 'out_planes': out_planes, 'dx_put': dx_put,
                'out_cat': getattr(out, 'y4_cat', None), 'scale_from': scale_from,
                'x_twin': getattr(x, 'y4_twin', None) if takes_planes(self, x.shape[2:], geo_of(x)) else None,
-               'grad': torch.is_grad_enabled()}
+               'grad': torch.is_grad_enabled(),
+               'filter_prep': self.__dict__.pop('_y4_prep', None)}
         if self.has_bn:
             use_batch_stats = self.training or n.running_mean is None
             cfg['training'] = use_batch_stats
@@ -65,6 +66,8 @@
             w = self.conv.weight
         cfg['weight_param'] = self.conv.weight
         z = ops.ConvBNActFn.apply(x, w, self.conv.bias, gamma, beta, residual, cfg)
+        if 'filter_need' in io:
+            self.__dict__['_y4_filter_need'] = io['filter_need']
         if io.get('z_planes'):
             z = ops.as_planes(z)
         if io.get('z_twin') is not None:
diff --git a/yolov4_amd/ops.py b/yolov4_amd/ops.py
--- a/yolov4_amd/ops.py
+++ b/yolov4_amd/ops.py
@@ -1,10 +1,11 @@
 import ctypes
 import functools
 import os
+import weakref
 
 import torch
 
-from ._lib import ACT_IDS, Y4Error, check, float_array, int_array, lib
+from ._lib import ACT_IDS, FILTER_BF16, FILTER_F16X2, FilterDesc, Y4Error, check, float_array, int_array, lib
 
 CL = torch.channels_last
 
@@ -260,12 +261,138 @@
     return _ws(lib().y4_conv2d_dgrad_workspace(Cin, Cout, k), device)
 
 
-def conv_fwd_bnstats_raw(x, w, k, s, running_mean, running_var, nbt, momentum, eps, x_amax=None, dgrad_filter=None):
+FILTER_BATCH = {'on': os.environ.get('Y4_FILTER_BATCH', '1') != '0'}
+FILTER_STATS = {'tables': 0, 'prepared': 0, 'taken': 0, 'own': 0}
+_FILTER_BATCHES = weakref.WeakKeyDictionary()
+
+
+def filter_need(bf16, Cout, Cin, k, Cout_fwd, Cout_pad, want_t, mirror):
+    return (FILTER_BF16 if bf16 else FILTER_F16X2, int(Cout), int(Cin), int(k) * int(k), int(Cout_fwd), int(Cout_pad),
+            1 if want_t else 0, 1 if (want_t and mirror) else 0)
+
+
+@functools.lru_cache(maxsize=4096)
+def _dgrad_mirror(x_planes, H, W, Cin, Cout, k, s):
+    return bool(lib().y4_conv2d_dgrad_filter_mirror(1 if x_planes else 0, int(H), int(W), int(Cin), int(Cout), int(k), int(s)))
+
+
+class FilterSlice:
+    __slots__ = ('need', 'wptr', 'fwd', 'tr')
+
+    def __init__(self, need, wptr, fwd, tr):
+        self.need, self.wptr, self.fwd, self.tr = need, wptr, fwd, tr
+
+
+def _take_prep(cfg, need, weight):
+    io = cfg.get('io')
+    if io is not None:
+        io['filter_need'] = need
+    p = cfg.get('filter_prep')
+    if p is None or need is None or p.need != need or p.wptr != krsc(weight).data_ptr():
+        FILTER_STATS['own'] += need is not None
+        return None
+    FILTER_STATS['taken'] += 1
+    return p
+
+
+def filter_table_layout(needs):
+    n = len(needs)
+    table = (FilterDesc * n)()
+    for d, (fmt, Cout, Cin, kk, Cout_fwd, Cout_pad, want_t, mirror) in zip(table, needs):
+        d.format, d.Cout, d.Cin, d.kk, d.Cout_fwd, d.Cout_pad, d.mirror = fmt, Cout, Cin, kk, Cout_fwd, Cout_pad, mirror
+        d.tr_off = 0 if want_t else -1
+    arena, tmax, tsplit = ctypes.c_size_t(0), ctypes.c_int(0), ctypes.c_int(0)
+    check(lib().y4_conv2d_filter_table_layout(table, n, ctypes.byref(arena), ctypes.byref(tmax), ctypes.byref(tsplit)),
+          'conv2d_filter_table_layout')
+    return table, arena.value, tmax.value, tsplit.value
+
+
+class FilterBatch:
+
+    def __init__(self, key, weights, needs):
+        self.key, self.needs = key, needs
+        FILTER_STATS['tables'] += 1
+        self.table, self.arena_bytes, self.tmax, self.tsplit = filter_table_layout(needs)
+        for d, w in zip(self.table, weights):
+            d.w = w.data_ptr()
+        self.wptrs = [w.data_ptr() for w in weights]
+        dev = weights[0].device
+        host = torch.frombuffer(bytearray(bytes(self.table)), dtype=torch.uint8)
+        self.table_dev = host.to(dev)
+        L = lib()
+        self.sizes = [(L.y4_conv2d_fwd_workspace(nd[2], nd[4], 3 if nd[3] == 9 else 1),
+                       L.y4_conv2d_dgrad_workspace(nd[2], nd[5], 3 if nd[3] == 9 else 1) if nd[6] else 0) for nd in needs]
+
+    def prepare(self):
+        dev = self.table_dev.device
+        arena = torch.empty(self.arena_bytes, dtype=torch.uint8, device=dev)
+        if arena.data_ptr() % 256:
+            return None
+        check(lib().y4_conv2d_prepare_filters_f32(_ptr(self.table_dev), self.table, len(self.needs), self.tmax, self.tsplit,
+                                                  _ptr(arena), self.arena_bytes, _stream()), 'conv2d_prepare_filters')
+        FILTER_STATS['prepared'] += 1
+        out = []
+        for d, nd, wp, (nf, nt) in zip(self.table, self.needs, self.wptrs, self.sizes):
+            out.append(FilterSlice(nd, wp, arena[d.fwd_off:d.fwd_off + nf], arena[d.tr_off:d.tr_off + nt] if nt else None))
+        return out
+
+
+def filter_batch_for(owner, layers):
+    if not FILTER_BATCH['on']:
+        return None
+    L = lib()
+    mode = (L.y4_get_conv_mode(), L.y4_get_planes_bf16())
+    mods, weights, needs, key = [], [], [], [mode]
+    for m in layers:
+        nd = getattr(m, '_y4_filter_need', None)
+        w = m.conv.weight
+        if nd is None or not w.is_cuda or w.dtype != torch.float32 or not _is_krsc_dense(w) or w.data_ptr() % 16:
+            continue
+        mods.append(m)
+        weights.append(w)
+        needs.append(nd)
+        key.append((w.data_ptr(), tuple(w.shape), tuple(w.stride()), nd))
+    if not mods or len({w.device for w in weights}) != 1:
+        return None
+    key = tuple(key)
+    fb = _FILTER_BATCHES.get(owner)
+    if fb is None or fb.key != key:
+        fb = FilterBatch(key, weights, needs)
+        _FILTER_BATCHES[owner] = fb
+    slices = fb.prepare()
+    return list(zip(mods, slices)) if slices is not None else None
+
+
+def _bnstats_fused(Cin, Cout, k, s):
+    return fast_conv_shape(Cin, k, s) and not (Cin == 3 and Cout > 32) and Cout % 4 == 0
+
+
+def _finalize(part, nparts, M, Cout, running_mean, running_var, nbt, momentum, eps, device, bound=None):
+    L = lib()
+    mean = torch.empty(Cout, device=device, dtype=torch.float32)
+    invstd = torch.empty(Cout, device=device, dtype=torch.float32)
+    wsb = L.y4_bn_finalize_workspace(Cout)
+    ws = _ws(wsb, device)
+    if bound is not None:
+        gamma, beta, res_cell, cell = bound
+        check(L.y4_bn_finalize_partials_bound_f32(_ptr(part), nparts, M, Cout, _ptr(mean), _ptr(invstd), _ptr(running_mean),
+                                                  _ptr(running_var), _ptr(nbt), float(momentum), float(eps), _ptr(gamma), _ptr(beta),
+                                                  _ptr(res_cell), None, _ptr(cell), _ptr(ws), wsb, _stream()),
+              'bn_finalize_partials_bound')
+    else:
+        check(L.y4_bn_finalize_partials_f32(_ptr(part), nparts, M, Cout, _ptr(mean), _ptr(invstd),
+                                            _ptr(running_mean), _ptr(running_var), _ptr(nbt), float(momentum), float(eps),
+                                            _ptr(ws), wsb, _stream()), 'bn_finalize_partials')
+    return mean, invstd
+
+
+def conv_fwd_bnstats_raw(x, w, k, s, running_mean, running_var, nbt, momentum, eps, x_amax=None, dgrad_filter=None, prep=None,
+                         bound=None):
     L = lib()
     B, Cin, H, W = x.shape
     Cout = w.shape[0]
     Ho, Wo = conv_out_hw(H, W, k, s)
-    if not fast_conv_shape(Cin, k, s) or (Cin == 3 and Cout > 32) or Cout % 4:
+    if not _bnstats_fused(Cin, Cout, k, s):
         if Cout % 4:
             raise Y4Error('BatchNorm over a channel count that is not a multiple of 4 is not supported')
         y = conv_fwd_raw(x, w, k, s, out=empty_nhwc(B, Cout, Ho, Wo, x.device, pad_to=4), x_amax=x_amax)
@@ -287,19 +414,13 @@
         x, ldx = as_nhwc(x)
         n = ctypes.c_longlong(0)
         nbytes = L.y4_conv2d_fwd_workspace(Cin, Cout, k)
-        cws = _ws(nbytes, x.device)
-        check(L.y4_conv2d_fwd_bnstats_f32(_ptr(x), ldx, _ptr(w), _ptr(y), ldy, B, H, W, Cin, Cout, k, s,
+        cws = prep if prep is not None else _ws(nbytes, x.device)
+        check(L.y4_conv2d_fwd_bnstats_f32(_ptr(x), ldx, None if prep is not None else _ptr(w), _ptr(y), ldy, B, H, W, Cin, Cout, k, s,
                                           _ptr(part), pbytes, ctypes.byref(n), _ptr(x_amax), _ptr(cws), nbytes,
                                           _ptr(dgrad_filter), dgrad_filter.numel() if dgrad_filter is not None else 0, _stream()),
               'conv2d_fwd_bnstats')
         nparts = n.value
-    mean = torch.empty(Cout, device=x.device, dtype=torch.float32)
-    invstd = torch.empty(Cout, device=x.device, dtype=torch.float32)
-    wsb = L.y4_bn_finalize_workspace(Cout)
-    ws = _ws(wsb, x.device)
-    check(L.y4_bn_finalize_partials_f32(_ptr(part), nparts, B * Ho * Wo, Cout, _ptr(mean), _ptr(invstd),
-                                        _ptr(running_mean), _ptr(running_var), _ptr(nbt), float(momentum), float(eps),
-                                        _ptr(ws), wsb, _stream()), 'bn_finalize_partials')
+    mean, invstd = _finalize(part, nparts, B * Ho * Wo, Cout, running_mean, running_var, nbt, momentum, eps, x.device, bound)
     return y, mean, invstd
 
 
@@ -410,19 +531,18 @@
     return Planes(buf, (B, C, H, W), amax)
 
 
-def conv_fwd_planes_raw(xp, w, k, s, stats=True, dgrad_filter=None, y_bf16=False, bias=None, out=None):
+def conv_fwd_planes_raw(xp, w, k, s, stats=True, dgrad_filter=None, y_bf16=False, bias=None, out=None, prep=None, cout=None):
     L = lib()
     B, Cin, H, W = xp.shape
-    Cout = w.shape[0]
+    Cout = cout if w is None else w.shape[0]
     Ho, Wo = conv_out_hw(H, W, k, s)
     y = out if _slot_ok(out, (B, Cout, Ho, Wo)) else empty_nhwc(B, Cout, Ho, Wo, xp.buf.device)
-    w = krsc(w)
     nbytes = L.y4_conv2d_fwd_workspace(Cin, Cout, k)
-    ws = _ws(nbytes, xp.buf.device)
+    ws = prep if prep is not None else _ws(nbytes, xp.buf.device)
     pbytes = ((B * Ho * Wo + 127) // 128) * 2 * Cout * 4 if stats else 0
     part = _ws(pbytes, xp.buf.device) if stats else None
     n = ctypes.c_longlong(0)
-    check(L.y4_conv2d_fwd_planes_f32(_ptr(xp.buf), _ptr(w), _ptr(y), nhwc_pitch(y), B, H, W, Cin, Cout, k, s,
+    check(L.y4_conv2d_fwd_planes_f32(_ptr(xp.buf), None if prep is not None else _ptr(krsc(w)), _ptr(y), nhwc_pitch(y), B, H, W, Cin, Cout, k, s,
                                      _ptr(part), pbytes, ctypes.byref(n), _ptr(xp.amax), _ptr(ws), nbytes,
                                      _ptr(dgrad_filter), dgrad_filter.numel() if dgrad_filter is not None else 0,
                                      1 if y_bf16 else 0, _ptr(bias), _stream()),
@@ -430,18 +550,12 @@
     return (y, part, n.value) if stats else y
 
 
-def conv_fwd_planes_bnstats_raw(xp, w, k, s, running_mean, running_var, nbt, momentum, eps, dgrad_filter=None, y_bf16=False):
-    L = lib()
-    y, part, nparts = conv_fwd_planes_raw(xp, w, k, s, dgrad_filter=dgrad_filter, y_bf16=y_bf16)
+def conv_fwd_planes_bnstats_raw(xp, w, k, s, running_mean, running_var, nbt, momentum, eps, dgrad_filter=None, y_bf16=False,
+                                prep=None, bound=None):
+    y, part, nparts = conv_fwd_planes_raw(xp, w, k, s, dgrad_filter=dgrad_filter, y_bf16=y_bf16, prep=prep)
     Cout = w.shape[0]
     M = y.shape[0] * y.shape[2] * y.shape[3]
-    mean = torch.empty(Cout, device=y.device, dtype=torch.float32)
-    invstd = torch.empty(Cout, device=y.device, dtype=torch.float32)
-    wsb = L.y4_bn_finalize_workspace(Cout)
-    ws = _ws(wsb, y.device)
-    check(L.y4_bn_finalize_partials_f32(_ptr(part), nparts, M, Cout, _ptr(mean), _ptr(invstd),
-                                        _ptr(running_mean), _ptr(running_var), _ptr(nbt), float(momentum), float(eps),
-                                        _ptr(ws), wsb, _stream()), 'bn_finalize_partials')
+    mean, invstd = _finalize(part, nparts, M, Cout, running_mean, running_var, nbt, momentum, eps, y.device, bound)
     return y, mean, invstd
 
 
@@ -595,7 +709,8 @@
             and out.data_ptr() % 16 == 0)
 
 
-def bn_act_fwd_raw(y, mean, invstd, gamma, beta, act, residual=None, out=None, out_amax=None, planes=False, y_bf16=False, cell=None):
+def bn_act_fwd_raw(y, mean, invstd, gamma, beta, act, residual=None, out=None, out_amax=None, planes=False, y_bf16=False, cell=None,
+                   bound_cell=None):
     L = lib()
     B, C, H, W = y.shape
     y, ldy = as_nhwc(y)
@@ -631,9 +746,9 @@
         given = cell is not None
         if given and (residual is not None or both):
             raise Y4Error('a given plane scale goes with a plain planes-only result')
-        cell = cell if given else planes_cell(y.device)
+        cell = cell if given else (bound_cell if bound_cell is not None else planes_cell(y.device))
         res_cell = amax_of(residual) if residual is not None else None
-        if given:
+        if given or bound_cell is not None:
             mode = 1
         elif residual is not None and res_cell is None:
             check(L.y4_bn_act_fwd_f32(*args, None, C, B * H * W, C, _ptr(cell), yb, None, None, _stream()), 'bn_act_fwd(measure)')
@@ -768,12 +883,14 @@
         torch.autograd.Variable._execution_engine.queue_callback(join_side_stream)
 
 
-def _pad_out_channels(weight, bias, cop):
+def _pad_out_channels(weight, bias, cop, filter_too=True):
     co = weight.shape[0]
     if cop == co:
         return weight, bias
-    wp = torch.zeros((cop,) + tuple(weight.shape[1:]), dtype=weight.dtype, device=weight.device).contiguous(memory_format=torch.channels_last)
-    wp[:co].copy_(weight)
+    wp = None
+    if filter_too:
+        wp = torch.zeros((cop,) + tuple(weight.shape[1:]), dtype=weight.dtype, device=weight.device).contiguous(memory_format=torch.channels_last)
+        wp[:co].copy_(weight)
     bp = None
     if bias is not None:
         bp = torch.zeros(cop, dtype=bias.dtype, device=bias.device)
@@ -827,11 +944,23 @@
             if x.shape[0] * conv_out_hw(x.shape[2], x.shape[3], k, s)[0] * conv_out_hw(x.shape[2], x.shape[3], k, s)[1] <= 1:
                 raise ValueError('Expected more than 1 value per channel when training')
             ctx.dgrad_filter = None
-            if ((f16 or (bfm and xp is not None)) and ctx.needs_input_grad[0] and x.shape[1] % 32 == 0 and fast_conv_shape(x.shape[1], k, s)
-                    and weight.shape[0] % 4 == 0 and (xp is None or weight.shape[0] % 32 == 0)
-                    and not (bfm and xp is not None and s == 2
-                             and not s2_plane_dgrad(x.shape[0], x.shape[2], x.shape[3], x.shape[1], weight.shape[0]))):
-                ctx.dgrad_filter = dgrad_filter_buffer(x.shape[1], weight.shape[0], k, x.device)
+            Cin, Cout = x.shape[1], weight.shape[0]
+            want_t = bool((f16 or (bfm and xp is not None)) and ctx.needs_input_grad[0] and Cin % 32 == 0 and fast_conv_shape(Cin, k, s)
+                          and Cout % 4 == 0 and (xp is None or Cout % 32 == 0)
+                          and not (bfm and xp is not None and s == 2
+                                   and not s2_plane_dgrad(x.shape[0], x.shape[2], x.shape[3], Cin, Cout)))
+            need = None
+            if xp is not None:
+                need = filter_need(bfm, Cout, Cin, k, Cout, Cout, want_t, s == 1)
+            elif f16 and _bnstats_fused(Cin, Cout, k, s):
+                need = filter_need(False, Cout, Cin, k, Cout, (Cout + 31) // 32 * 32, want_t,
+                                   want_t and _dgrad_mirror(False, x.shape[2], x.shape[3], Cin, Cout, k, s))
+            prep = _take_prep(cfg, need, weight)
+            if prep is not None:
+                ctx.dgrad_filter = prep.tr
+            elif want_t:
+                ctx.dgrad_filter = dgrad_filter_buffer(Cin, Cout, k, x.device)
+            prep = prep.fwd if prep is not None else None
             ybf = ctx.y_bf16 = bool(bfm and xp is not None and weight.shape[0] % 32 == 0 and _BF16_Y)
             cb = cfg.get('out_cat')
             if (xp is None and residual is None and not cfg.get('out_planes') and not (cb is not None and cb.planes)
@@ -847,26 +976,33 @@
                 if io is not None:
                     io['z_amax'] = z_amax
                 return z
+            want = cfg.get('out_planes')
+            sf = cfg.get('scale_from')
+            sf_cell = sf.cell if (sf is not None and sf.planes and sf.cell is not None and want is True) else None
+            bound = None
+            if (want and f16 and planes_mode() == 'f16x2' and Cout % 32 == 0 and (want == 'both' or dest is None)
+                    and not (cb is not None and cb.planes) and sf_cell is None
+                    and (residual is None or amax_of(residual) is not None)
+                    and (xp is not None or _bnstats_fused(Cin, Cout, k, s))):
+                bound = (gamma, beta, amax_of(residual) if residual is not None else None, planes_cell(x.device))
+            more = {key: v for key, v in (('prep', prep), ('bound', bound)) if v is not None}
             if xp is not None:
                 y, mean, invstd = conv_fwd_planes_bnstats_raw(xp, weight, k, s, cfg['running_mean'], cfg['running_var'],
                                                               cfg['nbt'], cfg['momentum'], cfg['eps'], dgrad_filter=ctx.dgrad_filter,
-                                                              y_bf16=ybf)
+                                                              y_bf16=ybf, **more)
             else:
                 y, mean, invstd = conv_fwd_bnstats_raw(x, weight, k, s, cfg['running_mean'], cfg['running_var'],
                                                        cfg['nbt'], cfg['momentum'], cfg['eps'], x_amax=x_amax,
-                                                       dgrad_filter=ctx.dgrad_filter)
-            want = cfg.get('out_planes')
-            cb = cfg.get('out_cat')
+                                                       dgrad_filter=ctx.dgrad_filter, **more)
             if cb is not None and cb.planes:
                 z = bn_act_fwd_raw(y, mean, invstd, gamma, beta, act, residual, out=dest, planes='slot', y_bf16=ybf)
                 if io is not None:
                     io['z_planes'] = True
                 z_amax = cb.cell[0:1] if cb.cell is not None else None
             elif want and (f16 or bfm) and y.shape[1] % 32 == 0 and (want == 'both' or dest is None):
-                sf = cfg.get('scale_from')
                 z = bn_act_fwd_raw(y, mean, invstd, gamma, beta, act, residual, out=dest if want == 'both' else None,
-                                   planes='both' if want == 'both' else True, y_bf16=ybf,
-                                   cell=sf.cell if (sf is not None and sf.planes and sf.cell is not None and want is True) else None)
+                                   planes='both' if want == 'both' else True, y_bf16=ybf, cell=sf_cell,
+                                   bound_cell=bound[3] if bound is not None else None)
                 z_amax = getattr(z, 'y4_amax', None)
                 if io is not None:
                     io['z_planes'] = want != 'both'
@@ -910,11 +1046,17 @@
             co = weight.shape[0]
             q = 64 if bfm else 32
             cop = (co + q - 1) // q * q
-            wpad, bpad = _pad_out_channels(weight, bias, cop)
+            want_t = bool(ctx.needs_input_grad[0])
+            prep = _take_prep(cfg, filter_need(bfm, co, x.shape[1], k, cop, cop, want_t, True), weight)
+            wpad, bpad = _pad_out_channels(weight, bias, cop, filter_too=prep is None)
             Ho, Wo = conv_out_hw(x.shape[2], x.shape[3], k, s)
             zf = empty_nhwc(x.shape[0], cop, Ho, Wo, x.device)
-            ctx.dgrad_filter = dgrad_filter_buffer(x.shape[1], cop, k, x.device) if ctx.needs_input_grad[0] else None
-            conv_fwd_planes_raw(xp, wpad, k, s, stats=False, dgrad_filter=ctx.dgrad_filter, bias=bpad, out=zf)
+            if prep is not None:
+                ctx.dgrad_filter = prep.tr
+            else:
+                ctx.dgrad_filter = dgrad_filter_buffer(x.shape[1], cop, k, x.device) if want_t else None
+            conv_fwd_planes_raw(xp, wpad, k, s, stats=False, dgrad_filter=ctx.dgrad_filter, bias=bpad, out=zf,
+                                prep=prep.fwd if prep is not None else None, cout=cop)
             z = zf[:, :co]
             ctx.save_for_backward(xp.buf, weight)
             ctx.mode = 'nobn_linear'
diff --git a/yolov4_amd/yolo/model/yolov4.py b/yolov4_amd/yolo/model/yolov4.py
--- a/yolov4_amd/yolo/model/yolov4.py
+++ b/yolov4_amd/yolo/model/yolov4.py
@@ -235,9 +235,21 @@
                    for h, st in ((self.head.yolo1, 8), (self.head.yolo2, 16), (self.head.yolo3, 32)))
         seen = observed(self.backbone, self.neck, self.neck.spp, self.neck.spp.conv1, self.neck.fpn)
         readers = ((self.neck.fpn.conv11,), (self.neck.fpn.conv4,), () if seen else (self.neck.spp.conv1[0],))
-        p1, p2, p3 = self.neck(*self.backbone(x, readers=readers), head_planes=hp)
-        if self.training:
-            return list(self.head(p1, p2, p3))
+        prepared = None
+        if self.training and torch.is_grad_enabled() and x.is_cuda:
+            if getattr(self, '_y4_convs', None) is None:
+                self.__dict__['_y4_convs'] = [m for m in self.modules() if isinstance(m, ConvBNAct)]
+            prepared = ops.filter_batch_for(self, self._y4_convs)
+        try:
+            for m, sl in prepared or ():
+                m.__dict__['_y4_prep'] = sl
+            p1, p2, p3 = self.neck(*self.backbone(x, readers=readers), head_planes=hp)
+            if self.training:
+                return list(self.head(p1, p2, p3))
+        finally:
+            for m, _ in prepared or ():
+                m.__dict__.pop('_y4_prep', None)
+            prepared = None
         if observed(self.head, self.head.yolo1, self.head.yolo2, self.head.yolo3):
             return torch.cat(list(self.head(p1, p2, p3)), dim=1)
         logits = self.head.logits(p1, p2, p3)
```
